# OpenGene/AfterQC

Measured on AMD Instinct MI355X. Metric: Mreads/s (paired 2x150 bp) end-to-end good/bad split, higher is better.
Workload: dtype u8

## Files before the change

### afterqc_amd/capi.py

```python
import ctypes as C
import os

import numpy as np

HERE = os.path.dirname(os.path.abspath(__file__))
LIB_PATH = os.environ.get("AQC_LIB") or os.path.join(HERE, "csrc", "libafterqc_hip.so")

AQC_MAX_READ_LEN = 1000
AQC_QC_COLS = 1024

FLAG_NAMES = ["GOOD", "BADBCD1", "BADBCD2", "BADTRIM1", "BADTRIM2", "BADBBL", "BADLEN", "BADPOL", "BADLQC",
              "BADNCT", "BADDIFF", "BADMISMATCH"]
(GOOD, BADBCD1, BADBCD2, BADTRIM1, BADTRIM2, BADBBL, BADLEN, BADPOL, BADLQC, BADNCT, BADDIFF,
 BADMISMATCH) = range(12)
N_FLAGS = 12
EDIT_FIX_R2, EDIT_FIX_R1, EDIT_MASK = 1, 2, 3
STORE_OFF, STORE_OVERLAP, STORE_MERGED = 0, 1, 2

C_TOTAL_READS, C_TOTAL_BASES, C_GOOD_READS, C_GOOD_BASES, C_FLAG0 = 0, 1, 2, 3, 4
C_READ_CORRECTED = C_FLAG0 + N_FLAGS
(C_BASE_CORRECTED, C_BASE_SKIPPED_CORRECTION, C_BASE_ZERO_QUAL_MASKED, C_OVERLAPPED, C_OVERLAP_LEN_SUM,
 C_OVERLAP_BASE_SUM, C_OVERLAP_BASE_ERR, C_TRIMMED_ADAPTER_BASE, C_TRIMMED_ADAPTER_READ,
 C_ERR_MATRIX0) = range(C_READ_CORRECTED + 1, C_READ_CORRECTED + 11)
N_COUNTERS = C_ERR_MATRIX0 + 16

(QC_TOTAL_NUM, QC_TOTAL_QUAL, QC_BASE_COUNT_A, QC_BASE_COUNT_T, QC_BASE_COUNT_C, QC_BASE_COUNT_G, QC_BASE_QUAL_A,
 QC_BASE_QUAL_T, QC_BASE_QUAL_C, QC_BASE_QUAL_G, QC_DISCONTINUITY, QC_GC_HIST, QC_SCALARS, QC_ROWS) = range(14)
QC_R1_PRE, QC_R2_PRE, QC_R1_POST, QC_R2_POST = range(4)
K_FILTER_OVERLAP, K_QC_STAT, N_KERNELS = 0, 1, 2
UINT64_MAX = (1 << 64) - 1

ERRORS = {-1: "HIP runtime error", -2: "bad argument", -3: "read longer than AQC_MAX_READ_LEN", -4: "no gfx950 device",
          -5: "bad call sequence", -6: "byte outside the reference's COMP alphabet", -7: "unsupported option value",
          -8: "quality line too short for the overlap walk (IndexError upstream)"}
ERR_ARG, ERR_ALPHABET, ERR_INDEX = -2, -6, -8
RECORD_ERRORS = (ERR_ARG, ERR_ALPHABET, ERR_INDEX)

EDIT_DTYPE = np.dtype([("o", "<u2"), ("kind", "u1"), ("base", "u1"), ("qual", "u1")])
RESULT_DTYPE = np.dtype([("flag", "u1"), ("n_edits", "u1"), ("start1", "<u2"), ("len1", "<u2"), ("start2", "<u2"),
                         ("len2", "<u2"), ("offset", "<i2"), ("overlap_len", "<u2"), ("distance", "<u2"),
                         ("edits", EDIT_DTYPE, (3,)), ("barcode", "u1")])
assert RESULT_DTYPE.itemsize == 32
SPAN_EVENT_DTYPE = np.dtype([("in_start", "<u4"), ("in_len", "<u4"), ("out_len", "<u4")])
CENSUS_HIT_DTYPE = np.dtype([("index", "<u8"), ("lane", "<i8"), ("tile_no", "<i8"), ("tile", "<i8"), ("x", "<i8"), ("y", "<i8"),
                             ("name_off", "<u4"), ("name_len", "<u4"), ("count", "<i4"), ("surface", "u1"), ("swath", "u1"),
                             ("camera", "u1"), ("base", "u1"), ("status", "u1"), ("wide", "u1"), ("pad_", "u1", (6,))])
CENSUS_OK, CENSUS_NO_NAME, CENSUS_RAISE = 0, 1, 2


def assemble_spans(chunk, end, events, stream0):
    out = []
    cursor = poff = 0
    for e in events:
        a, ln, ol = int(e["in_start"]), int(e["in_len"]), int(e["out_len"])
        out.append(bytes(chunk[cursor:a]))
        out.append(bytes(stream0[poff:poff + ol]))
        poff += ol
        cursor = a + ln
    out.append(bytes(chunk[cursor:end]))
    return b"".join(out)


class Config(C.Structure):
    _fields_ = [(n, C.c_int32) for n in (
        "paired", "count_r2_bases", "trim_front", "trim_tail", "trim_front2", "trim_tail2", "seq_len_req",
        "poly_size_limit", "allow_mismatch_in_poly", "qualified_quality_phred", "unqualified_base_limit",
        "n_base_limit", "no_overlap", "no_correction", "mask_mismatch", "barcode", "barcode_length",
        "barcode_verify_len")] + [("barcode_verify", C.c_uint8 * 32), ("debubble", C.c_int32), ("qc_kmer", C.c_int32)]

    def set_verify(self, verify):
        v = verify.encode() if isinstance(verify, str) else bytes(verify)
        if len(v) > 32:
            raise ValueError("barcode_verify longer than 32 bytes")
        self.barcode_verify_len = len(v)
        for i, ch in enumerate(v):
            self.barcode_verify[i] = ch


class CutConfig(C.Structure):
    _fields_ = [("front", C.c_int32), ("tail", C.c_int32), ("right", C.c_int32), ("window", C.c_int32), ("mean_quality", C.c_int32)]

    @property
    def on(self):
        return bool(self.front or self.tail or self.right)


class AdapterConfig(C.Structure):
    _fields_ = [("len1", C.c_int32), ("len2", C.c_int32), ("min_overlap", C.c_int32), ("seq1", C.c_uint8 * 64), ("seq2", C.c_uint8 * 64)]

    def __init__(self, seq1=b"", seq2=b"", min_overlap=4):
        super().__init__()
        seq1, seq2 = [s.encode() if isinstance(s, str) else bytes(s) for s in (seq1, seq2)]
        self.len1, self.len2, self.min_overlap = len(seq1), len(seq2), int(min_overlap)
        for dst, s in ((self.seq1, seq1), (self.seq2, seq2)):
            for i, ch in enumerate(s[:64]):
                dst[i] = ch

    @property
    def on(self):
        return bool(self.len1 or self.len2)

    def adapters(self):
        return bytes(self.seq1[:min(self.len1, 64)]), bytes(self.seq2[:min(self.len2, 64)])


class PolyConfig(C.Structure):
    _fields_ = [("min_len", C.c_int32 * 4)]

    def __init__(self, a=0, c=0, g=0, t=0):
        super().__init__()
        for i, v in enumerate((a, c, g, t)):
            self.min_len[i] = int(v)

    @property
    def on(self):
        return any(self.min_len)

    def lengths(self):
        return tuple(int(v) for v in self.min_len)


class BatchStruct(C.Structure):
    _fields_ = [("n", C.c_uint64), ("first_index", C.c_uint64),
                ("seq1", C.c_void_p), ("qual1", C.c_void_p), ("off1", C.c_void_p), ("qoff1", C.c_void_p),
                ("len1", C.c_void_p), ("bytes1", C.c_uint64), ("qbytes1", C.c_uint64),
                ("seq2", C.c_void_p), ("qual2", C.c_void_p), ("off2", C.c_void_p), ("qoff2", C.c_void_p),
                ("len2", C.c_void_p), ("bytes2", C.c_uint64), ("qbytes2", C.c_uint64),
                ("aux_lane", C.c_void_p), ("aux_tile", C.c_void_p), ("aux_x", C.c_void_p), ("aux_y", C.c_void_p),
                ("aux_ok", C.c_void_p), ("qlen1", C.c_void_p), ("qlen2", C.c_void_p)]


def _ptr(a):
    return None if a is None else a.ctypes.data_as(C.c_void_p)


class TextChunk(C.Structure):
    _fields_ = [("text1", C.c_void_p), ("bytes1", C.c_uint64), ("text2", C.c_void_p), ("bytes2", C.c_uint64),
                ("final1", C.c_int32), ("final2", C.c_int32), ("max_records", C.c_uint64), ("first_index", C.c_uint64)]


class TextExtent(C.Structure):
    _fields_ = [("offset", C.c_uint64), ("bytes", C.c_uint64), ("device_text", C.c_void_p)]


class FrameInfo(C.Structure):
    _fields_ = [("n", C.c_uint64), ("avail1", C.c_uint64), ("avail2", C.c_uint64), ("consumed1", C.c_uint64),
                ("consumed2", C.c_uint64), ("eof1", C.c_int32), ("eof2", C.c_int32), ("max_len", C.c_uint32),
                ("next_len1", C.c_uint32)]


class PipeIO(C.Structure):
    _fields_ = [("in_path", C.c_char_p * 2), ("in_mem", C.c_void_p * 2), ("in_mem_bytes", C.c_uint64 * 2),
                ("gzip_in", C.c_int32 * 2), ("out_path", (C.c_char_p * 3) * 2), ("gzip_out", C.c_int32), ("gzip_level", C.c_int32)]


class PipeOpts(C.Structure):
    _fields_ = [("chunk_records", C.c_uint64), ("qc_sample", C.c_int64), ("store_overlap", C.c_int32), ("no_output", C.c_int32),
                ("chunk_index0", C.c_uint64), ("chunk_index_stride", C.c_uint64)]


class PipeResult(C.Structure):
    _fields_ = [("records", C.c_uint64), ("chunks", C.c_uint64), ("bytes_out", C.c_uint64 * 6), ("anomaly", C.c_int32),
                ("fused_chunks", C.c_int32), ("extra_bases", C.c_uint64), ("seconds", C.c_double)] + [(k, C.c_double) for k in (
                    "t_read", "t_count", "t_wait_ring", "t_frame", "t_kernels", "t_wait_set", "t_fetch", "t_write")]

    def breakdown(self):
        return {k: round(getattr(self, k), 4) for k in ("seconds", "t_read", "t_count", "t_wait_ring", "t_frame", "t_kernels",
                                                        "t_wait_set", "t_fetch", "t_write")}


class HostBuffer:

    def __init__(self, lib, nbytes):
        self._lib = lib
        self.nbytes = int(nbytes)
        self.ptr = lib.aqc_host_alloc(self.nbytes)
        if not self.ptr:
            raise MemoryError("aqc_host_alloc(%d) failed" % self.nbytes)
        self.array = np.ctypeslib.as_array((C.c_uint8 * self.nbytes).from_address(self.ptr))
        self.view = memoryview(self.array)

    def free(self):
        if self.ptr:
            self.array = None
            self.view = None
            self._lib.aqc_host_free(self.ptr)
            self.ptr = None

# ... 68 lines not shown
    def _pack_strings(seqs, quals):
        enc = [s.encode("latin-1") if isinstance(s, str) else bytes(s) for s in seqs]
        lens = np.array([len(s) for s in enc], dtype=np.uint32)
        off, total = Batch._offsets(lens)
        sa = np.zeros(total, dtype=np.uint8)
        qa = np.zeros(total, dtype=np.uint8)
        for i, s in enumerate(enc):
            o = int(off[i])
            sa[o:o + len(s)] = np.frombuffer(s, dtype=np.uint8)
        if quals is not None:
            for i, q in enumerate(quals):
                q = q.encode("latin-1") if isinstance(q, str) else bytes(q)
                if len(q) != int(lens[i]):
                    raise ValueError("record %d: quality length %d != sequence length %d" % (i, len(q), int(lens[i])))
                o = int(off[i])
                qa[o:o + len(q)] = np.frombuffer(q, dtype=np.uint8)
        else:
            for i in range(len(enc)):
                o = int(off[i])
                qa[o:o + int(lens[i])] = ord("I")
        return sa, qa, off, lens

    @classmethod
    def from_raw(cls, rb1, rb2=None, first_index=0):
        b = cls(rb1.n, first_index)
        b.seq1 = b.qual1 = rb1.text
        b.off1, b.qoff1, b.len1 = rb1.seq_off, rb1.qual_off, rb1.seq_len
        irregular = not np.array_equal(rb1.seq_len, rb1.qual_len)
        if rb2 is not None:
            b.seq2 = b.qual2 = rb2.text
            b.off2, b.qoff2, b.len2 = rb2.seq_off, rb2.qual_off, rb2.seq_len
            irregular = irregular or not np.array_equal(rb2.seq_len, rb2.qual_len)
        if irregular:
            b.qlen1 = np.ascontiguousarray(rb1.qual_len, dtype=np.uint32)
            if rb2 is not None:
                b.qlen2 = np.ascontiguousarray(rb2.qual_len, dtype=np.uint32)
        return b

    def set_aux(self, lane, tile, x, y, ok):
        self.aux = (np.ascontiguousarray(lane, dtype=np.int32), np.ascontiguousarray(tile, dtype=np.int32),
                    np.ascontiguousarray(x, dtype=np.int32), np.ascontiguousarray(y, dtype=np.int32),
                    np.ascontiguousarray(ok, dtype=np.uint8))

    def max_len(self):
        m = int(self.len1.max()) if self.n else 0
        if self.len2 is not None and self.n:
            m = max(m, int(self.len2.max()))
        return m

    def as_struct(self):
        s = BatchStruct()
        s.n = self.n
        s.first_index = self.first_index
        s.seq1, s.qual1, s.off1, s.len1 = _ptr(self.seq1), _ptr(self.qual1), _ptr(self.off1), _ptr(self.len1)
        s.qoff1 = _ptr(self.qoff1)
        s.bytes1 = 0 if self.seq1 is None else self.seq1.size
        s.qbytes1 = 0 if self.qual1 is None else self.qual1.size
        s.seq2, s.qual2, s.off2, s.len2 = _ptr(self.seq2), _ptr(self.qual2), _ptr(self.off2), _ptr(self.len2)
        s.qoff2 = _ptr(self.qoff2)
        s.bytes2 = 0 if self.seq2 is None else self.seq2.size
        s.qbytes2 = 0 if self.qual2 is None else self.qual2.size
        if self.aux is not None:
            s.aux_lane, s.aux_tile, s.aux_x, s.aux_y, s.aux_ok = (_ptr(a) for a in self.aux)
        s.qlen1, s.qlen2 = _ptr(self.qlen1), _ptr(self.qlen2)
        return s

    def read1(self, i):
        o = int(self.off1[i]); l = int(self.len1[i])
        q = o if self.qoff1 is None else int(self.qoff1[i])
        ql = l if self.qlen1 is None else int(self.qlen1[i])
        return self.seq1[o:o + l].tobytes(), self.qual1[q:q + ql].tobytes()

    def read2(self, i):
        o = int(self.off2[i]); l = int(self.len2[i])
        q = o if self.qoff2 is None else int(self.qoff2[i])
        ql = l if self.qlen2 is None else int(self.qlen2[i])
        return self.seq2[o:o + l].tobytes(), self.qual2[q:q + ql].tobytes()


class AqcError(RuntimeError):
    def __init__(self, code, msg):
        RuntimeError.__init__(self, "afterqc_hip error %d (%s): %s" % (code, ERRORS.get(code, "?"), msg))
        self.code = code


_lib = None


def load_library():
    global _lib
    if _lib is not None:
        return _lib
    if not os.path.exists(LIB_PATH):
        raise RuntimeError("HIP library %s is missing: build it with `python __graft_entry__.py build` "
                           "(hipcc --offload-arch=gfx950); afterqc_amd has no CPU fallback" % LIB_PATH)
    lib = C.CDLL(LIB_PATH)
    P = C.c_void_p
    lib.aqc_abi_version.restype = C.c_int
    lib.aqc_device_count.restype = C.c_int
    lib.aqc_last_error.restype = C.c_char_p
    lib.aqc_create.argtypes = [C.c_int, C.c_int, C.POINTER(P)]
    lib.aqc_destroy.argtypes = [P]
    lib.aqc_destroy.restype = None
    lib.aqc_device_name.argtypes = [P, C.c_char_p, C.c_int]
    lib.aqc_set_config.argtypes = [P, C.POINTER(Config)]
    lib.aqc_set_circles.argtypes = [P, P, P, P, P, P, C.c_int32]
    lib.aqc_reset_stats.argtypes = [P]
    lib.aqc_set_quality_cut.argtypes = [P, C.POINTER(CutConfig)]
    lib.aqc_get_cut_stats.argtypes = [P, P]
    lib.aqc_cut_ms.argtypes = [P, C.c_int, C.POINTER(C.c_float)]
    lib.aqc_quality_cut_views.argtypes = [P, C.POINTER(BatchStruct), C.POINTER(CutConfig), C.c_int32, C.c_int32, P]
    lib.aqc_set_adapter_trim.argtypes = [P, C.POINTER(AdapterConfig)]
    lib.aqc_get_adapter_stats.argtypes = [P, P]
    lib.aqc_adapter_ms.argtypes = [P, C.c_int, C.POINTER(C.c_float)]
    lib.aqc_adapter_views.argtypes = [P, C.POINTER(BatchStruct), C.POINTER(AdapterConfig), C.c_int32, C.c_int32, P, P]
    lib.aqc_set_poly_trim.argtypes = [P, C.POINTER(PolyConfig)]
    lib.aqc_get_poly_stats.argtypes = [P, P]
    lib.aqc_poly_ms.argtypes = [P, C.c_int, C.POINTER(C.c_float)]
    lib.aqc_poly_views.argtypes = [P, C.POINTER(BatchStruct), C.POINTER(PolyConfig), C.c_int32, C.c_int32, P, P]
    lib.aqc_upload.argtypes = [P, C.c_int, C.POINTER(BatchStruct)]
    lib.aqc_run.argtypes = [P, C.c_int, C.c_uint64]
    lib.aqc_qc_stat.argtypes = [P, C.c_int, C.c_int, C.c_int, C.c_uint64, C.c_uint64, C.c_int]
    lib.aqc_fetch_results.argtypes = [P, C.c_int, P, C.c_uint64]
    lib.aqc_format_spans.argtypes = [P, C.c_int, C.c_uint64, C.c_int32, P, P]
    lib.aqc_fetch_span_events.argtypes = [P, C.c_int, C.c_int, P, C.c_uint64]
    lib.aqc_span_end.argtypes = [P, C.c_int, C.c_uint64, P]
    lib.aqc_poly_census.argtypes = [P, C.c_int, C.c_int32, P]
    lib.aqc_fetch_census.argtypes = [P, C.c_int, P, C.c_uint64]
    lib.aqc_census_ms.argtypes = [P, C.c_int, P]
    lib.aqc_format_fused.argtypes = [P, C.c_int]
    lib.aqc_fetch_quality_views.argtypes = [P, C.c_int, C.c_int, P, C.c_uint64]
    lib.aqc_error_record.argtypes = [P, C.c_int, C.POINTER(C.c_uint64)]
    lib.aqc_sync.argtypes = [P, C.c_int]
    lib.aqc_last_deferred.argtypes = [P, C.c_int, P, C.c_uint64, C.POINTER(C.c_uint64)]
    lib.aqc_last_deferred.restype = C.c_int
    lib.aqc_last_verdict_words.argtypes = [P, C.c_int]
    lib.aqc_last_verdict_words.restype = C.c_int
    lib.aqc_kernel_ms.argtypes = [P, C.c_int, P]
    lib.aqc_timing_reset.argtypes = [P, C.c_int]
    lib.aqc_timing_mean.argtypes = [P, C.c_int, P, P]
    lib.aqc_get_counters.argtypes = [P, P]
    lib.aqc_get_histograms.argtypes = [P, P, P, C.c_int32]
    lib.aqc_get_qc.argtypes = [P, C.c_int, P]
    lib.aqc_get_kmers.argtypes = [P, C.c_int, P, P, P, C.c_uint64, C.POINTER(C.c_uint64)]
    lib.aqc_overlap.argtypes = [P, C.POINTER(BatchStruct), P, P, P]
    lib.aqc_read_stats.argtypes = [P, C.POINTER(BatchStruct), C.c_int32, C.c_int32, C.c_int32, P, P, P]
    lib.aqc_edit_distance.argtypes = [P, C.POINTER(BatchStruct), P]
    lib.aqc_frame.argtypes = [P, C.c_int, C.POINTER(TextChunk), C.POINTER(FrameInfo)]
    lib.aqc_frame_mixed.argtypes = [P, C.c_int, C.POINTER(TextChunk), C.POINTER(TextExtent), C.c_uint64, C.c_uint8, C.POINTER(TextExtent), C.c_uint64, C.c_uint8,
                                    C.POINTER(FrameInfo)]
    lib.aqc_frame_mixed.restype = C.c_int
    lib.aqc_reframe.argtypes = [P, C.c_int, C.POINTER(FrameInfo)]
    lib.aqc_reframe.restype = C.c_int
    lib.aqc_format.argtypes = [P, C.c_int, C.c_uint64, C.c_int32, P]
    lib.aqc_format_plain.argtypes = [P, C.c_int, C.c_int, C.c_uint64, C.c_int32, P]
    lib.aqc_fetch_text.argtypes = [P, C.c_int, C.c_int, C.c_int, P, C.c_uint64]
    lib.aqc_fetch_streams.argtypes = [P, C.c_int, C.c_int32, C.POINTER(C.c_void_p * 6), C.POINTER(C.c_uint64 * 6)]
    lib.aqc_gunzip_dev.argtypes = [C.c_int, P, C.c_uint64, P, C.c_uint64, C.POINTER(C.c_uint64), P, C.c_int, C.c_uint64, C.c_uint64]
    lib.aqc_bunzip2_dev.argtypes = [C.c_int, P, C.c_uint64, P, C.c_uint64, C.POINTER(C.c_uint64), P, C.c_int, C.c_uint64]
    lib.aqc_bunzip2_dev.restype = C.c_int
    lib.aqc_gunzip_probe.argtypes = [C.c_int, C.c_int, P, C.c_uint64, C.c_int, P, P, P, C.c_uint32, C.c_uint32, C.c_uint32, P, C.c_uint64, P, P, P, P, C.c_uint64,
                                     C.POINTER(C.c_uint64), P, C.c_uint64, C.POINTER(C.c_uint64), P, C.POINTER(C.c_uint64)]
    lib.aqc_gunzip_probe.restype = C.c_int
    lib.aqc_compress.argtypes = [P, C.c_int, C.c_int32, P]
    lib.aqc_fetch_gz.argtypes = [P, C.c_int, C.c_int, C.c_int, P, C.c_uint64]
    lib.aqc_pipe_create.argtypes = [C.POINTER(P), C.c_int32, C.c_int32, C.c_int32, C.POINTER(P)]
    lib.aqc_pipe_create.restype = C.c_int
    lib.aqc_pipe_destroy.argtypes = [P]
    lib.aqc_pipe_destroy.restype = None
    lib.aqc_pipe_run.argtypes = [P, C.POINTER(PipeIO), C.POINTER(PipeOpts), C.POINTER(PipeResult)]
    lib.aqc_pipe_run.restype = C.c_int
    lib.aqc_pipe_last_error.restype = C.c_char_p
    lib.aqc_source_open.argtypes = [C.c_char_p, C.c_int32, C.c_int32]
    lib.aqc_source_open.restype = P
    lib.aqc_source_read.argtypes = [P, P, C.c_uint64]
    lib.aqc_source_read.restype = C.c_int64
    lib.aqc_source_close.argtypes = [P]
    lib.aqc_source_close.restype = None
    lib.aqc_source_open2.argtypes = [C.c_char_p, C.c_int32, C.c_int32, C.c_uint64]
    lib.aqc_source_open2.restype = P
    lib.aqc_source_error.argtypes = [P]
    lib.aqc_source_error.restype = C.c_char_p
    lib.aqc_source_gz_stats.argtypes = [P, C.POINTER(C.c_uint64 * 4)]
    lib.aqc_source_gz_stats.restype = C.c_int
    lib.aqc_gz_input_stats.argtypes = [C.POINTER(C.c_uint64 * 4)]
    lib.aqc_gz_input_stats.restype = C.c_int
    lib.aqc_bz2_input_stats.argtypes = [C.POINTER(C.c_uint64 * 4)]
    lib.aqc_bz2_input_stats.restype = C.c_int
    lib.aqc_gz_deflate_block.argtypes = [P, C.c_uint64, C.c_int32, P, C.c_uint64, C.POINTER(C.c_uint64)]
    lib.aqc_gz_deflate_block.restype = C.c_int
    lib.aqc_gz_inflate_raw.argtypes = [P, C.c_uint64, P, C.c_uint64]
    lib.aqc_gz_inflate_raw.restype = C.c_int64
    lib.aqc_gz_crc32.argtypes = [C.c_uint32, P, C.c_uint64]
    lib.aqc_gz_crc32.restype = C.c_uint32
    lib.aqc_host_count_newlines.argtypes = [P, C.c_uint64]
    lib.aqc_host_count_newlines.restype = C.c_uint64
    lib.aqc_bgzf_compress.argtypes = [P, C.c_uint64, C.c_int32, P, C.c_uint64, C.POINTER(C.c_uint64)]
    lib.aqc_bgzf_compress.restype = C.c_int
    lib.aqc_pipe_split.argtypes = [C.POINTER(PipeIO), C.c_int32, C.c_uint64, C.c_int32, P, P, C.c_uint64, C.POINTER(C.c_uint64),
                                   C.POINTER(C.c_uint32)]
    lib.aqc_pipe_split.restype = C.c_int
    lib.aqc_host_alloc.argtypes = [C.c_uint64]
    lib.aqc_host_alloc.restype = C.c_void_p
    lib.aqc_host_free.argtypes = [P]
    lib.aqc_host_free.restype = None
    for name in ("aqc_create", "aqc_device_name", "aqc_set_config", "aqc_set_circles", "aqc_reset_stats", "aqc_upload",
                 "aqc_run", "aqc_qc_stat", "aqc_fetch_results", "aqc_sync", "aqc_kernel_ms", "aqc_timing_reset",
                 "aqc_timing_mean", "aqc_get_counters", "aqc_get_histograms", "aqc_get_qc", "aqc_get_kmers",
                 "aqc_overlap", "aqc_read_stats", "aqc_edit_distance", "aqc_frame", "aqc_frame_mixed", "aqc_reframe", "aqc_format", "aqc_format_plain",
                 "aqc_fetch_text", "aqc_fetch_quality_views", "aqc_error_record", "aqc_format_spans", "aqc_fetch_span_events", "aqc_span_end", "aqc_format_fused",
                 "aqc_poly_census", "aqc_fetch_census", "aqc_census_ms", "aqc_set_quality_cut", "aqc_get_cut_stats", "aqc_cut_ms", "aqc_quality_cut_views",
                 "aqc_set_adapter_trim", "aqc_get_adapter_stats", "aqc_adapter_ms", "aqc_adapter_views",
                 "aqc_set_poly_trim", "aqc_get_poly_stats", "aqc_poly_ms", "aqc_poly_views"):
        getattr(lib, name).restype = C.c_int
    if lib.aqc_abi_version() != 3:
        raise RuntimeError("libafterqc_hip.so ABI version mismatch")
    _lib = lib
    return lib


EXPORTED_SYMBOLS = ["aqc_abi_version", "aqc_device_count", "aqc_device_index", "aqc_device_numa_node", "aqc_device_numa_node_of", "aqc_bind_thread_to_node", "aqc_last_error", "aqc_create", "aqc_destroy",
                    "aqc_device_name", "aqc_set_config", "aqc_set_circles", "aqc_reset_stats", "aqc_upload", "aqc_run",
                    "aqc_qc_stat", "aqc_fetch_results", "aqc_fetch_quality_views", "aqc_error_record", "aqc_sync", "aqc_last_deferred", "aqc_last_verdict_words", "aqc_kernel_ms", "aqc_timing_reset",
                    "aqc_timing_mean", "aqc_get_counters",
                    "aqc_get_histograms", "aqc_get_qc", "aqc_get_kmers", "aqc_overlap", "aqc_read_stats",
                    "aqc_edit_distance", "aqc_frame", "aqc_frame_mixed", "aqc_reframe", "aqc_format", "aqc_format_spans", "aqc_fetch_span_events", "aqc_span_end", "aqc_format_fused", "aqc_poly_census", "aqc_fetch_census", "aqc_census_ms", "aqc_format_plain", "aqc_fetch_text", "aqc_fetch_streams", "aqc_compress", "aqc_fetch_gz", "aqc_gunzip_dev", "aqc_bunzip2_dev", "aqc_gunzip_probe", "aqc_host_alloc",
                    "aqc_host_free",
                    "aqc_pipe_create", "aqc_pipe_destroy", "aqc_pipe_run", "aqc_pipe_last_error",
                    "aqc_host_count_newlines", "aqc_bgzf_compress", "aqc_pipe_split",
                    "aqc_source_open", "aqc_source_open2", "aqc_source_read", "aqc_source_error", "aqc_source_gz_stats", "aqc_gz_input_stats", "aqc_bz2_input_stats", "aqc_source_close",
                    "aqc_gz_deflate_block", "aqc_gz_inflate_raw", "aqc_gz_crc32",
                    "aqc_set_quality_cut", "aqc_get_cut_stats", "aqc_cut_ms", "aqc_quality_cut_views",
                    "aqc_set_adapter_trim", "aqc_get_adapter_stats", "aqc_adapter_ms", "aqc_adapter_views",
                    "aqc_set_poly_trim", "aqc_get_poly_stats", "aqc_poly_ms", "aqc_poly_views",
                    "edit_distance", "seek_overlap"]


class Engine:

    formats_merged = True

    def __init__(self, device=0, n_slots=2):
        self.lib = load_library()
        if self.lib.aqc_device_count() <= 0:
            raise RuntimeError("afterqc_amd: no AMD GPU visible (aqc_device_count() == 0); the HIP path is the only "
                               "path — there is no CPU fallback")
        h = C.c_void_p()
        self._check(self.lib.aqc_create(device, n_slots, C.byref(h)))
        self.h = h
        self.n_slots = n_slots
        self.slot_n = [0] * n_slots

    def _check(self, rc):
        if rc != 0:
            raise AqcError(rc, (self.lib.aqc_last_error() or b"").decode("utf-8", "replace"))

    def close(self):
        if getattr(self, "h", None):
            self.lib.aqc_destroy(self.h)
            self.h = None

    def __del__(self):
        try:
            self.close()
        except Exception:
            pass

    def device_name(self):
        buf = C.create_string_buffer(256)
        self._check(self.lib.aqc_device_name(self.h, buf, 256))
        return buf.value.decode()

    def set_config(self, cfg):
        self._check(self.lib.aqc_set_config(self.h, C.byref(cfg)))

    def set_circles(self, circles):
        n = len(circles)
        cx = np.array([c[0] for c in circles], dtype=np.float64)
        cy = np.array([c[1] for c in circles], dtype=np.float64)
        cr = np.array([c[2] for c in circles], dtype=np.float64)
        ln = np.array([c[3] for c in circles], dtype=np.int32)
        tl = np.array([c[4] for c in circles], dtype=np.int32)
        self._check(self.lib.aqc_set_circles(self.h, _ptr(cx), _ptr(cy), _ptr(cr), _ptr(ln), _ptr(tl), n))

    def reset_stats(self):
        self._check(self.lib.aqc_reset_stats(self.h))

    def _four_counts(self, getter):
        out = np.zeros(4, dtype=np.int64)
        self._check(getter(self.h, _ptr(out)))
        return out

    def _pass_ms(self, getter, slot):
        ms = C.c_float(0)
        self._check(getter(self.h, slot, C.byref(ms)))
        return float(ms.value)

    def set_quality_cut(self, cut):
        self._check(self.lib.aqc_set_quality_cut(self.h, C.byref(cut) if cut is not None else None))

    def cut_stats(self):
        return self._four_counts(self.lib.aqc_get_cut_stats)

    def cut_ms(self, slot):
        return self._pass_ms(self.lib.aqc_cut_ms, slot)

    def set_adapter_trim(self, adapter):
        self._check(self.lib.aqc_set_adapter_trim(self.h, C.byref(adapter) if adapter is not None else None))

    def adapter_stats(self):
        return self._four_counts(self.lib.aqc_get_adapter_stats)

    def adapter_ms(self, slot):
        return self._pass_ms(self.lib.aqc_adapter_ms, slot)

    def set_poly_trim(self, poly):
        self._check(self.lib.aqc_set_poly_trim(self.h, C.byref(poly) if poly is not None else None))

    def poly_stats(self):
        return self._four_counts(self.lib.aqc_get_poly_stats)

    def poly_ms(self, slot):
        return self._pass_ms(self.lib.aqc_poly_ms, slot)

    def upload(self, slot, batch):
        s = batch.as_struct()
        self._check(self.lib.aqc_upload(self.h, slot, C.byref(s)))
        self.slot_n[slot] = batch.n

    def run(self, slot, accum_limit=UINT64_MAX):
        self._check(self.lib.aqc_run(self.h, slot, accum_limit))

    def qc_stat(self, slot, which, mate, first, count, post):
        self._check(self.lib.aqc_qc_stat(self.h, slot, which, mate, first, count, 1 if post else 0))

    def fetch_results(self, slot):
        out = np.zeros(self.slot_n[slot], dtype=RESULT_DTYPE)
        self._check(self.lib.aqc_fetch_results(self.h, slot, _ptr(out), self.slot_n[slot]))
        return out

    def sync(self, slot):
        self._check(self.lib.aqc_sync(self.h, slot))

    def fetch_quality_views(self, slot, mate):
        out = np.zeros(self.slot_n[slot], dtype=np.uint32)
        self._check(self.lib.aqc_fetch_quality_views(self.h, slot, mate, _ptr(out), self.slot_n[slot]))
        return (out & 0xffff).astype(np.int64), (out >> 16).astype(np.int64)

    def error_record(self, slot):
        rec = C.c_uint64(0)
        self._check(self.lib.aqc_error_record(self.h, slot, C.byref(rec)))
        return None if rec.value == UINT64_MAX else int(rec.value)

    def last_deferred(self, slot, want_indices=False):
        n = C.c_uint64(0)
        cap = self.slot_n[slot] if want_indices else 0
        idx = np.zeros(max(cap, 1), dtype=np.uint32)
        self._check(self.lib.aqc_last_deferred(self.h, slot, _ptr(idx), cap, C.byref(n)))
        return (int(n.value), idx[:min(int(n.value), cap)]) if want_indices else int(n.value)

    def last_verdict_words(self, slot):
        w = self.lib.aqc_last_verdict_words(self.h, slot)
        if w < 0:
            self._check(w)
        return int(w)

    def kernel_ms(self, slot):
        ms = np.zeros(N_KERNELS, dtype=np.float32)
        self._check(self.lib.aqc_kernel_ms(self.h, slot, _ptr(ms)))
        return ms

    def timing_reset(self, slot):
        self._check(self.lib.aqc_timing_reset(self.h, slot))

    def timing_mean(self, slot):
        ms = np.zeros(N_KERNELS, dtype=np.float32)
        n = np.zeros(N_KERNELS, dtype=np.int32)
        self._check(self.lib.aqc_timing_mean(self.h, slot, _ptr(ms), _ptr(n)))
        return ms, n

    def counters(self):
        out = np.zeros(N_COUNTERS, dtype=np.int64)
        self._check(self.lib.aqc_get_counters(self.h, _ptr(out)))
        return out

    def histograms(self, n=AQC_QC_COLS):
        a = np.zeros(n, dtype=np.int64)
        b = np.zeros(n, dtype=np.int64)
        self._check(self.lib.aqc_get_histograms(self.h, _ptr(a), _ptr(b), n))
        return a, b

    def qc(self, which):
        out = np.zeros((QC_ROWS, AQC_QC_COLS), dtype=np.int64)
        self._check(self.lib.aqc_get_qc(self.h, which, _ptr(out)))
        return out

    def kmers(self, which, cap=1 << 22):
        keys = np.zeros(cap, dtype=np.uint64)
        counts = np.zeros(cap, dtype=np.int64)
        order = np.zeros(cap, dtype=np.uint64)
        n = C.c_uint64(0)
        self._check(self.lib.aqc_get_kmers(self.h, which, _ptr(keys), _ptr(counts), _ptr(order), cap, C.byref(n)))
        m = n.value
        return keys[:m], counts[:m], order[:m]

    def host_buffer(self, nbytes):
        return HostBuffer(self.lib, nbytes)

    def frame(self, slot, text1, bytes1, final1, text2=None, bytes2=0, final2=False, max_records=UINT64_MAX, first_index=0):
        ch = TextChunk()
        ch.text1, ch.bytes1, ch.final1 = text1.ctypes.data, int(bytes1), 1 if final1 else 0
        if text2 is not None:
            ch.text2, ch.bytes2, ch.final2 = text2.ctypes.data, int(bytes2), 1 if final2 else 0
        ch.max_records, ch.first_index = int(max_records), int(first_index)
        info = FrameInfo()
        self._check(self.lib.aqc_frame(self.h, slot, C.byref(ch), C.byref(info)))
        self.slot_n[slot] = info.n
        return info

    def reframe(self, slot):
        info = FrameInfo()
        self._check(self.lib.aqc_reframe(self.h, slot, C.byref(info)))
        self.slot_n[slot] = info.n
        return info

    def format(self, slot, n, store_overlap=False):
        sizes = np.zeros(6, dtype=np.uint64)
        self._check(self.lib.aqc_format(self.h, slot, int(n), int(store_overlap), _ptr(sizes)))
        return [int(x) for x in sizes]

    def format_spans(self, slot, n, store_overlap=False):
        sizes = (C.c_uint64 * 6)()
        n_ev = (C.c_uint64 * 2)()
        self._check(self.lib.aqc_format_spans(self.h, slot, n, int(store_overlap), sizes, n_ev))
        return [int(x) for x in sizes], [int(x) for x in n_ev]

    def fetch_span_events(self, slot, file, n_events):
        ev = np.zeros(max(n_events, 1), dtype=SPAN_EVENT_DTYPE)
        self._check(self.lib.aqc_fetch_span_events(self.h, slot, file, _ptr(ev), n_events))
        return ev[:n_events]

    def format_fused(self, slot):
        rc = self.lib.aqc_format_fused(self.h, slot)
        if rc < 0:
            self._check(rc)
        return rc == 1

    def span_end(self, slot, n):
        end = (C.c_uint64 * 2)()
        self._check(self.lib.aqc_span_end(self.h, slot, n, end))
        return [int(x) for x in end]

    def poly_census(self, slot, poly_max):
        n = C.c_uint64()
        self._check(self.lib.aqc_poly_census(self.h, slot, int(poly_max), C.byref(n)))
        return int(n.value)

    def fetch_census(self, slot, n):
        out = np.zeros(n, dtype=CENSUS_HIT_DTYPE)
        if n:
            self._check(self.lib.aqc_fetch_census(self.h, slot, _ptr(out), n))
        return out

    def census_ms(self, slot):
        ms = C.c_float()
        self._check(self.lib.aqc_census_ms(self.h, slot, C.byref(ms)))
        return float(ms.value)

    def format_plain(self, slot, verdict_slot, n, store_overlap=False):
        sizes = np.zeros(6, dtype=np.uint64)
        self._check(self.lib.aqc_format_plain(self.h, slot, verdict_slot, int(n), int(store_overlap), _ptr(sizes)))
        return [int(x) for x in sizes]

    def compress(self, slot, level=2):
        sizes = np.zeros(6, dtype=np.uint64)
        self._check(self.lib.aqc_compress(self.h, slot, int(level), _ptr(sizes)))
        return [int(x) for x in sizes]

    def fetch_gz(self, slot, file, stream, dst, cap):
        self._check(self.lib.aqc_fetch_gz(self.h, slot, file, stream, dst.ctypes.data if dst is not None else None, int(cap)))

    def fetch_text(self, slot, file, stream, dst, cap):
        self._check(self.lib.aqc_fetch_text(self.h, slot, file, stream, dst.ctypes.data if dst is not None else None, int(cap)))

    def overlap(self, batch):
        n = batch.n
        off = np.zeros(n, dtype=np.int32); ol = np.zeros(n, dtype=np.int32); df = np.zeros(n, dtype=np.int32)
        s = batch.as_struct()
        self._check(self.lib.aqc_overlap(self.h, C.byref(s), _ptr(off), _ptr(ol), _ptr(df)))
        return off, ol, df

    def read_stats(self, batch, max_poly, mismatch, qual):
        n = batch.n
        px = np.zeros(n, dtype=np.uint8); lq = np.zeros(n, dtype=np.int32); nn = np.zeros(n, dtype=np.int32)
        s = batch.as_struct()
        self._check(self.lib.aqc_read_stats(self.h, C.byref(s), max_poly, mismatch, qual, _ptr(px), _ptr(lq), _ptr(nn)))
        return px, lq, nn

    def quality_cut_views(self, batch, cut, trim_front=0, trim_tail=0):
        v = np.zeros(batch.n, dtype=np.uint32)
        s = batch.as_struct()
        self._check(self.lib.aqc_quality_cut_views(self.h, C.byref(s), C.byref(cut), int(trim_front), int(trim_tail), _ptr(v)))
        return (v & 0xffff).astype(np.int64), (v >> 16).astype(np.int64)

    def adapter_views(self, batch, adapter, trim_front=0, trim_tail=0, view_in=None):
        v = np.zeros(batch.n, dtype=np.uint32)
        vin = None
        if view_in is not None:
            vin = (np.asarray(view_in[0], dtype=np.uint32) | (np.asarray(view_in[1], dtype=np.uint32) << 16)).astype(np.uint32)
            assert vin.shape == (batch.n,)
        s = batch.as_struct()
        self._check(self.lib.aqc_adapter_views(self.h, C.byref(s), C.byref(adapter), int(trim_front), int(trim_tail),
                                               _ptr(vin) if vin is not None else None, _ptr(v)))
        return (v & 0xffff).astype(np.int64), (v >> 16).astype(np.int64)

    def poly_views(self, batch, poly, trim_front=0, trim_tail=0, view_in=None):
        v = np.zeros(batch.n, dtype=np.uint32)
        vin = None
        if view_in is not None:
            vin = (np.asarray(view_in[0], dtype=np.uint32) | (np.asarray(view_in[1], dtype=np.uint32) << 16)).astype(np.uint32)
            assert vin.shape == (batch.n,)
        s = batch.as_struct()
        self._check(self.lib.aqc_poly_views(self.h, C.byref(s), C.byref(poly), int(trim_front), int(trim_tail),
                                            _ptr(vin) if vin is not None else None, _ptr(v)))
        return (v & 0xffff).astype(np.int64), (v >> 16).astype(np.int64)

    def edit_distance(self, batch):
        d = np.zeros(batch.n, dtype=np.int32)
        s = batch.as_struct()
        self._check(self.lib.aqc_edit_distance(self.h, C.byref(s), _ptr(d)))
        return d


class Pipe:

    def __init__(self, engines, slots=3, io_threads=0):
        self.lib = load_library()
        self.engines = list(engines)
        arr = (C.c_void_p * len(self.engines))(*[e.h for e in self.engines])
        h = C.c_void_p()
        rc = self.lib.aqc_pipe_create(arr, len(self.engines), slots, io_threads, C.byref(h))
        if rc != 0:
            raise AqcError(rc, "aqc_pipe_create failed")
        self.h = h

    def close(self):
        if getattr(self, "h", None):
            self.lib.aqc_pipe_destroy(self.h)
            self.h = None

    def __del__(self):
        try:
            self.close()
        except Exception:
            pass

    def run(self, inputs, outputs=None, gzip_in=(False, False), gzip_out=False, gzip_level=2, chunk_records=0, qc_sample=200000,
            store_overlap=False, no_output=False, chunk_index0=0, chunk_index_stride=1):
        io = PipeIO()
        keep = []
        for k, src in enumerate(inputs):
            if src is None:
                continue
            if isinstance(src, (str, bytes)):
                b = src.encode() if isinstance(src, str) else src
                keep.append(b)
                io.in_path[k] = b
                io.gzip_in[k] = int(gzip_in[k]) if gzip_in[k] else 0
            else:
                arr, nbytes = src
                keep.append(arr)
# ... 215 lines not shown
```

### afterqc_amd/csrc/aqc_capi.hip

```cpp
#include <hip/hip_runtime.h>

#include <cstdarg>
#include <cstdio>
#include <cstdlib>
#include <cstring>
#include <algorithm>
#include <mutex>
#include <vector>

#include "aqc_ctx.hpp"
#include <sys/mman.h>
#include <sched.h>
#include <pthread.h>
#include <cctype>

using namespace aqc;

static thread_local char g_err[512] = "";

int aqc::fail(int code, const char* fmt, ...) {
    va_list ap;
    va_start(ap, fmt);
    vsnprintf(g_err, sizeof(g_err), fmt, ap);
    va_end(ap);
    return code;
}

namespace aqc {

hipEvent_t launch_event(Slot& s, int k, int which) {
    if (s.collecting && s.ring_used[k] < RING_CAP) {
        if ((int)s.ring[k][which].size() <= s.ring_used[k]) {
            hipEvent_t e = nullptr;
            (void)hipEventCreate(&e);
            s.ring[k][which].push_back(e);
        }
        hipEvent_t e = s.ring[k][which][s.ring_used[k]];
        if (which == 1) s.ring_used[k]++;
        return e;
    }
    return s.ev[k][which];
}

hipError_t slot_sync(Slot& s) {
    hipError_t e = hipStreamSynchronize(s.stream);
    const uint64_t g = s.qc.gen.load(std::memory_order_acquire);
    if (e == hipSuccess && s.qc.synced.load(std::memory_order_acquire) < g) {
        e = hipEventSynchronize(s.ev_qc);
        if (e == hipSuccess) {
            uint64_t seen = s.qc.synced.load(std::memory_order_relaxed);
            while (seen < g && !s.qc.synced.compare_exchange_weak(seen, g, std::memory_order_release)) { }
        }
    }
    return e;
}

const char* status_text(int st, bool at_record) {
    if (st == AQC_ERR_ALPHABET) return "a base outside the reference's COMP table reached the correction walk (KeyError upstream)";
    if (at_record) {
        if (st == AQC_ERR_INDEX) return "the overlap walk read a quality line beyond its length — the line is shorter than its sequence line (IndexError upstream)";
        if (st == AQC_ERR_ARG) return "a name field the bubble filter converts with int() is not a number (ValueError upstream)";
    } else {
        if (st == AQC_ERR_READ_TOO_LONG) return "a read (or its quality line) is longer than AQC_MAX_READ_LEN";
        if (st == AQC_ERR_ARG) return "a read shorter than 5 bases reached statRead (IndexError upstream)";
        if (st == AQC_ERR_UNSUPPORTED) return "device limit exceeded (k-mer table full or string longer than 64)";
    }
    return "device-side error";
}

int check_status(Slot& sl) {
    StatusWords w{0, 0, ~0ull};
    HIP_TRY(hipMemcpyAsync(&w, sl.status, sizeof(w), hipMemcpyDeviceToHost, sl.stream));
    HIP_TRY(hipStreamSynchronize(sl.stream));
    int st = w.status;
    if (st != 0) {
        (void)hipMemcpyAsync(sl.status, &STATUS_CLEAR, sizeof(STATUS_CLEAR), hipMemcpyHostToDevice, sl.stream);
        (void)hipStreamSynchronize(sl.stream);
        sl.err_record = UINT64_MAX;
        const bool record_kind = st == AQC_ERR_INDEX || st == AQC_ERR_ALPHABET || st == AQC_ERR_ARG;
        if (w.err_key != ~0ull && record_kind) {
            sl.err_record = w.err_key >> 8;
            st = -(int)(w.err_key & 0xffu);
            return fail(st, "%s; record %llu of the chunk — the run ends there, the records before it are valid (aqc_error_record)", status_text(st, true),
                        (unsigned long long)sl.err_record);
        }
        return fail(st, "%s", status_text(st, false));
    }
    return 0;
}

int get_slot(aqc_ctx* c, int slot, Slot** out) {
    if (!c) return fail(AQC_ERR_ARG, "null context");
    if (slot < 0 || slot >= c->n_slots) return fail(AQC_ERR_ARG, "slot %d out of range", slot);
    HIP_TRY(hipSetDevice(c->device));
    *out = &c->slots[slot];
    return 0;
}

int fetch_out(Slot& s, const void* src, uint64_t bytes, void* dst, uint64_t cap, const char* who) {
    if (bytes > cap) return fail(AQC_ERR_ARG, "%s: %llu bytes do not fit %llu", who, (unsigned long long)bytes, (unsigned long long)cap);
    if (bytes) {
        if (!dst) return fail(AQC_ERR_ARG, "%s: null destination", who);
        HIP_TRY(hipMemcpyAsync(dst, src, bytes, hipMemcpyDeviceToHost, s.stream));
    }
    HIP_TRY(hipStreamSynchronize(s.stream));
    return check_status(s);
}

int sync_all(aqc_ctx* c) {
    HIP_TRY(hipSetDevice(c->device));
    for (auto& s : c->slots) {
        HIP_TRY(slot_sync(s));
        int rc = check_status(s);
        if (rc) return rc;
    }
    return 0;
}

}

extern "C" {

int aqc_abi_version(void) { return AQC_ABI_VERSION; }

int aqc_device_count(void) {
    int n = 0;
    if (hipGetDeviceCount(&n) != hipSuccess) return 0;
    return n;
}

const char* aqc_last_error(void) { return g_err; }

int aqc_create(int device, int n_slots, aqc_ctx** out) {
    if (!out || n_slots < 1 || n_slots > 16) return fail(AQC_ERR_ARG, "aqc_create: bad arguments");
    int n = 0;
    if (hipGetDeviceCount(&n) != hipSuccess || n <= 0) return fail(AQC_ERR_NO_DEVICE, "no HIP device visible");
    if (device < 0 || device >= n) return fail(AQC_ERR_ARG, "device %d out of range (%d visible)", device, n);
    HIP_TRY(hipSetDevice(device));
    {
        const char* sy = getenv("AQC_SYNC");
        if (!(sy && !strcmp(sy, "spin")) && hipSetDeviceFlags(hipDeviceScheduleBlockingSync) != hipSuccess) (void)hipGetLastError();
    }
    aqc_ctx* c = new aqc_ctx();
    c->device = device;
    c->n_slots = n_slots;
    c->slots = std::vector<Slot>(n_slots);
    hipDeviceProp_t prop;
    HIP_TRY(hipGetDeviceProperties(&prop, device));
    snprintf(c->name, sizeof(c->name), "%s (%s, %d CUs)", prop.name, prop.gcnArchName, prop.multiProcessorCount);
    c->n_cu = prop.multiProcessorCount > 0 ? prop.multiProcessorCount : 256;
    const char* fg = getenv("AQC_FORCE_GENERIC");
    c->force_generic = fg && fg[0] == '1';
    const char* fu = getenv("AQC_FUSED");
    c->fuse_opt = fu && fu[0] == '1';
    const char* qi = getenv("AQC_QC_STREAM");
    c->qc_inline = qi && qi[0] == '0';
    if (int rc = allow_kmer_lds()) return rc;
    HIP_TRY(hipStreamCreateWithFlags(&c->qc_stream, hipStreamNonBlocking));
    for (auto& s : c->slots) {
        HIP_TRY(hipStreamCreateWithFlags(&s.stream, hipStreamNonBlocking));
        for (int k = 0; k < AQC_N_KERNELS; k++)
            for (int j = 0; j < 2; j++) HIP_TRY(hipEventCreate(&s.ev[k][j]));
        HIP_TRY(hipEventCreateWithFlags(&s.ev_main, hipEventDisableTiming));
        HIP_TRY(hipEventCreateWithFlags(&s.ev_qc, hipEventDisableTiming));
    }
    HIP_TRY(hipMalloc((void**)&c->counters, sizeof(unsigned long long) * (AQC_N_COUNTERS + 16)));
    HIP_TRY(hipMalloc((void**)&c->ovl_hist, sizeof(unsigned long long) * AQC_QC_COLS));
    HIP_TRY(hipMalloc((void**)&c->dist_hist, sizeof(unsigned long long) * AQC_QC_COLS));
    for (auto& s : c->slots) {
        HIP_TRY(hipMalloc((void**)&s.status, sizeof(StatusWords)));
        HIP_TRY(hipMemcpy(s.status, &STATUS_CLEAR, sizeof(STATUS_CLEAR), hipMemcpyHostToDevice));
    }
    for (int k = 0; k < 4; k++)
        HIP_TRY(hipMalloc((void**)&c->qc[k].acc, sizeof(unsigned long long) * AQC_QC_ROWS * AQC_QC_COLS));
    *out = c;
    return aqc_reset_stats(c);
}

void aqc_destroy(aqc_ctx* c) {
    if (!c) return;
    (void)hipSetDevice(c->device);
    (void)hipDeviceSynchronize();
    for (auto& s : c->slots) {
        for (int k = 0; k < AQC_N_KERNELS; k++)
            for (int j = 0; j < 2; j++) {
                if (s.ev[k][j]) (void)hipEventDestroy(s.ev[k][j]);
                for (hipEvent_t e : s.ring[k][j]) (void)hipEventDestroy(e);
            }
        if (s.status) (void)hipFree(s.status);
        for (hipEvent_t e : s.census_ev) if (e) (void)hipEventDestroy(e);
        for (ViewPass& vp : s.pass)
            for (hipEvent_t e : vp.ev) if (e) (void)hipEventDestroy(e);
        if (s.ev_main) (void)hipEventDestroy(s.ev_main);
        if (s.ev_qc) (void)hipEventDestroy(s.ev_qc);
        if (s.stream) (void)hipStreamDestroy(s.stream);
    }
    if (c->qc_stream) (void)hipStreamDestroy(c->qc_stream);
    (void)hipFree(c->counters); (void)hipFree(c->ovl_hist); (void)hipFree(c->dist_hist);
    for (PassCounts& pc : c->pass_stats) pc.free();
    for (int k = 0; k < 4; k++) {
        (void)hipFree(c->qc[k].acc);
        free_kmer(c->qc[k].kt);
    }
    delete c;
}

int aqc_device_index(aqc_ctx* c) { return c ? c->device : -1; }

int aqc_device_numa_node_of(int device) {
    char bus[64] = "";
    if (hipDeviceGetPCIBusId(bus, (int)sizeof(bus), device) != hipSuccess) { (void)hipGetLastError(); return -1; }
    for (char* p = bus; *p; ++p) *p = (char)tolower((unsigned char)*p);
    char path[160];
    snprintf(path, sizeof(path), "/sys/bus/pci/devices/%s/numa_node", bus);
    int node = -1;
    if (FILE* f = fopen(path, "r")) {
        if (fscanf(f, "%d", &node) != 1) node = -1;
        fclose(f);
    }
    return node;
}
int aqc_device_numa_node(aqc_ctx* c) { return c ? aqc_device_numa_node_of(c->device) : -1; }

int aqc_bind_thread_to_node(int node) {
    if (node < 0) return 0;
    if (const char* e = getenv("AQC_PIPE_NUMA")) if (e[0] == '0') return 0;
    char path[96];
    snprintf(path, sizeof(path), "/sys/devices/system/node/node%d/cpulist", node);
    FILE* f = fopen(path, "r");
    if (!f) return 0;
    char list[4096] = "";
    const bool got = fgets(list, sizeof(list), f) != nullptr;
    fclose(f);
    if (!got) return 0;
    cpu_set_t have, want;
    CPU_ZERO(&want);
    if (sched_getaffinity(0, sizeof(have), &have) != 0) return 0;
    int n = 0;
    for (char* p = list; *p;) {
        char* q;
        const long a = strtol(p, &q, 10);
        if (q == p) break;
        long b = a;
        if (*q == '-') { p = q + 1; b = strtol(p, &q, 10); }
        for (long cpu = a; cpu <= b && cpu < CPU_SETSIZE; ++cpu)
            if (CPU_ISSET((int)cpu, &have)) { CPU_SET((int)cpu, &want); ++n; }
        p = *q == ',' ? q + 1 : q;
        if (*q != ',') break;
    }
    if (n == 0 || n == CPU_COUNT(&have)) return 0;
    if (pthread_setaffinity_np(pthread_self(), sizeof(want), &want) != 0) return 0;
    return n;
}

int aqc_device_name(aqc_ctx* c, char* buf, int buflen) {
    if (!c || !buf || buflen <= 0) return fail(AQC_ERR_ARG, "aqc_device_name: bad arguments");
    snprintf(buf, (size_t)buflen, "%s", c->name);
    return 0;
}

int aqc_set_config(aqc_ctx* c, const aqc_config* cfg) {
    if (!c || !cfg) return fail(AQC_ERR_ARG, "aqc_set_config: null argument");
    if (cfg->trim_front < 0 || cfg->trim_tail < 0 || cfg->trim_front2 < 0 || cfg->trim_tail2 < 0)
        return fail(AQC_ERR_ARG, "trim values must be resolved (>= 0) before they reach the device");
    if (cfg->qc_kmer < 1 || cfg->qc_kmer > 8) return fail(AQC_ERR_UNSUPPORTED, "qc_kmer %d outside 1..8", cfg->qc_kmer);
    if (cfg->barcode) {
        if (cfg->barcode_verify_len < 0 || cfg->barcode_verify_len > 32 || cfg->barcode_length < 1 ||
            cfg->barcode_length + 1 + cfg->barcode_verify_len > 62)
            return fail(AQC_ERR_UNSUPPORTED, "barcode_length + verify too long for the device path");
    }
    c->cfg = *cfg;
    c->has_cfg = true;
    return 0;
}

int aqc_set_quality_cut(aqc_ctx* c, const aqc_cut_config* cut) {
    if (!c) return fail(AQC_ERR_ARG, "aqc_set_quality_cut: null context");
    QcutOpts o{};
    if (cut) o = QcutOpts{cut->front ? 1 : 0, cut->tail ? 1 : 0, cut->right ? 1 : 0, cut->window, cut->mean_quality};
    if (!qcut_on(o)) { c->cut = QcutOpts{}; return 0; }
    if (!qcut_opts_ok(o))
        return fail(AQC_ERR_ARG, "aqc_set_quality_cut: window %d (1 .. %d) / mean quality %d (0 .. %d)", o.window, AQC_MAX_READ_LEN, o.mean_quality, QCUT_MAX_QUALITY);
    HIP_TRY(c->pass_stats[VP_CUT].ensure(c->device));
    c->cut = o;
    return 0;
}

static int get_pass_stats(aqc_ctx* c, ViewPassId which, int64_t out[4]) {
    if (!c || !out) return fail(AQC_ERR_ARG, "null argument");
    int rc = sync_all(c);
    if (rc) return rc;
    HIP_TRY(c->pass_stats[which].get(out));
    return 0;
}
int aqc_get_cut_stats(aqc_ctx* c, int64_t out[4]) { return get_pass_stats(c, VP_CUT, out); }

int aqc_set_adapter_trim(aqc_ctx* c, const aqc_adapter_config* adapter) {
    if (!c) return fail(AQC_ERR_ARG, "aqc_set_adapter_trim: null context");
    AdapterOpts a{};
    if (!adp_from_config(adapter, a))
        return fail(AQC_ERR_ARG, "aqc_set_adapter_trim: adapter lengths %d / %d (0 or %d .. %d letters of ACGT), min overlap %d (1 .. the shorter adapter)",
                    adapter->len1, adapter->len2, ADP_MIN_LEN, ADP_MAX_LEN, adapter->min_overlap);
    if (!adp_on(a)) { c->adapter = AdapterOpts{}; return 0; }
    HIP_TRY(c->pass_stats[VP_ADAPTER].ensure(c->device));
    c->adapter = a;
    return 0;
}

int aqc_get_adapter_stats(aqc_ctx* c, int64_t out[4]) { return get_pass_stats(c, VP_ADAPTER, out); }

int aqc_set_poly_trim(aqc_ctx* c, const aqc_poly_config* poly) {
    if (!c) return fail(AQC_ERR_ARG, "aqc_set_poly_trim: null context");
    PolyOpts o{};
    if (!poly_from_config(poly, o))
        return fail(AQC_ERR_ARG, "aqc_set_poly_trim: minimum lengths %d / %d / %d / %d of A / C / G / T (0: off, or 1 .. %d)", poly->min_len[0], poly->min_len[1],
                    poly->min_len[2], poly->min_len[3], POLY_MAX_MIN_LEN);
    if (!poly_on(o)) { c->poly = PolyOpts{}; return 0; }
    HIP_TRY(c->pass_stats[VP_POLY].ensure(c->device));
    c->poly = o;
    return 0;
}

int aqc_get_poly_stats(aqc_ctx* c, int64_t out[4]) { return get_pass_stats(c, VP_POLY, out); }

int aqc_set_circles(aqc_ctx* c, const double* cx, const double* cy, const double* r, const int32_t* lane,
                    const int32_t* tile, int32_t n) {
    if (!c || n < 0) return fail(AQC_ERR_ARG, "aqc_set_circles: bad arguments");
    HIP_TRY(hipSetDevice(c->device));
    c->circles = DevCircles{};
    c->circles.n = n;
    if (n == 0) return 0;
    const void* src[5] = {cx, cy, r, lane, tile};
    const size_t sz[5] = {sizeof(double) * n, sizeof(double) * n, sizeof(double) * n, sizeof(int32_t) * n, sizeof(int32_t) * n};
    for (int k = 0; k < 5; k++) {
        if (!src[k]) return fail(AQC_ERR_ARG, "aqc_set_circles: null array");
        if (c->circ[k].reserve(sz[k])) return fail(AQC_ERR_HIP, "hipMalloc failed");
        HIP_TRY(hipMemcpy(c->circ[k].p, src[k], sz[k], hipMemcpyHostToDevice));
    }
    c->circles.cx = (const double*)c->circ[0].p;
    c->circles.cy = (const double*)c->circ[1].p;
    c->circles.cr = (const double*)c->circ[2].p;
    c->circles.lane = (const int32_t*)c->circ[3].p;
    c->circles.tile = (const int32_t*)c->circ[4].p;
    return 0;
}

int aqc_reset_stats(aqc_ctx* c) {
    if (!c) return fail(AQC_ERR_ARG, "null context");
    HIP_TRY(hipSetDevice(c->device));
    HIP_TRY(hipDeviceSynchronize());
    HIP_TRY(hipMemset(c->counters, 0, sizeof(unsigned long long) * (AQC_N_COUNTERS + 16)));
    HIP_TRY(hipMemset(c->ovl_hist, 0, sizeof(unsigned long long) * AQC_QC_COLS));
    HIP_TRY(hipMemset(c->dist_hist, 0, sizeof(unsigned long long) * AQC_QC_COLS));
    for (PassCounts& pc : c->pass_stats) HIP_TRY(pc.zero());
    for (auto& sl : c->slots) { HIP_TRY(hipMemcpy(sl.status, &STATUS_CLEAR, sizeof(STATUS_CLEAR), hipMemcpyHostToDevice)); sl.err_record = UINT64_MAX; }
    for (int k = 0; k < 4; k++) {
        HIP_TRY(hipMemset(c->qc[k].acc, 0, sizeof(unsigned long long) * AQC_QC_ROWS * AQC_QC_COLS));
        c->qc[k].last_end = 0;
        c->qc[k].epoch = 0;
        if (c->qc[k].kt.keys) {
// ... 165 lines not shown
```

### afterqc_amd/csrc/aqc_capi_run.hip

```cpp
#include <hip/hip_runtime.h>

#include <cstdio>
#include <cstdlib>
#include <functional>
#include <mutex>
#include <vector>

#include "aqc_ctx.hpp"
#include "aqc_prim.hpp"
#include "aqc_upload.hpp"
#include "aqc_record.hpp"
#include "aqc_seams.hpp"
#include "aqc_fast.hpp"
#include "aqc_gzdev.hpp"
#include "aqc_gzlz.hpp"
#include "aqc_gz.hpp"
#include <zlib.h>

using namespace aqc;

static bool views_on(const aqc_ctx* c) { return qcut_on(c->cut) || adp_on(c->adapter) || poly_on(c->poly); }

constexpr int FUSE_WPBT = 12;
#ifndef AQC_TIER20_WPBT
// ... 324 lines not shown
                           (const unsigned int*)s->n_deferred.p);
    }
    HIP_TRY(hipGetLastError());
    HIP_TRY(hipEventRecord(launch_event(*s, AQC_K_FILTER_OVERLAP, 1), s->stream));
    s->timed[AQC_K_FILTER_OVERLAP] = !s->collecting;
    s->ran = true;
    return 0;
}

int aqc_fetch_results(aqc_ctx* c, int slot, aqc_result* out, uint64_t n) {
    GET_SLOT(s);
    if (!s->ran) return fail(AQC_ERR_STATE, "aqc_fetch_results before aqc_run");
    if (n > s->n) return fail(AQC_ERR_ARG, "aqc_fetch_results: n exceeds the slot's records");
    if (n) HIP_TRY(hipMemcpyAsync(out, s->results.p, sizeof(aqc_result) * n, hipMemcpyDeviceToHost, s->stream));
    HIP_TRY(slot_sync(*s));
    return check_status(*s);
}

int aqc_fetch_quality_views(aqc_ctx* c, int slot, int mate, uint32_t* out, uint64_t n) {
    GET_SLOT(s);
    if (!s->ran) return fail(AQC_ERR_STATE, "aqc_fetch_quality_views before aqc_run");
    if (n > s->n || !out || mate < 0 || mate > 1 || (mate == 1 && !s->paired)) return fail(AQC_ERR_ARG, "aqc_fetch_quality_views: bad arguments");
    if (n == 0) return 0;
    if (s->off_stage.reserve(sizeof(uint32_t) * n)) return fail(AQC_ERR_HIP, "hipMalloc failed");
    hipLaunchKernelGGL(quality_views_kernel, dim3((unsigned)((n + 255) / 256)), dim3(256), 0, s->stream, s->view, (const aqc_result*)s->results.p, mate,
                       (uint32_t*)s->off_stage.p, n);
    HIP_TRY(hipGetLastError());
    HIP_TRY(hipMemcpyAsync(out, s->off_stage.p, sizeof(uint32_t) * n, hipMemcpyDeviceToHost, s->stream));
    HIP_TRY(slot_sync(*s));
    return 0;
}

static int view_pass_ms(aqc_ctx* c, int slot, ViewPassId which, float* ms, const char* who) {
    GET_SLOT(s);
    if (!ms) return fail(AQC_ERR_ARG, "%s: null argument", who);
    *ms = 0.f;
    const ViewPass& vp = s->pass[which];
    if (!vp.ran) return 0;
    HIP_TRY(slot_sync(*s));
    HIP_TRY(hipEventElapsedTime(ms, vp.ev[0], vp.ev[1]));
    return 0;
}
int aqc_cut_ms(aqc_ctx* c, int slot, float* ms) { return view_pass_ms(c, slot, VP_CUT, ms, "aqc_cut_ms"); }
int aqc_adapter_ms(aqc_ctx* c, int slot, float* ms) { return view_pass_ms(c, slot, VP_ADAPTER, ms, "aqc_adapter_ms"); }
int aqc_poly_ms(aqc_ctx* c, int slot, float* ms) { return view_pass_ms(c, slot, VP_POLY, ms, "aqc_poly_ms"); }

int aqc_last_verdict_words(aqc_ctx* c, int slot) {
    GET_SLOT(s);
    if (!s->ran) return fail(AQC_ERR_STATE, "aqc_last_verdict_words before aqc_run");
    return s->verdict_words;
}

int aqc_last_deferred(aqc_ctx* c, int slot, uint32_t* idx, uint64_t cap, uint64_t* n) {
    GET_SLOT(s);
    if (!n) return fail(AQC_ERR_ARG, "aqc_last_deferred: null argument");
    if (!s->ran) return fail(AQC_ERR_STATE, "aqc_last_deferred before aqc_run");
    HIP_TRY(slot_sync(*s));
    *n = 0;
    if (!s->used_fast || !s->n_deferred.p) return 0;
    unsigned int m = 0;
    HIP_TRY(hipMemcpy(&m, s->n_deferred.p, sizeof(m), hipMemcpyDeviceToHost));
    *n = m;
    const uint64_t w = m < cap ? m : cap;
    if (idx && w) HIP_TRY(hipMemcpy(idx, s->deferred.p, sizeof(uint32_t) * w, hipMemcpyDeviceToHost));
    return 0;
}

static int ensure_gz_tables(aqc_ctx* c) {
    if (c->gz_crc.p) return 0;
    GzCrcTables t;
    for (uint32_t i = 0; i < 256; ++i) {
        uint32_t v = i;
        for (int k = 0; k < 8; ++k) v = (v >> 1) ^ (0xEDB88320u & (0u - (v & 1u)));
        t.byte_table[i] = v;
    }
    for (int k = 0; k < 8; ++k)
        for (int j = 0; j < 32; ++j) t.shift[k][j] = (uint32_t)crc32_combine((uLong)(1u << j), 0UL, (z_off_t)(GZ_SEG << k));
    if (c->gz_crc.reserve(sizeof(t))) return fail(AQC_ERR_HIP, "hipMalloc failed");
    HIP_TRY(hipMemcpy(c->gz_crc.p, &t, sizeof(t), hipMemcpyHostToDevice));
    return 0;
}

int aqc_compress(aqc_ctx* c, int slot, int32_t level, uint64_t gz_bytes_out[6]) {
    GET_SLOT(s);
    int rc;
    if (!gz_bytes_out) return fail(AQC_ERR_ARG, "aqc_compress: null argument");
    if (!s->formatted) return fail(AQC_ERR_STATE, "aqc_compress before aqc_format");
    if (level < 1) return fail(AQC_ERR_UNSUPPORTED, "aqc_compress: level %d (stored output is the host writer's business)", level);
    if (level > 9) return fail(AQC_ERR_ARG, "aqc_compress: level %d (1 .. 9)", level);
    if ((rc = ensure_gz_tables(c))) return rc;
    static_assert(sizeof(GzCodebookDev) == sizeof(aqcgz::GzCodebook), "host and device codebook layouts must agree");
    GzJob J{};
    uint32_t n_members = 0;
    static const bool wave_enc = [] { const char* e = getenv("AQC_GZ_ENCODER"); return !(e && e[0] == 's'); }();
    static const bool lz_on = [] { const char* e = getenv("AQC_GZ_LZ"); return !(e && e[0] == '0'); }();
    const bool lz = level >= 6 && lz_on;
    const bool wave_members = wave_enc && !lz;
    J.member_text = wave_members ? (uint32_t)GZW_TEXT : (uint32_t)GZ_TEXT;
    J.slot_bytes = wave_members ? (uint32_t)GZW_SLOT : (uint32_t)GZ_SLOT;
    for (int q = 0; q < 6; ++q) {
        J.text[q] = (const uint8_t*)s->f_out[q].p;
        J.bytes[q] = s->f_bytes[q];
        J.first_block[q] = n_members;
        n_members += (uint32_t)((s->f_bytes[q] + J.member_text - 1) / J.member_text);
        s->g_bytes[q] = 0;
        gz_bytes_out[q] = 0;
    }
    J.first_block[6] = n_members;
    if (n_members == 0) { s->compressed = true; return 0; }
    if (s->g_stage.reserve((size_t)n_members * J.slot_bytes) || s->g_sizes.reserve(4 * (size_t)n_members) || s->g_offsets.reserve(8 * (size_t)n_members) ||
        s->g_total.reserve(64) || s->g_hist.reserve(6 * 320 * 4) || s->g_code.reserve(6 * sizeof(GzCodebookDev)))
        return fail(AQC_ERR_HIP, "hipMalloc failed");
    for (int q = 0; q < 6; ++q) {
        const uint64_t nb = J.first_block[q + 1] - J.first_block[q];
        if (s->g_packed[q].reserve(nb * (J.member_text + 31) + 64)) return fail(AQC_ERR_HIP, "hipMalloc failed");
        J.packed[q] = (uint8_t*)s->g_packed[q].p;
    }
    J.stage = (uint8_t*)s->g_stage.p; J.sizes = (uint32_t*)s->g_sizes.p; J.offsets = (uint64_t*)s->g_offsets.p; J.total = (uint64_t*)s->g_total.p;
    J.hist = (uint32_t*)s->g_hist.p; J.code = (const GzCodebookDev*)s->g_code.p; J.crc = (const GzCrcTables*)c->gz_crc.p;
    HIP_TRY(hipMemsetAsync(s->g_hist.p, 0, 6 * 320 * 4, s->stream));
    if (lz) hipLaunchKernelGGL(gz_hist_lz_kernel, dim3(6 * GZ_SAMPLES), dim3(WAVE), 0, s->stream, J, gzlz_depth(level));
    else hipLaunchKernelGGL(gz_hist_kernel, dim3(6 * GZ_SAMPLES), dim3(GZ_THREADS), 0, s->stream, J);
    HIP_TRY(hipGetLastError());
    uint32_t h[6][320];
    HIP_TRY(hipMemcpyAsync(h, s->g_hist.p, sizeof(h), hipMemcpyDeviceToHost, s->stream));
    HIP_TRY(hipStreamSynchronize(s->stream));
    std::vector<aqcgz::GzCodebook> cb(6);
    for (int q = 0; q < 6; ++q)
        if (!aqcgz::build_codebook(h[q], h[q] + 286, &cb[q])) return fail(AQC_ERR_STATE, "aqc_compress: could not build a Huffman code");
    HIP_TRY(hipMemcpyAsync(s->g_code.p, cb.data(), 6 * sizeof(aqcgz::GzCodebook), hipMemcpyHostToDevice, s->stream));
    if (lz) hipLaunchKernelGGL(gz_encode_lz_kernel, dim3(n_members), dim3(WAVE), 0, s->stream, J, gzlz_depth(level));
    else if (wave_enc) hipLaunchKernelGGL(gz_encode_wave_kernel, dim3(n_members), dim3(WAVE), 0, s->stream, J);
    else hipLaunchKernelGGL(gz_encode_kernel, dim3(n_members), dim3(GZ_THREADS), 0, s->stream, J);
    hipLaunchKernelGGL(gz_offsets_kernel, dim3(6), dim3(GZ_THREADS), 0, s->stream, J);
    hipLaunchKernelGGL(gz_pack_kernel, dim3(n_members), dim3(GZ_THREADS), 0, s->stream, J);
    HIP_TRY(hipGetLastError());
    unsigned long long tot[6];
    HIP_TRY(hipMemcpyAsync(tot, s->g_total.p, sizeof(tot), hipMemcpyDeviceToHost, s->stream));
    HIP_TRY(hipStreamSynchronize(s->stream));
    for (int q = 0; q < 6; ++q) {
        s->g_bytes[q] = tot[q];
        gz_bytes_out[q] = tot[q];
    }
    rc = check_status(*s);
    s->compressed = rc == 0;
    return rc;
}

int aqc_fetch_gz(aqc_ctx* c, int slot, int file, int stream, uint8_t* dst, uint64_t cap) {
    GET_SLOT(s);
    if (!s->compressed) return fail(AQC_ERR_STATE, "aqc_fetch_gz before aqc_compress");
    if (file < 0 || file > 1 || stream < 0 || stream > 2) return fail(AQC_ERR_ARG, "aqc_fetch_gz: bad file/stream");
    const int q = file * 3 + stream;
    return fetch_out(*s, s->g_packed[q].p, s->g_bytes[q], dst, cap, "aqc_fetch_gz");
}

static int seam_prepare(aqc_ctx* c, const aqc_batch* b, bool need_qual, bool need_pair, Slot** out) {
    if (!c || !b) return fail(AQC_ERR_ARG, "null argument");
    Slot* s;
    int rc = get_slot(c, c->n_slots - 1, &s);
    if (rc) return rc;
    if ((rc = fill_slot(c, *s, b, need_qual, need_pair))) return rc;
    for (uint64_t i = 0; i < b->n; i++)
        if (b->len1[i] > AQC_MAX_READ_LEN || (need_pair && b->len2[i] > AQC_MAX_READ_LEN))
            return fail(AQC_ERR_READ_TOO_LONG, "record %llu is longer than %d", (unsigned long long)i, AQC_MAX_READ_LEN);
    *out = s;
    return 0;
}

static int seam_out_bytes(Slot* s, DevBuf& d, void* host, size_t bytes) {
    if (bytes) HIP_TRY(hipMemcpyAsync(host, d.p, bytes, hipMemcpyDeviceToHost, s->stream));
    return 0;
}
#define seam_out(s, d, host, n) seam_out_bytes(s, d, host, sizeof(*(host)) * (n))

int aqc_overlap(aqc_ctx* c, const aqc_batch* b, int32_t* offset, int32_t* overlap_len, int32_t* diff) {
    Slot* s;
    int rc = seam_prepare(c, b, false, true, &s);
    if (rc) return rc;
    const uint64_t n = b->n;
    if (n == 0) return 0;
    DevBuf o[3];
    for (auto& d : o)
        if (d.reserve(4 * n)) return fail(AQC_ERR_HIP, "hipMalloc failed");
    hipLaunchKernelGGL(overlap_seam_kernel, dim3((unsigned)((n + WPB - 1) / WPB)), dim3(BLOCK), 0, s->stream, s->view,
                       (int32_t*)o[0].p, (int32_t*)o[1].p, (int32_t*)o[2].p);
    HIP_TRY(hipGetLastError());
    if ((rc = seam_out(s, o[0], offset, n)) || (rc = seam_out(s, o[1], overlap_len, n)) || (rc = seam_out(s, o[2], diff, n))) return rc;
    HIP_TRY(slot_sync(*s));
    return 0;
}

int aqc_read_stats(aqc_ctx* c, const aqc_batch* b, int32_t max_poly, int32_t mismatch, int32_t qual, uint8_t* polyx,
                   int32_t* low_qual, int32_t* n_count) {
    Slot* s;
    int rc = seam_prepare(c, b, true, false, &s);
    if (rc) return rc;
    const uint64_t n = b->n;
    if (n == 0) return 0;
    DevBuf o[3];
    if (o[0].reserve(n) || o[1].reserve(4 * n) || o[2].reserve(4 * n)) return fail(AQC_ERR_HIP, "hipMalloc failed");
    hipLaunchKernelGGL(read_stats_seam_kernel, dim3((unsigned)((n + WPB - 1) / WPB)), dim3(BLOCK), 0, s->stream, s->view,
                       max_poly, mismatch, qual, (uint8_t*)o[0].p, (int32_t*)o[1].p, (int32_t*)o[2].p);
    HIP_TRY(hipGetLastError());
    if ((rc = seam_out(s, o[0], polyx, n)) || (rc = seam_out(s, o[1], low_qual, n)) || (rc = seam_out(s, o[2], n_count, n))) return rc;
    HIP_TRY(slot_sync(*s));
    return 0;
}

int aqc_edit_distance(aqc_ctx* c, const aqc_batch* b, int32_t* dist) {
    Slot* s;
    int rc = seam_prepare(c, b, false, true, &s);
    if (rc) return rc;
    const uint64_t n = b->n;
    if (n == 0) return 0;
    DevBuf o;
    if (o.reserve(4 * n)) return fail(AQC_ERR_HIP, "hipMalloc failed");
    hipLaunchKernelGGL(edit_distance_seam_kernel, dim3((unsigned)((n + 255) / 256)), dim3(256), 0, s->stream, s->view,
                       (int32_t*)o.p, s->status);
    HIP_TRY(hipGetLastError());
    if ((rc = seam_out(s, o, dist, n))) return rc;
    HIP_TRY(slot_sync(*s));
    return check_status(*s);
}

static int view_seam(aqc_ctx* c, const aqc_batch* b, bool need_qual, const uint32_t* view_in, uint32_t* view,
                     const std::function<int(Slot&, uint32_t*)>& launch) {
    Slot* s;
    int rc = seam_prepare(c, b, need_qual, false, &s);
    if (rc) return rc;
    const uint64_t n = b->n;
    if (n == 0) return 0;
    DevBuf out;
    if (out.reserve(4 * n)) return fail(AQC_ERR_HIP, "hipMalloc failed");
    if (view_in) HIP_TRY(hipMemcpyAsync(out.p, view_in, 4 * n, hipMemcpyHostToDevice, s->stream));
    if ((rc = launch(*s, (uint32_t*)out.p))) return rc;
    if ((rc = seam_out(s, out, view, n))) return rc;
    HIP_TRY(slot_sync(*s));
    return check_status(*s);
}

int aqc_quality_cut_views(aqc_ctx* c, const aqc_batch* b, const aqc_cut_config* cut, int32_t trim_front, int32_t trim_tail, uint32_t* view) {
    if (!cut || !view) return fail(AQC_ERR_ARG, "aqc_quality_cut_views: null argument");
    const QcutOpts o{cut->front ? 1 : 0, cut->tail ? 1 : 0, cut->right ? 1 : 0, cut->window, cut->mean_quality};
    if (!qcut_opts_ok(o) || trim_front < 0 || trim_tail < 0) return fail(AQC_ERR_ARG, "aqc_quality_cut_views: window / mean quality / trim out of range");
    const int32_t tf[2] = {trim_front, 0}, tt[2] = {trim_tail, 0};
    return view_seam(c, b, true, nullptr, view, [&](Slot& s, uint32_t* v) { return launch_cut(c, s, o, tf, tt, 1, v, nullptr, UINT64_MAX); });
}

int aqc_adapter_views(aqc_ctx* c, const aqc_batch* b, const aqc_adapter_config* adapter, int32_t trim_front, int32_t trim_tail, const uint32_t* view_in,
                      uint32_t* view) {
    if (!adapter || !view) return fail(AQC_ERR_ARG, "aqc_adapter_views: null argument");
    AdapterOpts a{};
    if (!adp_from_config(adapter, a) || trim_front < 0 || trim_tail < 0) return fail(AQC_ERR_ARG, "aqc_adapter_views: adapter / min overlap / trim out of range");
    a.len[1] = 0;
    const int32_t tf[2] = {trim_front, 0}, tt[2] = {trim_tail, 0};
    return view_seam(c, b, b && b->qual1 != nullptr, view_in, view,
                     [&](Slot& s, uint32_t* v) { return launch_adapter(c, s, a, tf, tt, 1, view_in ? v : nullptr, v, nullptr, UINT64_MAX); });
}

int aqc_poly_views(aqc_ctx* c, const aqc_batch* b, const aqc_poly_config* poly, int32_t trim_front, int32_t trim_tail, const uint32_t* view_in,
                   uint32_t* view) {
    if (!poly || !view) return fail(AQC_ERR_ARG, "aqc_poly_views: null argument");
    PolyOpts o{};
    if (!poly_from_config(poly, o) || trim_front < 0 || trim_tail < 0) return fail(AQC_ERR_ARG, "aqc_poly_views: minimum length / trim out of range");
    const int32_t tf[2] = {trim_front, 0}, tt[2] = {trim_tail, 0};
    return view_seam(c, b, b && b->qual1 != nullptr, view_in, view,
                     [&](Slot& s, uint32_t* v) { return launch_poly(c, s, o, tf, tt, 1, view_in ? v : nullptr, v, nullptr, UINT64_MAX); });
}

static std::mutex g_compat_mu;
static aqc_ctx* g_compat = nullptr;
static DevBuf* const g_compat_buf = new DevBuf[4];

static int compat_prepare(const char* a, size_t la, const char* b, size_t lb, size_t row_bytes) {
    if (!g_compat) {
        int rc = aqc_create(0, 1, &g_compat);
        if (rc) { g_compat = nullptr; return rc; }
    }
    HIP_TRY(hipSetDevice(g_compat->device));
    if (g_compat_buf[0].reserve(la + 16) || g_compat_buf[1].reserve(lb + 16) || g_compat_buf[2].reserve(row_bytes + 16) ||
        g_compat_buf[3].reserve(16))
        return fail(AQC_ERR_HIP, "hipMalloc failed");
    if (la) HIP_TRY(hipMemcpy(g_compat_buf[0].p, a, la, hipMemcpyHostToDevice));
    if (lb) HIP_TRY(hipMemcpy(g_compat_buf[1].p, b, lb, hipMemcpyHostToDevice));
    return 0;
}

unsigned int edit_distance(const char* a, const unsigned int asize, const char* b, const unsigned int bsize) {
    if (asize == 0) return bsize;
    if (bsize == 0) return asize;
    std::lock_guard<std::mutex> g(g_compat_mu);
    int out = -1;
    if (compat_prepare(a, asize, b, bsize, sizeof(int) * ((size_t)bsize + 1)) == 0) {
        hipLaunchKernelGGL(edit_distance_any_kernel, dim3(1), dim3(WAVE), 0, 0, (const uint8_t*)g_compat_buf[0].p, (int)asize,
                           (const uint8_t*)g_compat_buf[1].p, (int)bsize, (int*)g_compat_buf[2].p, (int*)g_compat_buf[3].p);
        if (hipMemcpy(&out, g_compat_buf[3].p, sizeof(int), hipMemcpyDeviceToHost) != hipSuccess) out = -1;
    }
    if (out < 0) fprintf(stderr, "libafterqc_hip: edit_distance failed: %s\n", aqc_last_error());
    return (unsigned int)out;
}

int seek_overlap(const char* r1, const int len1, const char* r2, const int len2, const int limit_distance,
                 const int complete_compare_require, const int overlap_require) {
    std::lock_guard<std::mutex> g(g_compat_mu);
    int out = 0x7FFFFFFF;
    bool ok = len1 >= 0 && len2 >= 0 && compat_prepare(r1, (size_t)len1, r2, (size_t)len2, 0) == 0;
// ... 13 lines not shown
```

### afterqc_amd/csrc/aqc_capi_text.hip

```cpp
#include <hip/hip_runtime.h>

#include <cstddef>
#include <cstdlib>
#include <cstring>
#include <algorithm>

#include "aqc_ctx.hpp"
#include "aqc_prim.hpp"
#include "aqc_fast.hpp"
#include "aqc_textin.hpp"
#include "aqc_fmt.hpp"
#include "aqc_fmtcopy.hpp"
#include "aqc_census.hpp"

using namespace aqc;

extern "C" {

struct TextScratch {
    alignas(64) FrameMeta meta[2];
    alignas(64) unsigned long long lines[2];
    union alignas(64) { FrameOut frame; unsigned long long fmt_totals[FMT_STREAMS]; };
};
constexpr size_t TEXT_SCRATCH_BYTES = 256;
static_assert(offsetof(TextScratch, lines) == 64 && offsetof(TextScratch, frame) == 128 && offsetof(TextScratch, fmt_totals) == 128 &&
              sizeof(TextScratch) <= TEXT_SCRATCH_BYTES, "the kernels of both stages were measured with these places");

struct FrameExtents { const aqc_text_extent* ext[2]; uint64_t n[2]; uint8_t last[2]; };
struct FrameJob {
    const aqc_text_chunk* ch;
    int nf;
    const uint8_t* text[2];
    uint64_t bytes[2];
    uint8_t* tbase[2];
    uint64_t tiles[2], cap[2];
    uint32_t virt[2];
    bool bubble;
};
constexpr size_t TEXT_SLACK = IDX_TILE + 64;

static int put_extents(Slot* s, const FrameJob& j, int k, const FrameExtents& fx) {
    uint64_t cur = 0;
    for (uint64_t e = 0; e < fx.n[k]; ++e) {
        const aqc_text_extent& x = fx.ext[k][e];
        if (x.offset < cur || x.offset + x.bytes > j.bytes[k] || !x.device_text) return fail(AQC_ERR_ARG, "aqc_frame_mixed: extents must be sorted, disjoint and inside the chunk");
        if (x.offset > cur) HIP_TRY(hipMemcpyAsync(j.tbase[k] + cur, j.text[k] + cur, x.offset - cur, hipMemcpyHostToDevice, s->stream));
        if (x.bytes) HIP_TRY(hipMemcpyAsync(j.tbase[k] + x.offset, x.device_text, x.bytes, hipMemcpyDeviceToDevice, s->stream));
        cur = x.offset + x.bytes;
    }
    if (j.bytes[k] > cur) HIP_TRY(hipMemcpyAsync(j.tbase[k] + cur, j.text[k] + cur, j.bytes[k] - cur, hipMemcpyHostToDevice, s->stream));
    return 0;
}

static int put_text(Slot* s, FrameJob& j, int k, bool resident, const FrameExtents* fx) {
    Mate& m = s->m[k];
    if (m.seq.reserve(TEXT_FRONT + j.bytes[k] + TEXT_SLACK)) return fail(AQC_ERR_HIP, "hipMalloc of %llu bytes failed", (unsigned long long)j.bytes[k]);
    j.tbase[k] = (uint8_t*)m.seq.p + TEXT_FRONT;
    if (resident) return 0;
    const bool mixed = fx && fx->n[k];
    if (mixed) {
        const int rc = put_extents(s, j, k, *fx);
        if (rc) return rc;
    } else if (j.bytes[k]) HIP_TRY(hipMemcpyAsync(j.tbase[k], j.text[k], j.bytes[k], hipMemcpyHostToDevice, s->stream));
    HIP_TRY(hipMemsetAsync(j.tbase[k] + j.bytes[k], 0, TEXT_SLACK, s->stream));
    m.last_byte = !j.bytes[k] ? (uint8_t)'\n' : mixed ? fx->last[k] : j.text[k][j.bytes[k] - 1];
    return 0;
}

static int size_line_table(Slot* s, FrameJob& j, int k) {
    DevBuf& le = s->m[k].line_end;
    j.tiles[k] = j.bytes[k] ? (j.bytes[k] + IDX_TILE - 1) / IDX_TILE : 1;
    const uint64_t guess = j.bytes[k] / 16 + 4096;
    j.cap[k] = le.cap / sizeof(uint32_t) > guess + 2 ? le.cap / sizeof(uint32_t) - 2 : guess;
    if (le.reserve(sizeof(uint32_t) * (j.cap[k] + 2))) return fail(AQC_ERR_HIP, "hipMalloc failed");
    return 0;
}

static int launch_index_and_frame(Slot* s, const FrameJob& j, TextScratch* sc) {
    const uint64_t all_tiles = j.tiles[0] + j.tiles[1];
    HIP_TRY(hipMemsetAsync(s->t_tile.p, 0, sizeof(unsigned long long) * (all_tiles + 1), s->stream));
    IndexFile f[2] = {};
    uint32_t t0 = 0;
    for (int k = 0; k < j.nf; k++) {
        f[k] = IndexFile{(const uint8_t*)j.tbase[k], j.bytes[k], (uint32_t*)s->m[k].line_end.p, j.cap[k], sc->lines + k, t0, (uint32_t)j.tiles[k]};
        t0 += (uint32_t)j.tiles[k];
    }
    hipLaunchKernelGGL(text_index_kernel, dim3((unsigned)all_tiles), dim3(TXT_BLOCK), 0, s->stream, f[0], f[1],
                       (unsigned long long*)s->t_tile.p, (unsigned int*)((unsigned long long*)s->t_tile.p + all_tiles));
    HIP_TRY(hipGetLastError());
    const FrameMeta init{0xffffffffu, 0u, 0xffffffffu, 0u};
    const FrameMeta h_meta[2] = {init, init};
    HIP_TRY(hipMemcpyAsync(sc->meta, h_meta, sizeof(h_meta), hipMemcpyHostToDevice, s->stream));
    uint64_t rec_cap = 0;
    for (int k = 0; k < j.nf; k++) {
        Mate& m = s->m[k];
        const uint64_t r = (j.cap[k] + 1) / 4 + 1;
        rec_cap = std::max(rec_cap, r);
        if (m.off.reserve(4 * r) || m.qoff.reserve(4 * r) || m.len.reserve(4 * r) || m.name_off.reserve(4 * r) || m.name_len.reserve(4 * r) ||
            m.plus_off.reserve(4 * r) || m.plus_len.reserve(4 * r) || m.qual_len.reserve(4 * r))
            return fail(AQC_ERR_HIP, "hipMalloc failed");
        FramedFile ff{(uint32_t*)m.off.p, (uint32_t*)m.qoff.p, (uint32_t*)m.len.p, (uint32_t*)m.name_off.p,
                      (uint32_t*)m.name_len.p, (uint32_t*)m.plus_off.p, (uint32_t*)m.plus_len.p, (uint32_t*)m.qual_len.p};
        hipLaunchKernelGGL(frame_records_kernel, dim3((unsigned)((r + TXT_BLOCK - 1) / TXT_BLOCK)), dim3(TXT_BLOCK), 0, s->stream,
                           (const uint8_t*)j.tbase[k], (const uint32_t*)m.line_end.p, (const unsigned long long*)(sc->lines + k), j.virt[k], ff, sc->meta + k, (uint64_t)j.cap[k]);
    }
    hipLaunchKernelGGL(frame_finish_kernel, dim3(1), dim3(1), 0, s->stream, (const unsigned long long*)sc->lines, (const FrameMeta*)sc->meta,
                       (const uint32_t*)s->m[0].line_end.p, (const uint32_t*)s->m[j.nf - 1].line_end.p, (const uint32_t*)s->m[0].len.p,
                       j.virt[0], j.virt[1], (unsigned long long)j.bytes[0], (unsigned long long)j.bytes[1], j.nf, (unsigned long long)j.ch->max_records, &sc->frame,
                       (unsigned long long)j.cap[0], (unsigned long long)j.cap[1]);
    if (j.bubble) {
        for (int k = 0; k < 5; k++)
            if (s->aux[k].reserve((k < 4 ? sizeof(int32_t) : 1) * rec_cap)) return fail(AQC_ERR_HIP, "hipMalloc failed");
        hipLaunchKernelGGL(parse_names_kernel, dim3((unsigned)((rec_cap + TXT_BLOCK - 1) / TXT_BLOCK)), dim3(TXT_BLOCK), 0, s->stream,
                           (const uint8_t*)j.tbase[0], (const uint32_t*)s->m[0].name_off.p, (const uint32_t*)s->m[0].name_len.p, (const unsigned long long*)&sc->frame.n,
                           (int32_t*)s->aux[0].p, (int32_t*)s->aux[1].p, (int32_t*)s->aux[2].p, (int32_t*)s->aux[3].p,
                           (uint8_t*)s->aux[4].p);
    }
    HIP_TRY(hipGetLastError());
    return 0;
}

static int index_and_frame(Slot* s, FrameJob& j, FrameOut& fo) {
    TextScratch* sc = (TextScratch*)s->t_scratch.p;
    for (int attempt = 0; attempt < 2; ++attempt) {
        const int rc = launch_index_and_frame(s, j, sc);
        if (rc) return rc;
        HIP_TRY(hipMemcpyAsync(&fo, &sc->frame, sizeof(fo), hipMemcpyDeviceToHost, s->stream));
        HIP_TRY(slot_sync(*s));
        bool fits = true;
        for (int k = 0; k < j.nf; k++) {
            const uint64_t real = fo.lines[k] - (j.virt[k] ? 1 : 0);
            if (real > j.cap[k]) {
                fits = false;
                j.cap[k] = real;
                if (s->m[k].line_end.reserve(sizeof(uint32_t) * (j.cap[k] + 2))) return fail(AQC_ERR_HIP, "hipMalloc failed");
            }
        }
        if (fits) break;
    }
    return 0;
}

static int publish_view(Slot* s, const FrameJob& j, const FrameOut& fo) {
    const uint64_t n = fo.n;
    DevBatch v{};
    v.n = n;
    v.first_index = j.ch->first_index;
    if (s->results.reserve(sizeof(aqc_result) * (n ? n : 1))) return fail(AQC_ERR_HIP, "hipMalloc failed");
    s->has_irregular = fo.first_mismatch[0] < n || (j.nf == 2 && fo.first_mismatch[1] < n);
    for (int k = 0; k < j.nf; k++) {
        Mate& m = s->m[k];
        if (s->has_irregular && m.qview.reserve(sizeof(uint32_t) * (n ? n : 1))) return fail(AQC_ERR_HIP, "hipMalloc failed");
        set_mate(v, k, MateView{j.tbase[k], j.tbase[k], (const uint32_t*)m.off.p, (const uint32_t*)m.qoff.p, (const uint32_t*)m.len.p,
                                (const uint32_t*)m.qual_len.p, (uint32_t*)m.qview.p});
    }
    for (int k = 0; k < 2; k++) s->m[k].consumed = fo.consumed[k];
    if (j.bubble) {
        v.aux_lane = (const int32_t*)s->aux[0].p; v.aux_tile = (const int32_t*)s->aux[1].p;
        v.aux_x = (const int32_t*)s->aux[2].p; v.aux_y = (const int32_t*)s->aux[3].p; v.aux_ok = (const uint8_t*)s->aux[4].p;
    }
    s->view = v;
    s->n = n;
    s->paired = j.nf == 2;
    s->raw_max_len = s->max_len = fo.max_len;
    return 0;
}

static void fill_frame_info(aqc_frame_info* info, const FrameOut& fo, bool paired) {
    memset(info, 0, sizeof(*info));
    info->n = fo.n;
    info->avail1 = fo.avail[0];
    info->avail2 = fo.avail[1];
    info->eof1 = (int32_t)fo.eof[0];
    info->eof2 = paired ? (int32_t)fo.eof[1] : 0;
    info->max_len = fo.max_len;
    info->consumed1 = fo.consumed[0];
    info->consumed2 = fo.consumed[1];
    info->next_len1 = fo.next_len1;
}

static int frame_impl(aqc_ctx* c, int slot, const aqc_text_chunk* ch, aqc_frame_info* info, bool resident, const FrameExtents* fx = nullptr) {
    GET_SLOT(s);
    if (!ch || !info || !ch->text1) return fail(AQC_ERR_ARG, "aqc_frame: null argument");
    const bool paired = ch->text2 != nullptr;
    FrameJob j{ch, paired ? 2 : 1, {ch->text1, ch->text2}, {ch->bytes1, paired ? ch->bytes2 : 0}};
    for (int k = 0; k < j.nf; k++)
        if (j.bytes[k] >= (1ull << 31) - IDX_TILE) return fail(AQC_ERR_ARG, "aqc_frame: chunks must be < 2 GiB");
    HIP_TRY(slot_sync(*s));
    s->framed = s->formatted = false;
    s->ran = false;
    s->fused = false;
    if (s->t_scratch.reserve(TEXT_SCRATCH_BYTES)) return fail(AQC_ERR_HIP, "hipMalloc failed");
    int rc;
    for (int k = 0; k < j.nf; k++)
        if ((rc = put_text(s, j, k, resident, fx)) || (rc = size_line_table(s, j, k))) return rc;
    if (s->t_tile.reserve(sizeof(unsigned long long) * (j.tiles[0] + j.tiles[1] + 1))) return fail(AQC_ERR_HIP, "hipMalloc failed");
    const int final_[2] = {ch->final1, ch->final2};
    for (int k = 0; k < j.nf; k++)
        if (final_[k] && j.bytes[k] > 0 && s->m[k].last_byte != '\n') j.virt[k] = (uint32_t)j.bytes[k] | LINE_WS;
    j.bubble = c->has_cfg && c->cfg.debubble;
    FrameOut fo{};
    if ((rc = index_and_frame(s, j, fo)) || (rc = publish_view(s, j, fo))) return rc;
    fill_frame_info(info, fo, paired);
    s->framed = true;
    s->last_chunk = *ch;
    return 0;
}

int aqc_frame(aqc_ctx* c, int slot, const aqc_text_chunk* ch, aqc_frame_info* info) { return frame_impl(c, slot, ch, info, false); }

int aqc_frame_mixed(aqc_ctx* c, int slot, const aqc_text_chunk* ch, const aqc_text_extent* ext1, uint64_t n_ext1, uint8_t last1,
                    const aqc_text_extent* ext2, uint64_t n_ext2, uint8_t last2, aqc_frame_info* info) {
    if ((n_ext1 && !ext1) || (n_ext2 && !ext2)) return fail(AQC_ERR_ARG, "aqc_frame_mixed: null extent list");
    const FrameExtents fx{{ext1, ext2}, {n_ext1, ch && ch->text2 ? n_ext2 : 0}, {last1, last2}};
    return frame_impl(c, slot, ch, info, false, &fx);
}

int aqc_reframe(aqc_ctx* c, int slot, aqc_frame_info* info) {
    GET_SLOT(s);
    if (!s->framed) return fail(AQC_ERR_STATE, "aqc_reframe needs a slot filled by aqc_frame");
    const aqc_text_chunk ch = s->last_chunk;
    return frame_impl(c, slot, &ch, info, true);
}

static FormatView make_format_view(const aqc_ctx* c, const Slot* s, const Slot* vs, bool plain, int32_t store_overlap, bool spans) {
    FormatView v{};
    v.paired = s->paired ? 1 : 0;
    v.results = (const aqc_result*)vs->results.p;
    v.plain = plain ? 1 : 0;
    v.verdict_paired = vs->paired ? 1 : 0;
    v.barcode = c->cfg.barcode ? 1 : 0;
    v.barcode_length = c->cfg.barcode_length;
    v.store_overlap = !(store_overlap && vs->paired) ? 0 : store_overlap == AQC_STORE_MERGED ? AQC_STORE_MERGED : AQC_STORE_OVERLAP;
    v.spans = (spans && !plain) ? 1 : 0;
    v.n_framed = s->n;
    v.consumed[0] = (uint32_t)s->m[0].consumed; v.consumed[1] = (uint32_t)s->m[1].consumed;
    for (int k = 0; k < (s->paired ? 2 : 1); k++) {
        const Mate& m = s->m[k];
        v.f[k].text = (const uint8_t*)m.seq.p + TEXT_FRONT;
        v.f[k].seq_off = (const uint32_t*)m.off.p;
        v.f[k].qual_off = (const uint32_t*)m.qoff.p;
        v.f[k].seq_len = (const uint32_t*)m.len.p;
        v.f[k].name_off = (const uint32_t*)m.name_off.p;
        v.f[k].name_len = (const uint32_t*)m.name_len.p;
        v.f[k].plus_off = (const uint32_t*)m.plus_off.p;
        v.f[k].plus_len = (const uint32_t*)m.plus_len.p;
        v.f[k].qual_len = (const uint32_t*)m.qual_len.p;
        v.f[k].qview = (const uint32_t*)m.qview.p;
    }
    return v;
}

static int sizes_from_fused(Slot* s, FormatView& v, unsigned long long h_tot[FMT_STREAMS]) {
    unsigned long long misc[5];
    HIP_TRY(hipMemcpyAsync(misc, s->fz_misc.p, sizeof(misc), hipMemcpyDeviceToHost, s->stream));
    HIP_TRY(hipStreamSynchronize(s->stream));
    if ((misc[0] >> 32) != 0) return 0;
    v.fused = 1;
    v.fstate[0] = (const uint32_t*)s->m[0].fz_rec.p; v.fstate[1] = (const uint32_t*)s->m[1].fz_rec.p;
    v.fbatch = (const unsigned long long*)s->fz_state.p;
    v.fbatch_shift = 5;
    static_assert(FastWaveLds<10, true, true>::PPW == 32, "fbatch_shift");
    h_tot[0] = misc[1]; h_tot[3] = misc[2]; h_tot[1] = misc[3]; h_tot[4] = misc[4];
    return 0;
}

static int sizes_from_sums(Slot* s, const FormatView& v, uint64_t n, uint64_t n_tiles, uint64_t n_super, unsigned long long h_tot[FMT_STREAMS]) {
    if (s->f_tile.reserve(sizeof(unsigned long long) * FMT_STREAMS * (n_tiles + n_super)) || s->t_scratch.reserve(TEXT_SCRATCH_BYTES))
        return fail(AQC_ERR_HIP, "hipMalloc failed");
    unsigned long long* d_tot = ((TextScratch*)s->t_scratch.p)->fmt_totals;
    unsigned long long* d_super = (unsigned long long*)s->f_tile.p + FMT_STREAMS * n_tiles;
    if (n) hipLaunchKernelGGL(fmt_tile_sums_kernel, dim3((unsigned)n_super), dim3(TXT_BLOCK), 0, s->stream, v, n, n_tiles, n_super, (unsigned long long*)s->f_tile.p, d_super);
    else HIP_TRY(hipMemsetAsync(s->f_tile.p, 0, sizeof(unsigned long long) * FMT_STREAMS * (n_tiles + n_super), s->stream));
    hipLaunchKernelGGL(fmt_tile_bases_kernel, dim3(v.spans ? FMT_STREAMS : 6), dim3(TXT_BLOCK), 0, s->stream, d_super, n_super, d_tot);
    HIP_TRY(hipGetLastError());
    HIP_TRY(hipMemcpyAsync(h_tot, d_tot, sizeof(unsigned long long) * (v.spans ? FMT_STREAMS : 6), hipMemcpyDeviceToHost, s->stream));
    HIP_TRY(hipStreamSynchronize(s->stream));
    return 0;
}

struct FormatLayout {
    uint64_t n_tasks, gen_cap, per_list;
    uint4 *plan0, *listed, *patch0, *wplan;
    FmtTask* over;
    uint32_t* lists;
    unsigned int *n_gen, *n_whole;
    unsigned list_blocks, copy_blocks;
};
static int carve_format_buffers(Slot* s, uint64_t n, uint64_t n_tiles, FormatLayout& L) {
    const int nf = s->paired ? 2 : 1;
    L.n_tasks = n * nf;
    L.gen_cap = ((n_tiles + GEN_LISTS - 1) / GEN_LISTS) * FMT_TILE * nf;
    const uint64_t plan0_bytes = (16 * L.n_tasks + 255) / 256 * 256;
    if (s->f_plan.reserve(plan0_bytes + 16 * PLAN_Q * L.gen_cap * GEN_LISTS) || s->f_patch.reserve(16 * L.n_tasks + 32 * L.gen_cap * GEN_LISTS) || s->f_over.reserve(sizeof(FmtTask) * L.n_tasks) ||
        s->f_pos.reserve(4 * L.gen_cap * GEN_LISTS + 2 * sizeof(unsigned int) * GEN_LISTS + 64))
        return fail(AQC_ERR_HIP, "hipMalloc failed");
    L.plan0 = (uint4*)s->f_plan.p;
    L.listed = (uint4*)((uint8_t*)s->f_plan.p + plan0_bytes);
    L.patch0 = (uint4*)s->f_patch.p;
    L.wplan = (uint4*)((uint8_t*)s->f_patch.p + 16 * L.n_tasks);
    L.over = (FmtTask*)s->f_over.p;
    L.lists = (uint32_t*)s->f_pos.p;
    L.n_gen = (unsigned int*)((uint8_t*)s->f_pos.p + 4 * L.gen_cap * GEN_LISTS);
    L.n_whole = L.n_gen + GEN_LISTS;
    L.per_list = std::min<uint64_t>(std::max<uint64_t>((L.gen_cap + GEN_ROUND - 1) / GEN_ROUND, 1), 32);
    L.list_blocks = (unsigned)(GEN_LISTS * L.per_list);
    L.copy_blocks = (unsigned)((L.n_tasks + (COPY_BLOCK / 32) * FMT_UNROLL - 1) / ((COPY_BLOCK / 32) * FMT_UNROLL));
    return 0;
}

enum class Writer {
    PLACE_COPY,
    PLAN_WHOLE,
    PLAN_ONLY,
    PLAN_LISTED,
};
static Writer choose_writer(const FormatView& v, int pass) {
    static const bool place_copy = [] { const char* e = getenv("AQC_PLACE_COPY"); return !(e && e[0] == '0'); }();
    const bool sparse = v.spans || v.fused;
    if (sparse) return Writer::PLAN_LISTED;
    if (place_copy && pass == 0 && !v.plain && !v.barcode) return Writer::PLACE_COPY;
    return v.barcode && !v.plain ? Writer::PLAN_ONLY : Writer::PLAN_WHOLE;
}

static void write_pass(Slot* s, const FormatView& v, const FormatLayout& L, const FormatOut& outs, int pass, uint64_t n, uint64_t n_tiles, uint64_t n_super) {
    const unsigned long long* tb = (const unsigned long long*)s->f_tile.p;
    const Writer w = choose_writer(v, pass);
    if (w == Writer::PLACE_COPY) {
        hipLaunchKernelGGL(fmt_place_copy_kernel, dim3((unsigned)n_tiles), dim3(PC_BLOCK), 0, s->stream, v, n, n_tiles, n_super, tb, tb + FMT_STREAMS * n_tiles,
                           L.listed, L.lists, L.n_gen, L.gen_cap, outs);
        hipLaunchKernelGGL(fmt_plan_listed_kernel, dim3(L.list_blocks), dim3(FMT_TILE), 0, s->stream, v, L.listed, L.over,
                           (const uint32_t*)L.lists, (const unsigned int*)L.n_gen, L.gen_cap, s->status);
    } else {
        hipLaunchKernelGGL(fmt_plan_kernel, dim3((unsigned)n_tiles), dim3(FMT_TILE), 0, s->stream, v, n, n_tiles, n_super,
                           tb, tb + FMT_STREAMS * n_tiles, pass, s->status, L.plan0, L.patch0,
                           L.listed, L.over, L.lists, L.n_gen, L.gen_cap, L.wplan, L.n_whole, outs.p[0], outs.p[3],
                           (SpanEvent*)s->m[0].f_events.p, (SpanEvent*)s->m[1].f_events.p);
        if (w == Writer::PLAN_WHOLE) hipLaunchKernelGGL(fmt_copy_whole_kernel, dim3(L.copy_blocks), dim3(COPY_BLOCK), 0, s->stream, v, L.n_tasks, (const uint4*)L.plan0,
                                                        (const uint4*)L.patch0, outs);
        if (w == Writer::PLAN_LISTED) hipLaunchKernelGGL(fmt_copy_whole_list_kernel, dim3(L.list_blocks), dim3(COPY_BLOCK), 0, s->stream, v, (const uint4*)L.wplan, outs,
                                                         (const unsigned int*)L.n_whole, L.gen_cap);
    }
    hipLaunchKernelGGL(fmt_copy_kernel, dim3(L.list_blocks), dim3(COPY_BLOCK), 0, s->stream, v,
                       (const uint4*)L.listed, (const FmtTask*)L.over, outs, (const uint32_t*)L.lists,
                       (const unsigned int*)L.n_gen, L.gen_cap);
}

static int format_impl(aqc_ctx* c, int slot, int verdict_slot, uint64_t n, int32_t store_overlap, uint64_t bytes_out[6], bool spans = false) {
    GET_SLOT(s);
    int rc;
    const bool plain = verdict_slot != slot;
    Slot* vs = s;
    if (plain && (rc = get_slot(c, verdict_slot, &vs))) return rc;
    if (!bytes_out) return fail(AQC_ERR_ARG, "aqc_format: null argument");
    if (!s->framed) return fail(AQC_ERR_STATE, "aqc_format needs a slot filled by aqc_frame");
    if (!vs->ran) return fail(AQC_ERR_STATE, "aqc_format before aqc_run");
    if (n > s->n || n > vs->n) return fail(AQC_ERR_ARG, "aqc_format: n exceeds the slot's records");
    if (plain) HIP_TRY(slot_sync(*vs));
    FormatView v = make_format_view(c, s, vs, plain, store_overlap, spans);
    s->m[0].n_events = s->m[1].n_events = 0;
    const uint64_t n_tiles = n ? (n + FMT_TILE - 1) / FMT_TILE : 1;
    const uint64_t n_super = (n_tiles + FMT_SUPER - 1) / FMT_SUPER;
    unsigned long long h_tot[FMT_STREAMS] = {0, 0, 0, 0, 0, 0, 0, 0};
    if (s->fused && !plain && !spans && !v.store_overlap && n == s->n && n > 0 && (rc = sizes_from_fused(s, v, h_tot))) return rc;
    if (!v.fused) {
        s->fused = false;
        if ((rc = sizes_from_sums(s, v, n, n_tiles, n_super, h_tot))) return rc;
    }
    for (int f = 0; f < (v.spans ? (s->paired ? 2 : 1) : 0); ++f) {
        s->m[f].n_events = h_tot[FMT_EVENT_STREAM + f];
        if (s->m[f].f_events.reserve(sizeof(SpanEvent) * (s->m[f].n_events + 1))) return fail(AQC_ERR_HIP, "hipMalloc failed");
    }
    FormatOut outs{};
    for (int q = 0; q < 6; q++) {
        const bool live = (q < 3 || s->paired) && (q % 3 != 2 || v.store_overlap);
        s->f_bytes[q] = live ? h_tot[q] : 0;
        bytes_out[q] = s->f_bytes[q];
        if (s->f_out[q].reserve(s->f_bytes[q] + 64)) return fail(AQC_ERR_HIP, "hipMalloc failed");
        outs.p[q] = (uint8_t*)s->f_out[q].p;
    }
    if (n) {
        FormatLayout L;
        if ((rc = carve_format_buffers(s, n, n_tiles, L))) return rc;
        for (int pass = 0; pass < (v.store_overlap ? 2 : 1); ++pass) {
            if (pass == 1 && v.store_overlap == AQC_STORE_MERGED) {
                if (!plain) {
                    const unsigned long long* tb = (const unsigned long long*)s->f_tile.p;
                    hipLaunchKernelGGL(fmt_merged_kernel, dim3((unsigned)n_tiles), dim3(FMT_TILE), 0, s->stream, v, n, n_tiles, n_super, tb, tb + FMT_STREAMS * n_tiles,
                                       s->status, outs.p[2]);
                }
                continue;
            }
            HIP_TRY(hipMemsetAsync(L.n_gen, 0, 2 * sizeof(unsigned int) * GEN_LISTS, s->stream));
            write_pass(s, v, L, outs, pass, n, n_tiles, n_super);
        }
        HIP_TRY(hipGetLastError());
    }
    s->formatted = true;
    s->formatted_fused = v.fused != 0;
    s->compressed = false;
    return 0;
}

int aqc_format(aqc_ctx* c, int slot, uint64_t n, int32_t store_overlap, uint64_t bytes_out[6]) {
    return format_impl(c, slot, slot, n, store_overlap, bytes_out);
}

int aqc_format_spans(aqc_ctx* c, int slot, uint64_t n, int32_t store_overlap, uint64_t bytes_out[6], uint64_t n_events[2]) {
    if (!n_events) return fail(AQC_ERR_ARG, "aqc_format_spans: null argument");
    const int rc = format_impl(c, slot, slot, n, store_overlap, bytes_out, true);
    if (rc) return rc;
    n_events[0] = c->slots[slot].m[0].n_events;
    n_events[1] = c->slots[slot].m[1].n_events;
    return 0;
}

int aqc_format_fused(aqc_ctx* c, int slot) {
    GET_SLOT(s);
    if (!s->formatted) return fail(AQC_ERR_STATE, "aqc_format_fused before aqc_format");
    return s->formatted_fused ? 1 : 0;
}

int aqc_span_end(aqc_ctx* c, int slot, uint64_t n, uint64_t end[2]) {
    GET_SLOT(s);
    if (!s->framed || !end || n > s->n) return fail(AQC_ERR_ARG, "aqc_span_end: bad arguments");
    for (int f = 0; f < 2; ++f) {
        end[f] = 0;
        if (f == 1 && !s->paired) break;
        if (n == s->n) { end[f] = s->m[f].consumed; continue; }
        uint32_t off = 0;
        HIP_TRY(hipMemcpyAsync(&off, (const uint32_t*)s->m[f].name_off.p + n, sizeof(off), hipMemcpyDeviceToHost, s->stream));
        HIP_TRY(hipStreamSynchronize(s->stream));
        end[f] = off;
    }
    return 0;
}

int aqc_format_plain(aqc_ctx* c, int slot, int verdict_slot, uint64_t n, int32_t store_overlap, uint64_t bytes_out[6]) {
    if (slot == verdict_slot) return fail(AQC_ERR_ARG, "aqc_format_plain: the verdicts must come from another slot");
    return format_impl(c, slot, verdict_slot, n, store_overlap, bytes_out);
}

int aqc_fetch_text(aqc_ctx* c, int slot, int file, int stream, uint8_t* dst, uint64_t cap) {
    GET_SLOT(s);
    if (!s->formatted) return fail(AQC_ERR_STATE, "aqc_fetch_text before aqc_format");
    if (file < 0 || file > 1 || stream < 0 || stream > 2) return fail(AQC_ERR_ARG, "aqc_fetch_text: bad file/stream");
    const int q = file * 3 + stream;
    return fetch_out(*s, s->f_out[q].p, s->f_bytes[q], dst, cap, "aqc_fetch_text");
}

int aqc_fetch_streams(aqc_ctx* c, int slot, int32_t gz, uint8_t* const dst[6], const uint64_t cap[6]) {
    GET_SLOT(s);
    if (!dst || !cap) return fail(AQC_ERR_ARG, "aqc_fetch_streams: null argument");
    if (!s->formatted) return fail(AQC_ERR_STATE, "aqc_fetch_streams before aqc_format");
    if (gz && !s->compressed) return fail(AQC_ERR_STATE, "aqc_fetch_streams(gz) before aqc_compress");
    for (int q = 0; q < 6; ++q) {
        const uint64_t nb = gz ? s->g_bytes[q] : s->f_bytes[q];
        if (!nb) continue;
        if (!dst[q] || nb > cap[q]) return fail(AQC_ERR_ARG, "aqc_fetch_streams: stream %d (%llu bytes) does not fit", q, (unsigned long long)nb);
        HIP_TRY(hipMemcpyAsync(dst[q], gz ? s->g_packed[q].p : s->f_out[q].p, nb, hipMemcpyDeviceToHost, s->stream));
    }
    HIP_TRY(hipStreamSynchronize(s->stream));
    return check_status(*s);
}

int aqc_fetch_span_events(aqc_ctx* c, int slot, int file, aqc_span_event* dst, uint64_t cap) {
    GET_SLOT(s);
    if (!s->formatted) return fail(AQC_ERR_STATE, "aqc_fetch_span_events before aqc_format_spans");
    if (file < 0 || file > 1) return fail(AQC_ERR_ARG, "aqc_fetch_span_events: bad file");
    static_assert(sizeof(aqc_span_event) == sizeof(SpanEvent), "host and device event layouts must agree");
    const uint64_t ne = s->m[file].n_events;
    if (ne > cap) return fail(AQC_ERR_ARG, "aqc_fetch_span_events: %llu events do not fit %llu", (unsigned long long)ne, (unsigned long long)cap);
    return fetch_out(*s, s->m[file].f_events.p, sizeof(SpanEvent) * ne, dst, sizeof(SpanEvent) * ne, "aqc_fetch_span_events");
}

int aqc_poly_census(aqc_ctx* c, int slot, int32_t poly_max, uint64_t* n_hits) {
    GET_SLOT(s);
    int rc;
    if (!n_hits || poly_max < 1) return fail(AQC_ERR_ARG, "aqc_poly_census: null argument or poly_max < 1");
    if (!s->framed) return fail(AQC_ERR_STATE, "aqc_poly_census needs a slot filled by aqc_frame");
    if (s->paired) return fail(AQC_ERR_ARG, "aqc_poly_census: the census reads single-end slots (one file per chunk)");
    *n_hits = 0;
    s->n_census = 0;
    const uint64_t n = s->n;
    if (s->census_hits.reserve(sizeof(aqc_census_hit) * (n ? n : 1)) || s->census_n.reserve(sizeof(unsigned long long)))
        return fail(AQC_ERR_HIP, "hipMalloc failed");
    HIP_TRY(hipMemsetAsync(s->census_n.p, 0, sizeof(unsigned long long), s->stream));
    if (n) {
        const DevBatch& v = s->view;
        for (hipEvent_t& e : s->census_ev)
            if (!e) HIP_TRY(hipEventCreate(&e));
        HIP_TRY(hipEventRecord(s->census_ev[0], s->stream));
        const uint64_t per_block = (uint64_t)TXT_BLOCK * CENSUS_PER_THREAD;
        hipLaunchKernelGGL(poly_census_kernel, dim3((unsigned)((n + per_block - 1) / per_block)), dim3(TXT_BLOCK), 0, s->stream, v.seq1, v.off1,
                           v.len1, (const uint32_t*)s->m[0].name_off.p, (const uint32_t*)s->m[0].name_len.p, n, (int)poly_max, v.first_index,
                           (aqc_census_hit*)s->census_hits.p, (unsigned long long*)s->census_n.p, s->status);
        const uint64_t name_blocks = std::min<uint64_t>((n + TXT_BLOCK - 1) / TXT_BLOCK, (uint64_t)c->n_cu * 4);
        hipLaunchKernelGGL(census_names_kernel, dim3((unsigned)name_blocks), dim3(TXT_BLOCK), 0, s->stream, v.seq1,
                           (aqc_census_hit*)s->census_hits.p, (const unsigned long long*)s->census_n.p);
        HIP_TRY(hipGetLastError());
        HIP_TRY(hipEventRecord(s->census_ev[1], s->stream));
    }
    unsigned long long h = 0;
    HIP_TRY(hipMemcpyAsync(&h, s->census_n.p, sizeof(h), hipMemcpyDeviceToHost, s->stream));
    HIP_TRY(hipStreamSynchronize(s->stream));
    rc = check_status(*s);
    if (rc) return rc;
    s->n_census = h;
    *n_hits = h;
    return 0;
}

int aqc_census_ms(aqc_ctx* c, int slot, float* ms) {
    GET_SLOT(s);
    if (!ms) return fail(AQC_ERR_ARG, "aqc_census_ms: null argument");
    *ms = 0.f;
    if (s->census_ev[1]) HIP_TRY(hipEventElapsedTime(ms, s->census_ev[0], s->census_ev[1]));
    return 0;
}

int aqc_fetch_census(aqc_ctx* c, int slot, aqc_census_hit* dst, uint64_t cap) {
    GET_SLOT(s);
    if (!dst && cap) return fail(AQC_ERR_ARG, "aqc_fetch_census: null destination");
    const uint64_t m = std::min(cap, s->n_census);
    if (m) {
        HIP_TRY(hipMemcpyAsync(dst, s->census_hits.p, sizeof(aqc_census_hit) * m, hipMemcpyDeviceToHost, s->stream));
        HIP_TRY(hipStreamSynchronize(s->stream));
    }
    return 0;
}

}
```

### afterqc_amd/csrc/aqc_ctx.hpp

```cpp
#pragma once
#include <hip/hip_runtime.h>

#include <atomic>
#include <mutex>
#include <vector>

#include "aqc_dev.hpp"
#include "aqc_batch.hpp"
#include "aqc_qcut.hpp"
#include "aqc_adapter.hpp"
#include "aqc_polytail.hpp"

namespace aqc {

enum ViewPassId { VP_CUT = 0, VP_ADAPTER = 1, VP_POLY = 2, VP_N = 3 };
struct ViewPass { hipEvent_t ev[2] = {nullptr, nullptr}; bool ran = false; };
struct __attribute__((visibility("hidden"))) PassCounts {
    unsigned long long* p = nullptr;
    hipError_t ensure(int device) {
        if (p) return hipSuccess;
        hipError_t e = hipSetDevice(device);
        if (e == hipSuccess) e = hipMalloc((void**)&p, sizeof(unsigned long long) * 4);
        return e == hipSuccess ? zero() : e;
    }
    hipError_t zero() { return p ? hipMemset(p, 0, sizeof(unsigned long long) * 4) : hipSuccess; }
    hipError_t get(int64_t out[4]) const {
        for (int k = 0; k < 4; ++k) out[k] = 0;
        return p ? hipMemcpy(out, p, sizeof(int64_t) * 4, hipMemcpyDeviceToHost) : hipSuccess;
    }
    void free() { if (p) (void)hipFree(p); p = nullptr; }
};

struct __attribute__((visibility("hidden"))) Mate {
    DevBuf seq, qual, off, qoff, len;
    DevBuf qlen, qview;
    DevBuf fz_rec;
    DevBuf line_end, name_off, name_len, plus_off, plus_len, qual_len;
    uint8_t last_byte = '\n';
    uint64_t consumed = 0;
    DevBuf f_events;
    uint64_t n_events = 0;
};

struct MateView { const uint8_t *seq, *qual; const uint32_t *off, *qoff, *len, *qlen; uint32_t* qview; };
static inline void set_mate(DevBatch& v, int k, const MateView& m) {
    if (k == 0) { v.seq1 = m.seq; v.qual1 = m.qual; v.off1 = m.off; v.qoff1 = m.qoff; v.len1 = m.len; v.qlen1 = v.qlen2 = m.qlen; v.qview1 = v.qview2 = m.qview; }
    else { v.seq2 = m.seq; v.qual2 = m.qual; v.off2 = m.off; v.qoff2 = m.qoff; v.len2 = m.len; v.qlen2 = m.qlen; v.qview2 = m.qview; }
}

struct __attribute__((visibility("hidden"))) Slot {
    hipStream_t stream = nullptr;
    int* status = nullptr;
    uint64_t err_record = UINT64_MAX;
    hipEvent_t ev_main = nullptr, ev_qc = nullptr;
    struct QcGen {
        std::atomic<uint64_t> gen{0}, synced{0};
        bool pending() const { return synced.load(std::memory_order_acquire) < gen.load(std::memory_order_acquire); }
    } qc;
    hipEvent_t ev[AQC_N_KERNELS][2] = {};
    bool timed[AQC_N_KERNELS] = {};
    std::vector<hipEvent_t> ring[AQC_N_KERNELS][2];
    int ring_used[AQC_N_KERNELS] = {};
    bool collecting = false;

    bool has_irregular = false;
    Mate m[2];
    DevBuf aux[5], results;
    DevBuf deferred, n_deferred;
    DevBuf off_stage;
    uint32_t max_len = 0;
    uint32_t raw_max_len = 0;
    DevBatch view{};
    uint64_t n = 0;
    bool paired = false, ran = false, used_fast = false;
    int verdict_words = 0;
    DevBuf cut;
    ViewPass pass[VP_N];
    DevBuf fz_state, fz_misc;
    bool fused = false;

    DevBuf t_tile;
    DevBuf t_scratch;
    aqc_text_chunk last_chunk{};
    bool framed = false, formatted = false;
    DevBuf f_pos, f_tile, f_plan, f_patch, f_over, f_out[6];
    bool formatted_fused = false;
    uint64_t f_bytes[6] = {0, 0, 0, 0, 0, 0};
    DevBuf census_hits, census_n;
    uint64_t n_census = 0;
    hipEvent_t census_ev[2] = {nullptr, nullptr};

    DevBuf g_stage, g_sizes, g_offsets, g_total, g_hist, g_code, g_packed[6];
    uint64_t g_bytes[6] = {0, 0, 0, 0, 0, 0};
    bool compressed = false;
};

constexpr int RING_CAP = 256;

constexpr uint64_t KMER_CAP = 1ull << 21;
constexpr uint64_t DENSE_CAP = (uint64_t)N_XCD * DENSE_ENTRIES;

struct __attribute__((visibility("hidden"))) QcDev {
    unsigned long long* acc = nullptr;
    KmerTable kt{};
    unsigned long long last_end = 0, epoch = 0;
};

}

struct __attribute__((visibility("hidden"))) aqc_ctx {
    bool force_generic = false;
    bool fuse_opt = false;
    bool qc_inline = false;
    int device = 0;
    int n_slots = 0;
    std::vector<aqc::Slot> slots;
    aqc_config cfg{};
    bool has_cfg = false;
    aqc::QcutOpts cut{};
    aqc::AdapterOpts adapter{};
    aqc::PolyOpts poly{};
    aqc::PassCounts pass_stats[aqc::VP_N];
    aqc::DevBuf circ[5];
    aqc::DevBuf kmer_partial;
    aqc::DevBuf gz_crc;
    hipStream_t qc_stream = nullptr;
    std::mutex qc_mu;
    aqc::DevCircles circles{};
    unsigned long long *counters = nullptr, *ovl_hist = nullptr, *dist_hist = nullptr;
    aqc::QcDev qc[4];
    int n_cu = 256;
    char name[256] = "";
};

namespace aqc {

struct StatusWords { int status; int pad_; unsigned long long err_key; };
static const StatusWords STATUS_CLEAR{0, 0, ~0ull};
static unsigned long long* err_key_of(const Slot& sl) { return reinterpret_cast<unsigned long long*>(sl.status + 2); }

constexpr size_t ARENA_SLACK = 1024;
constexpr size_t TEXT_FRONT = 64;

#define AQC_INTERNAL __attribute__((visibility("hidden")))
AQC_INTERNAL hipEvent_t launch_event(Slot& s, int k, int which);
AQC_INTERNAL hipError_t slot_sync(Slot& s);
AQC_INTERNAL const char* status_text(int st, bool at_record);
AQC_INTERNAL int check_status(Slot& sl);
AQC_INTERNAL int get_slot(aqc_ctx* c, int slot, Slot** out);
AQC_INTERNAL int fetch_out(Slot& s, const void* src, uint64_t bytes, void* dst, uint64_t cap, const char* who);
AQC_INTERNAL int sync_all(aqc_ctx* c);
AQC_INTERNAL int allow_kmer_lds();
AQC_INTERNAL void free_kmer(KmerTable& t);
#ifdef AQC_PROFILE
AQC_INTERNAL void fetch_kprof(unsigned long long kp[16]);
#endif

#define GET_SLOT(s)                      \
    Slot* s;                             \
    do {                                 \
        int rc_ = get_slot(c, slot, &s); \
        if (rc_) return rc_;             \
    } while (0)

}
```

### afterqc_amd/csrc/aqc_pipe.cpp

```cpp
#include <sys/stat.h>
#include <sys/uio.h>
#include <zlib.h>

#include <atomic>
#include <chrono>
#include <condition_variable>
#include <cstdarg>
#include <cstdio>
#include <cstdlib>
#include <cstring>
#include <map>
#include <memory>
#include <mutex>
#include <string>
#include <thread>
#include <vector>

#include "../../include/afterqc_hip.h"
#include "aqc_gz.hpp"
#include "aqc_pool.hpp"
#include "aqc_pipe_prim.hpp"
#include "aqc_pipe_source.hpp"
#include "aqc_pipe_out.hpp"

// ... 643 lines not shown
        if (bytes < k.fill) k.carry_host.assign(hb.p + bytes, hb.p + k.fill);
        return true;
    }

    void read_stretches(int f, GzSource* src, int dec_device) {
        const uint64_t want_lines = 4 * K;
        double est = 360.0;
        StretchChunk k;
        k.f = f;
        bool eof = false;
        for (uint64_t idx = 0; !abort; ++idx) {
            const bool same_dev = aqc_device_index(P->ctx[(size_t)(idx % jobq.size())]) == dec_device;
            RingHold rb(*this, f);
            size_t cap = 0;
            if (!open_chunk(rb, est, k.carry_host.size(), cap)) return;
            HostBuf& hb = rb.buf();
            if (!take_carry(k, hb, same_dev)) return;
            while (k.lines < want_lines && !eof) {
                if (k.fill >= cap && !grow_chunk(hb, cap, k.fill)) return;
                const size_t want = std::min(hb.cap, cap) - k.fill;
                std::vector<aqcgz::DevSegment> segs;
                const uint64_t tr = now_ns();
                const size_t got = src->read_segments(hb.p + k.fill, want, same_dev ? &segs : nullptr);
                ns_read += now_ns() - tr;
                if (src->failed()) { fail(AQC_ERR_ARG, "%s: %s", io->in_path[f], src->why()); return; }
                if (got < want) eof = true;
                if (!add_stretches(k, hb, got, segs)) return;
            }
            size_t bytes = k.fill;
            if (k.lines >= want_lines && !cut_stretches(k, hb, bytes)) return;
            InChunk c;
            c.idx = idx;
            c.data = hb.p;
            c.bytes = bytes;
            uint8_t last_byte = '\n';
            if (bytes) {
                const Stretch& z = k.st.back();
                if (!z.dev) last_byte = hb.p[bytes - 1];
                else if (k.lines < want_lines && !fetch_now(z.d, z.d.sec_off + z.d.len - 1, z.d.sec_off + z.d.len, &last_byte)) {
                    device_copy_failed(f);
                    return;
                }
            }
            c.last_byte = last_byte;
            for (Stretch& x : k.st)
                if (x.dev && x.len) {
                    if (!c.ext) c.ext = std::make_shared<std::vector<aqcgz::DevSegment>>();
                    x.d.dst_off = x.off;
                    c.ext->push_back(std::move(x.d));
                }
            if (!close_chunk(c, rb, k.lines, eof && k.carry.empty() && k.carry_host.empty(), last_byte, est)) break;
        }
        inq[f]->close();
    }

    void release_inputs(const Job& j) { for (int f = 0; f < nf; ++f) release_ring(f, j.c[f].buf); }
    void dispatcher() {
        bind_io_thread("dispatcher");
        static const uint8_t nothing[1] = {0};
        bool over[2] = {false, nf < 2};
        for (uint64_t idx = 0; !abort && !ended; ++idx) {
            Job j;
            j.idx = idx;
            bool got[2] = {false, false};
            for (int f = 0; f < nf; ++f) {
                if (!over[f]) got[f] = inq[f]->pop(j.c[f]);
                if (!got[f]) {
                    j.c[f] = InChunk();
                    j.c[f].idx = idx; j.c[f].data = nothing; j.c[f].final = true;
                    over[f] = true;
                } else if (j.c[f].final) over[f] = true;
            }
            if (!got[0] && !(nf == 2 && got[1])) break;
            if (abort || ended) { release_inputs(j); break; }
            j.last = j.c[0].final;
            j.ticket = group_tickets[group_of_ctx[idx % jobq.size()]]++;
            if (!jobq[idx % jobq.size()]->push(j)) { release_inputs(j); break; }
            if (j.last) break;
        }
        for (auto& q : jobq) q->close();
    }

    struct Turn {
        aqc_ctx* c;
        int ci, slot, wid;
        Job& j;
        RingHold in[2];
        aqc_text_chunk ch{};
        aqc_frame_info info{};
        uint64_t n = 0;
        bool fatal = false;
        uint64_t tt = 0;
        Turn(Run& r, aqc_ctx* ctx, int ci_, int slot_, Job& job)
            : c(ctx), ci(ci_), slot(slot_), wid(ci_ * r.P->slots + slot_), j(job), in{{r, 0, job.c[0].buf}, {r, 1, job.c[1].buf}} {}
        void drop_input() { in[0].release(); in[1].release(); }
    };
    enum class Step { go, skip, quit };

    void worker(int ci, int slot) {
        aqc_ctx* c = P->ctx[ci];
        {
            const int node = aqc_device_numa_node(c), bound = aqc_bind_thread_to_node(node);
            if (slot == 0 && dbg)
                fprintf(stderr, "pipe: context %d (device %d) — NUMA node %d, its %d slot workers %s; reader / writer / pool threads are not bound (they serve all contexts)\n",
                        ci, aqc_device_index(c), node, P->slots, bound ? "bound to that node's CPUs" : "not bound (single node, unknown, or AQC_PIPE_NUMA=0)");
        }
        Job j;
        int set = 0;
        while (!abort && jobq[ci]->pop(j)) {
            Turn t(*this, c, ci, slot, j);
            if (!frame_chunk(t)) return;
            const Step s = end_of_input(t);
            if (s == Step::quit) return;
            if (s == Step::skip) continue;
            OutChunk oc;
            oc.idx = j.idx; oc.last = j.last; oc.worker = t.wid;
            if (t.n == 0) {
                t.drop_input();
                if (!outq.push(oc)) return;
                continue;
            }
            if (int rc = aqc_run(c, slot, UINT64_MAX)) { fail(rc, "aqc_run: %s", aqc_last_error()); return; }
            if (!qc_turn(t)) return;
            if (!opt->no_output) {
                if (!format_and_fetch(t, oc, set)) return;
                oc.set = set;
                set ^= 1;
            } else if (!sync_only(t)) return;
            oc.n = t.n;
            oc.fatal = t.fatal;
            if (t.fatal) oc.last = true;
            records += t.n;
            if (!outq.push(oc) || t.fatal) return;
        }
    }

    bool frame_chunk(Turn& t) {
        Job& j = t.j;
        aqc_text_chunk& ch = t.ch;
        ch.text1 = j.c[0].data; ch.bytes1 = j.c[0].bytes; ch.final1 = j.c[0].final ? 1 : 0;
        if (nf == 2) { ch.text2 = j.c[1].data; ch.bytes2 = j.c[1].bytes; ch.final2 = j.c[1].final ? 1 : 0; }
        ch.max_records = UINT64_MAX;
        ch.first_index = (opt->chunk_index0 + j.idx * (opt->chunk_index_stride ? opt->chunk_index_stride : 1)) * K;
        t.tt = now_ns();
        int rc;
        {
            GatePass up(*this);
            if (!up.enter(*up_gate[group_of_ctx[t.ci]], j.ticket)) return false;
            if (j.c[0].ext || (nf == 2 && j.c[1].ext)) {
                std::vector<aqc_text_extent> ex[2];
                for (int f = 0; f < nf; ++f)
                    if (j.c[f].ext)
                        for (const aqcgz::DevSegment& g : *j.c[f].ext) ex[f].push_back(aqc_text_extent{(uint64_t)g.dst_off, (uint64_t)g.len, g.dev});
                rc = aqc_frame_mixed(t.c, t.slot, &ch, ex[0].data(), ex[0].size(), j.c[0].last_byte, ex[1].data(), ex[1].size(), nf == 2 ? j.c[1].last_byte : (uint8_t)'\n', &t.info);
                for (int f = 0; f < nf; ++f) j.c[f].ext.reset();
            } else rc = aqc_frame(t.c, t.slot, &ch, &t.info);
        }
        ns_frame += now_ns() - t.tt;
        t.tt = now_ns();
        if (!spans_on || rc) t.drop_input();
        if (rc) { fail(rc, "aqc_frame: %s", aqc_last_error()); return false; }
        t.n = t.info.n;
        return true;
    }

    Step end_of_input(Turn& t) {
        Job& j = t.j;
        const aqc_frame_info& info = t.info;
        const bool fin1 = j.c[0].final, fin2 = nf == 2 ? j.c[1].final : fin1;
        const bool done1 = (info.eof1 || fin1) && info.avail1 == info.n;
        const bool done2 = nf == 2 && (info.eof2 || fin2) && info.avail2 == info.n;
        const bool stop = done1 || (done2 && info.avail1 > info.n);
        std::unique_lock<std::mutex> lk(fr_mu);
        fr_cv.wait(lk, [&] { return abort.load() || framed_next == j.idx; });
        if (abort) return Step::quit;
        const bool behind_end = end_chunk != UINT64_MAX;
        bool foreign = false;
        if (!behind_end) {
            if (stop) {
                end_chunk = j.idx;
                extra_bases = (!done1 && done2 && info.avail1 > info.n) ? info.next_len1 : 0;
                j.last = true;
            } else if (info.n != K) foreign = true;
        }
        framed_next = j.idx + 1;
        lk.unlock();
        fr_cv.notify_all();
        if (foreign) { anomaly = true; t.drop_input(); stop_all(); return Step::quit; }
        if (behind_end) return Step::skip;
        if (stop) end_input();
        return Step::go;
    }

    bool qc_turn(Turn& t) {
        const uint64_t idx = t.j.idx, g0 = t.ch.first_index;
        uint64_t n_qc = t.n;
        if (opt->qc_sample > 0) n_qc = (uint64_t)opt->qc_sample - 1 > g0 ? std::min<uint64_t>(t.n, (uint64_t)opt->qc_sample - 1 - g0) : 0;
        const bool may_qc = opt->qc_sample <= 0 || g0 < (uint64_t)opt->qc_sample - 1;
        if (!may_qc) {
            std::lock_guard<std::mutex> g(qc_mu);
            if (qc_next == idx) { qc_next = idx + 1; qc_cv.notify_all(); }
            return true;
        }
        int rc = 0;
        std::unique_lock<std::mutex> lk(qc_mu);
        qc_cv.wait(lk, [&] { return abort || qc_next == idx; });
        if (!abort && n_qc > 0) {
            rc = aqc_qc_stat(t.c, t.slot, AQC_QC_R1_POST, 0, 0, n_qc, 1);
            if (!rc && nf == 2) rc = aqc_qc_stat(t.c, t.slot, AQC_QC_R2_POST, 1, 0, n_qc, 1);
            if (!rc) rc = aqc_sync(t.c, t.slot);
        }
        qc_next = idx + 1;
        lk.unlock();
        qc_cv.notify_all();
        if (rc && !dies_at_record(t, rc)) { fail(rc, "aqc_qc_stat: %s", aqc_last_error()); return false; }
        return true;
    }

    bool format_and_fetch(Turn& t, OutChunk& oc, int set) {
        GatePass down(*this);
        bool have_set = false;
        uint64_t n_ev[2] = {0, 0};
        for (int round = 0; ; ++round) {
            const char* where = "aqc_format";
            int rc = spans_on ? aqc_format_spans(t.c, t.slot, t.n, opt->store_overlap, oc.sizes, n_ev) : aqc_format(t.c, t.slot, t.n, opt->store_overlap, oc.sizes);
            if (!rc) oc.fused = aqc_format_fused(t.c, t.slot) == 1;
            if (!rc && !have_set) {
                ns_kernels += now_ns() - t.tt;
                t.tt = now_ns();
                if (!acquire_set(t.wid, set)) return false;
                have_set = true;
                ns_wait_set += now_ns() - t.tt;
                t.tt = now_ns();
            }
            oc.gz = gz_on_device;
            if (!rc && oc.gz) { where = "aqc_compress"; rc = aqc_compress(t.c, t.slot, io->gzip_level, oc.gz_sizes); }
            if (!rc) {
                if (!down.held() && !down.enter(*down_gate[group_of_ctx[t.ci]], t.j.ticket)) return false;
                where = "fetching the output streams";
                if (!fetch_streams(t, oc, set, rc)) return false;
                if (!rc && spans_on && !fetch_spans(t, oc, set, n_ev, rc)) return false;
            }
            if (!rc) break;
            if (round == 0 && !t.fatal && dies_at_record(t, rc)) continue;
            fail(rc, "%s: %s", where, aqc_last_error());
            return false;
        }
        down.leave();
        ns_fetch += now_ns() - t.tt;
        return true;
    }
    bool fetch_streams(Turn& t, OutChunk& oc, int set, int& rc) {
        uint8_t* dstq[6] = {nullptr, nullptr, nullptr, nullptr, nullptr, nullptr};
        uint64_t capq[6] = {0, 0, 0, 0, 0, 0};
        for (int q = 0; q < 6; ++q) {
            if (!oc.sizes[q]) continue;
            HostBuf& hb = P->wbufs[t.wid].out[set][q];
            hb.ensure(oc.gz ? oc.gz_sizes[q] : oc.sizes[q]);
            if (!hb.p) { fail(AQC_ERR_HIP, "page-locked allocation failed"); return false; }
            dstq[q] = hb.p; capq[q] = hb.cap;
        }
        rc = aqc_fetch_streams(t.c, t.slot, oc.gz ? 1 : 0, dstq, capq);
        return true;
    }
    bool fetch_spans(Turn& t, OutChunk& oc, int set, const uint64_t n_ev[2], int& rc) {
        auto sp = std::make_shared<OutChunk::Spans>();
        for (int f = 0; f < nf && !rc; ++f) {
            sp->ev[f].resize((size_t)n_ev[f]);
            rc = aqc_fetch_span_events(t.c, t.slot, f, sp->ev[f].data(), n_ev[f]);
            sp->in[f] = t.j.c[f].data;
            sp->end[f] = t.n == t.info.n ? (f == 0 ? t.info.consumed1 : t.info.consumed2) : 0;
        }
        if (!rc && t.n != t.info.n) {
            uint64_t e2[2] = {0, 0};
            rc = aqc_span_end(t.c, t.slot, t.n, e2);
            sp->end[0] = e2[0]; sp->end[1] = e2[1];
        }
        if (rc) return true;
        for (int f = 0; f < nf; ++f) {
            uint64_t total = 0;
            walk_spans(sp->ev[f].data(), 0, sp->ev[f].size(), sp->end[f], [&](uint64_t, uint64_t len) { total += len; }, [&](uint64_t len) { total += len; });
            sp->good_total[f] = total;
        }
        if (!spans_assemble) {
            oc.spans = sp;
            for (int f = 0; f < nf; ++f) oc.in_buf[f] = t.in[f].hand_on();
            return true;
        }
        for (int f = 0; f < nf; ++f) {
            HostBuf& gb = P->wbufs[t.wid].good[set][f];
            gb.pageable = true;
            gb.ensure((size_t)sp->good_total[f] + 64);
            if (sp->good_total[f] && !gb.p) { fail(AQC_ERR_HIP, "allocation of a good-output buffer failed"); return false; }
            assemble_good(*sp, f, oc.sizes[3 * f] ? P->wbufs[t.wid].out[set][3 * f].p : nullptr, gb.p);
            oc.good_ptr[f] = gb.p;
            oc.good_bytes[f] = sp->good_total[f];
        }
        t.drop_input();
        return true;
    }
    bool sync_only(Turn& t) {
        {
            GatePass down(*this);
            if (!down.enter(*down_gate[group_of_ctx[t.ci]], t.j.ticket)) return false;
        }
        const int rc = aqc_sync(t.c, t.slot);
        if (rc && !dies_at_record(t, rc)) { fail(rc, "aqc_sync: %s", aqc_last_error()); return false; }
        return true;
    }

    void assemble_good(const OutChunk::Spans& sp, int f, const uint8_t* patch, uint8_t* dst) {
        const aqc_span_event* ev = sp.ev[f].data();
        const size_t n_ev = sp.ev[f].size();
        const uint8_t* in = sp.in[f];
        const uint64_t TASK = 1u << 20;
        struct Cut { size_t e; uint64_t out, poff; };
        std::vector<Cut> cuts{Cut{0, 0, 0}};
        size_t e = 0;
        uint64_t out = 0, poff = 0;
        walk_spans(ev, 0, n_ev, 0, [&](uint64_t, uint64_t len) { out += len; },
                   [&](uint64_t len) {
                       out += len; poff += len; ++e;
                       if (out - cuts.back().out >= TASK) cuts.push_back(Cut{e, out, poff});
                   });
        P->pool->parallel_for(cuts.size(), [&](size_t t) {
            const bool last = t + 1 == cuts.size();
            uint64_t o = cuts[t].out, po = cuts[t].poff;
            walk_spans(ev, cuts[t].e, last ? n_ev : cuts[t + 1].e, last ? sp.end[f] : 0,
                       [&](uint64_t at, uint64_t len) { memcpy(dst + o, in + at, (size_t)len); o += len; },
                       [&](uint64_t len) { if (len) { memcpy(dst + o, patch + po, (size_t)len); o += len; po += len; } });
        });
    }

    bool dies_at_record(Turn& t, int rc) {
        if (rc != AQC_ERR_INDEX && rc != AQC_ERR_ALPHABET && rc != AQC_ERR_ARG) return false;
        uint64_t rec = UINT64_MAX;
        if (aqc_error_record(t.c, t.slot, &rec) || rec == UINT64_MAX || rec >= t.n) return false;
        {
            std::lock_guard<std::mutex> g(err_mu);
            if (fatal_chunk == UINT64_MAX || t.j.idx < fatal_chunk) {
                fatal_chunk = t.j.idx;
                fatal_err = aqc_last_error();
                fatal_code = rc;
            }
        }
        t.n = rec;
        t.fatal = true;
        return true;
    }

    enum class Feed { nothing, assembled, spans, stream, device_gz };
    struct Share { Feed kind; uint64_t bytes; };
    Share share_of(const OutChunk& oc, int q) const {
        const int f = q / 3;
        uint64_t bytes = oc.sizes[q];
        Feed kind = !io->gzip_out ? Feed::stream : oc.gz ? Feed::device_gz : Feed::stream;
        if (q % 3 == 0 && oc.good_ptr[f]) { kind = Feed::assembled; bytes = oc.good_bytes[f]; }
        else if (q % 3 == 0 && oc.spans) { kind = Feed::spans; bytes = oc.spans->good_total[f]; }
        return Share{bytes ? kind : Feed::nothing, bytes};
    }

    void file_writer(int q) {
        bind_io_thread("file writer");
        std::shared_ptr<Commit> cm;
        while (fileq[q]->pop(cm)) {
            const OutChunk& oc = cm->oc;
            const uint64_t tw = now_ns();
            const Share sh = abort ? Share{Feed::nothing, 0} : share_of(oc, q);
            const uint8_t* p = oc.set >= 0 ? P->wbufs[oc.worker].out[oc.set][q].p : nullptr;
            bool ok = true;
            switch (sh.kind) {
            case Feed::nothing: break;
            case Feed::assembled: ok = out[q].append(oc.good_ptr[q / 3], (size_t)sh.bytes); break;
            case Feed::spans: {
                const OutChunk::Spans& sp = *oc.spans;
                const int f = q / 3;
                std::vector<struct iovec> iov;
                iov.reserve(2 * sp.ev[f].size() + 1);
                uint64_t poff = 0;
                walk_spans(sp.ev[f].data(), 0, sp.ev[f].size(), sp.end[f],
                           [&](uint64_t at, uint64_t len) { iov.push_back({(void*)(sp.in[f] + at), (size_t)len}); },
                           [&](uint64_t len) { if (len) { iov.push_back({(void*)(p + poff), (size_t)len}); poff += len; } });
                ok = out[q].appendv(iov);
                break;
            }
            case Feed::device_gz: ok = out[q].append(p, (size_t)oc.gz_sizes[q]); break;
            case Feed::stream: ok = io->gzip_out ? append_bgzf(q, p, (size_t)sh.bytes) : out[q].append(p, (size_t)sh.bytes); break;
            }
            if (!ok) fail(AQC_ERR_ARG, "write error on output %d (disk full?)", q);
            ns_write += now_ns() - tw;
            if (cm->remaining.fetch_sub(1) == 1) release_set(oc);
            writes_done.fetch_add(1);
        }
    }
    bool append_bgzf(int q, const uint8_t* p, size_t n) {
        const size_t blk = 0xff00;
        const size_t nb = (n + blk - 1) / blk;
        std::vector<std::vector<uint8_t>> z(nb);
        P->pool->parallel_for(nb, [&](size_t i) {
            const size_t o = i * blk;
            bgzf_block(p + o, std::min<size_t>(blk, n - o), io->gzip_level, z[i]);
        });
        size_t total = 0;
        for (auto& b : z) total += b.size();
        std::vector<uint8_t> cat(total);
        size_t o = 0;
        for (auto& b : z) { memcpy(cat.data() + o, b.data(), b.size()); o += b.size(); }
        return out[q].append(cat.data(), total);
    }

    void writer() {
        bind_io_thread("commit");
        std::map<uint64_t, OutChunk> pending;
        uint64_t next = 0;
        OutChunk oc;
// ... 312 lines not shown
```

### include/afterqc_hip.h

```cpp
#ifndef AFTERQC_HIP_H
#define AFTERQC_HIP_H

#include <stdint.h>

#ifdef __cplusplus
extern "C" {
#endif

#define AQC_ABI_VERSION 3

#define AQC_MAX_READ_LEN 1000
#define AQC_QC_COLS 1024

#define AQC_OK 0
#define AQC_ERR_HIP -1
#define AQC_ERR_ARG -2
#define AQC_ERR_READ_TOO_LONG -3
#define AQC_ERR_NO_DEVICE -4
#define AQC_ERR_STATE -5
#define AQC_ERR_ALPHABET -6
#define AQC_ERR_UNSUPPORTED -7
#define AQC_ERR_INDEX -8

enum aqc_flag {
// ... 53 lines not shown
    int32_t no_overlap;
    int32_t no_correction;
    int32_t mask_mismatch;
    int32_t barcode;
    int32_t barcode_length;
    int32_t barcode_verify_len;
    uint8_t barcode_verify[32];
    int32_t debubble;
    int32_t qc_kmer;
} aqc_config;

typedef struct aqc_batch {
    uint64_t n;
    uint64_t first_index;
    const uint8_t* seq1;
    const uint8_t* qual1;
    const uint64_t* off1;
    const uint64_t* qoff1;
    const uint32_t* len1;
    uint64_t bytes1;
    uint64_t qbytes1;
    const uint8_t* seq2;
    const uint8_t* qual2;
    const uint64_t* off2;
    const uint64_t* qoff2;
    const uint32_t* len2;
    uint64_t bytes2;
    uint64_t qbytes2;
    const int32_t* aux_lane;
    const int32_t* aux_tile;
    const int32_t* aux_x;
    const int32_t* aux_y;
    const uint8_t* aux_ok;
    const uint32_t* qlen1;
    const uint32_t* qlen2;
} aqc_batch;

enum aqc_counter {
    AQC_C_TOTAL_READS = 0,
    AQC_C_TOTAL_BASES,
    AQC_C_GOOD_READS,
    AQC_C_GOOD_BASES,
    AQC_C_FLAG0,
    AQC_C_READ_CORRECTED = AQC_C_FLAG0 + AQC_N_FLAGS,
    AQC_C_BASE_CORRECTED,
    AQC_C_BASE_SKIPPED_CORRECTION,
    AQC_C_BASE_ZERO_QUAL_MASKED,
    AQC_C_OVERLAPPED,
    AQC_C_OVERLAP_LEN_SUM,
    AQC_C_OVERLAP_BASE_SUM,
    AQC_C_OVERLAP_BASE_ERR,
    AQC_C_TRIMMED_ADAPTER_BASE,
    AQC_C_TRIMMED_ADAPTER_READ,
    AQC_C_ERR_MATRIX0,
    AQC_N_COUNTERS = AQC_C_ERR_MATRIX0 + 16
};

enum aqc_qc_row {
    AQC_QC_TOTAL_NUM = 0,
    AQC_QC_TOTAL_QUAL,
    AQC_QC_BASE_COUNT_A, AQC_QC_BASE_COUNT_T, AQC_QC_BASE_COUNT_C, AQC_QC_BASE_COUNT_G,
    AQC_QC_BASE_QUAL_A, AQC_QC_BASE_QUAL_T, AQC_QC_BASE_QUAL_C, AQC_QC_BASE_QUAL_G,
    AQC_QC_DISCONTINUITY,
    AQC_QC_GC_HIST,
    AQC_QC_SCALARS,
    AQC_QC_ROWS
};
#define AQC_QC_R1_PRE 0
#define AQC_QC_R2_PRE 1
#define AQC_QC_R1_POST 2
#define AQC_QC_R2_POST 3

enum aqc_kernel_id { AQC_K_FILTER_OVERLAP = 0, AQC_K_QC_STAT = 1, AQC_N_KERNELS = 2 };

typedef struct aqc_ctx aqc_ctx;

int aqc_abi_version(void);
int aqc_device_count(void);
const char* aqc_last_error(void);
int aqc_create(int device, int n_slots, aqc_ctx** out);
void aqc_destroy(aqc_ctx* ctx);
int aqc_device_name(aqc_ctx* ctx, char* buf, int buflen);
int aqc_device_index(aqc_ctx* ctx);
int aqc_device_numa_node(aqc_ctx* ctx);
int aqc_device_numa_node_of(int device);
int aqc_bind_thread_to_node(int node);

int aqc_set_config(aqc_ctx* ctx, const aqc_config* cfg);
int aqc_set_circles(aqc_ctx* ctx, const double* cx, const double* cy, const double* radius,
                    const int32_t* lane, const int32_t* tile, int32_t n);
int aqc_reset_stats(aqc_ctx* ctx);

typedef struct aqc_cut_config { int32_t front, tail, right, window, mean_quality; } aqc_cut_config;
int aqc_set_quality_cut(aqc_ctx* ctx, const aqc_cut_config* cut);
int aqc_get_cut_stats(aqc_ctx* ctx, int64_t out[4]);
int aqc_cut_ms(aqc_ctx* ctx, int slot, float* ms);

typedef struct aqc_adapter_config { int32_t len1, len2, min_overlap; uint8_t seq1[64], seq2[64]; } aqc_adapter_config;
int aqc_set_adapter_trim(aqc_ctx* ctx, const aqc_adapter_config* adapter);
int aqc_get_adapter_stats(aqc_ctx* ctx, int64_t out[4]);
int aqc_adapter_ms(aqc_ctx* ctx, int slot, float* ms);

typedef struct aqc_poly_config { int32_t min_len[4]; } aqc_poly_config;
int aqc_set_poly_trim(aqc_ctx* ctx, const aqc_poly_config* poly);
int aqc_get_poly_stats(aqc_ctx* ctx, int64_t out[4]);
int aqc_poly_ms(aqc_ctx* ctx, int slot, float* ms);

int aqc_upload(aqc_ctx* ctx, int slot, const aqc_batch* batch);
int aqc_run(aqc_ctx* ctx, int slot, uint64_t accum_limit);
int aqc_qc_stat(aqc_ctx* ctx, int slot, int which, int mate, uint64_t first, uint64_t count, int post);
int aqc_last_deferred(aqc_ctx* ctx, int slot, uint32_t* idx, uint64_t cap, uint64_t* n);
int aqc_last_verdict_words(aqc_ctx* ctx, int slot);
int aqc_fetch_results(aqc_ctx* ctx, int slot, aqc_result* out, uint64_t n);
int aqc_sync(aqc_ctx* ctx, int slot);
int aqc_fetch_quality_views(aqc_ctx* ctx, int slot, int mate, uint32_t* out, uint64_t n);
int aqc_error_record(aqc_ctx* ctx, int slot, uint64_t* record);
int aqc_kernel_ms(aqc_ctx* ctx, int slot, float* ms );
int aqc_timing_reset(aqc_ctx* ctx, int slot);
int aqc_timing_mean(aqc_ctx* ctx, int slot, float* mean_ms , int32_t* launches );

int aqc_get_counters(aqc_ctx* ctx, int64_t* out );
int aqc_get_histograms(aqc_ctx* ctx, int64_t* overlap_hist, int64_t* distance_hist, int32_t n);
int aqc_get_qc(aqc_ctx* ctx, int which, int64_t* out );
int aqc_get_kmers(aqc_ctx* ctx, int which, uint64_t* keys, int64_t* counts, uint64_t* order,
                  uint64_t cap, uint64_t* n);

typedef struct aqc_text_chunk {
    const uint8_t* text1;
    uint64_t bytes1;
    const uint8_t* text2;
    uint64_t bytes2;
    int32_t final1, final2;
    uint64_t max_records;
    uint64_t first_index;
} aqc_text_chunk;

typedef struct aqc_frame_info {
    uint64_t n;
    uint64_t avail1, avail2;
    uint64_t consumed1, consumed2;
    int32_t eof1, eof2;
    uint32_t max_len;
    uint32_t next_len1;
} aqc_frame_info;

int aqc_frame(aqc_ctx* ctx, int slot, const aqc_text_chunk* chunk, aqc_frame_info* info);
typedef struct aqc_text_extent {
    uint64_t offset, bytes;
    const void* device_text;
} aqc_text_extent;
int aqc_frame_mixed(aqc_ctx* ctx, int slot, const aqc_text_chunk* chunk, const aqc_text_extent* ext1, uint64_t n_ext1, uint8_t last1,
                    const aqc_text_extent* ext2, uint64_t n_ext2, uint8_t last2, aqc_frame_info* info);
int aqc_reframe(aqc_ctx* ctx, int slot, aqc_frame_info* info);
#define AQC_STORE_OVERLAP 1
#define AQC_STORE_MERGED 2
int aqc_format(aqc_ctx* ctx, int slot, uint64_t n, int32_t store_overlap, uint64_t bytes_out[6]);
typedef struct aqc_span_event {
    uint32_t in_start;
    uint32_t in_len;
    uint32_t out_len;
} aqc_span_event;
int aqc_format_spans(aqc_ctx* ctx, int slot, uint64_t n, int32_t store_overlap, uint64_t bytes_out[6], uint64_t n_events[2]);
int aqc_fetch_span_events(aqc_ctx* ctx, int slot, int file, aqc_span_event* dst, uint64_t cap);
int aqc_span_end(aqc_ctx* ctx, int slot, uint64_t n, uint64_t end[2]);

#define AQC_CENSUS_OK 0
#define AQC_CENSUS_NO_NAME 1
#define AQC_CENSUS_RAISE 2
typedef struct aqc_census_hit {
    uint64_t index;
    int64_t lane, tile_no, tile, x, y;
    uint32_t name_off;
    uint32_t name_len;
    int32_t count;
    uint8_t surface, swath, camera;
    uint8_t base;
    uint8_t status;
    uint8_t wide;
    uint8_t pad_[6];
} aqc_census_hit;
int aqc_poly_census(aqc_ctx* ctx, int slot, int32_t poly_max, uint64_t* n_hits);
int aqc_fetch_census(aqc_ctx* ctx, int slot, aqc_census_hit* dst, uint64_t cap);
int aqc_census_ms(aqc_ctx* ctx, int slot, float* ms);
int aqc_format_fused(aqc_ctx* ctx, int slot);
int aqc_format_plain(aqc_ctx* ctx, int slot, int verdict_slot, uint64_t n, int32_t store_overlap, uint64_t bytes_out[6]);
int aqc_fetch_text(aqc_ctx* ctx, int slot, int file, int stream, uint8_t* dst, uint64_t cap);
int aqc_fetch_streams(aqc_ctx* ctx, int slot, int32_t gz, uint8_t* const dst[6], const uint64_t cap[6]);
int aqc_compress(aqc_ctx* ctx, int slot, int32_t level, uint64_t gz_bytes_out[6]);
int aqc_fetch_gz(aqc_ctx* ctx, int slot, int file, int stream, uint8_t* dst, uint64_t cap);
int aqc_gunzip_dev(int device, const uint8_t* gz, uint64_t size, uint8_t* out, uint64_t cap, uint64_t* n_out, uint64_t stats[8], int threads,
                   uint64_t section_bytes, uint64_t group_bytes);
int aqc_bunzip2_dev(int device, const uint8_t* bz, uint64_t size, uint8_t* out, uint64_t cap, uint64_t* n_out, uint64_t stats[8], int threads,
                    uint64_t group_blocks);
int aqc_gunzip_probe(int engine, int device, const uint8_t* gz, uint64_t size, int n, const uint64_t* nominal, const uint64_t* stop, const uint8_t* exact,
                     uint32_t ratio_cap, uint32_t tok_ratio, uint32_t overlap_tokens, const uint8_t* win, uint64_t wlen, uint64_t* sec, int32_t* run,
                     uint32_t* crc, uint32_t* piece_nl, uint64_t piece_cap, uint64_t* n_pieces, uint8_t* text, uint64_t text_cap, uint64_t* n_text,
                     uint8_t* tail, uint64_t* tail_len);
void* aqc_host_alloc(uint64_t bytes);
void aqc_host_free(void* p);

int aqc_overlap(aqc_ctx* ctx, const aqc_batch* pairs, int32_t* offset, int32_t* overlap_len, int32_t* diff);
int aqc_read_stats(aqc_ctx* ctx, const aqc_batch* reads, int32_t max_poly, int32_t mismatch, int32_t qual,
                   uint8_t* polyx, int32_t* low_qual, int32_t* n_count);
int aqc_edit_distance(aqc_ctx* ctx, const aqc_batch* pairs, int32_t* dist);
int aqc_quality_cut_views(aqc_ctx* ctx, const aqc_batch* reads, const aqc_cut_config* cut, int32_t trim_front, int32_t trim_tail, uint32_t* view);
int aqc_adapter_views(aqc_ctx* ctx, const aqc_batch* reads, const aqc_adapter_config* adapter, int32_t trim_front, int32_t trim_tail,
                      const uint32_t* view_in , uint32_t* view);
int aqc_poly_views(aqc_ctx* ctx, const aqc_batch* reads, const aqc_poly_config* poly, int32_t trim_front, int32_t trim_tail,
                   const uint32_t* view_in , uint32_t* view);

typedef struct aqc_pipe aqc_pipe;

typedef struct aqc_pipe_io {
    const char* in_path[2];
    const uint8_t* in_mem[2];
    uint64_t in_mem_bytes[2];
    int32_t gzip_in[2];
    const char* out_path[2][3];
    int32_t gzip_out;
    int32_t gzip_level;
} aqc_pipe_io;

typedef struct aqc_pipe_opts {
    uint64_t chunk_records;
    int64_t qc_sample;
    int32_t store_overlap;
    int32_t no_output;
    uint64_t chunk_index0;
    uint64_t chunk_index_stride;
} aqc_pipe_opts;

typedef struct aqc_pipe_result {
    uint64_t records;
    uint64_t chunks;
    uint64_t bytes_out[6];
    int32_t anomaly;
    int32_t fused_chunks;
    uint64_t extra_bases;
    double seconds;
    double t_read, t_count, t_wait_ring, t_frame, t_kernels, t_wait_set, t_fetch, t_write;
} aqc_pipe_result;

int aqc_pipe_create(aqc_ctx** ctxs, int32_t n_ctx, int32_t slots_per_ctx, int32_t io_threads, aqc_pipe** out);
void aqc_pipe_destroy(aqc_pipe* p);
int aqc_pipe_run(aqc_pipe* p, const aqc_pipe_io* io, const aqc_pipe_opts* opts, aqc_pipe_result* result);
const char* aqc_pipe_last_error(void);
typedef struct aqc_source aqc_source;
aqc_source* aqc_source_open(const char* path, int32_t gzip, int32_t io_threads);
aqc_source* aqc_source_open2(const char* path, int32_t gzip, int32_t io_threads, uint64_t gz_section_bytes);
int64_t aqc_source_read(aqc_source* s, uint8_t* dst, uint64_t want);
const char* aqc_source_error(aqc_source* s);
int aqc_source_gz_stats(aqc_source* s, uint64_t out[4]);
int aqc_gz_input_stats(uint64_t out[4]);
int aqc_bz2_input_stats(uint64_t out[4]);
void aqc_source_close(aqc_source* s);
int aqc_gz_deflate_block(const uint8_t* src, uint64_t n, int32_t level, uint8_t* dst, uint64_t cap, uint64_t* out_n);
int64_t aqc_gz_inflate_raw(const uint8_t* src, uint64_t n, uint8_t* dst, uint64_t cap);
uint32_t aqc_gz_crc32(uint32_t crc, const uint8_t* p, uint64_t n);

uint64_t aqc_host_count_newlines(const uint8_t* p, uint64_t n);
int aqc_bgzf_compress(const uint8_t* src, uint64_t n, int32_t level, uint8_t* dst, uint64_t cap, uint64_t* out_n);
int aqc_pipe_split(const aqc_pipe_io* io, int32_t file_index, uint64_t chunk_records, int32_t io_threads, uint64_t* bytes,
                   uint64_t* lines, uint64_t cap, uint64_t* n_chunks, uint32_t* crc);

unsigned int edit_distance(const char* a, const unsigned int asize, const char* b, const unsigned int bsize);
int seek_overlap(const char* r1, const int len1, const char* r2_revcomp, const int len2, const int limit_distance,
                 const int complete_compare_require, const int overlap_require);

#ifdef __cplusplus
}
#endif
#endif
```

Before: 64.92.

## Split frame and fetch into begin/end phases and narrow the download gate

Splits framing and stream fetching into begin and end calls. The pipeline's download gate is now held only while the device-to-host copies are enqueued, not across the stream synchronize, span fetch and the rest of the fetch. This lets other slots issue their downloads while one slot waits for completion. It also adds an opt-in per-device link lane (AQC_LINK_ORDER=1) that orders host-device copies across streams through events; it is off by default and adds a mutex and event record on each copy when enabled.

```diff
diff --git a/afterqc_amd/capi.py b/afterqc_amd/capi.py
--- a/afterqc_amd/capi.py
+++ b/afterqc_amd/capi.py
@@ -34,6 +34,7 @@
           -5: "bad call sequence", -6: "byte outside the reference's COMP alphabet", -7: "unsupported option value",
           -8: "quality line too short for the overlap walk (IndexError upstream)"}
 ERR_ARG, ERR_ALPHABET, ERR_INDEX = -2, -6, -8
+ERR_STATE = -5
 RECORD_ERRORS = (ERR_ARG, ERR_ALPHABET, ERR_INDEX)
 
 EDIT_DTYPE = np.dtype([("o", "<u2"), ("kind", "u1"), ("base", "u1"), ("qual", "u1")])
@@ -408,6 +409,14 @@
     lib.aqc_frame_mixed.restype = C.c_int
     lib.aqc_reframe.argtypes = [P, C.c_int, C.POINTER(FrameInfo)]
     lib.aqc_reframe.restype = C.c_int
+    lib.aqc_frame_begin.argtypes = [P, C.c_int, C.POINTER(TextChunk)]
+    lib.aqc_frame_begin_mixed.argtypes = [P, C.c_int, C.POINTER(TextChunk), C.POINTER(TextExtent), C.c_uint64, C.c_uint8, C.POINTER(TextExtent), C.c_uint64, C.c_uint8]
+    lib.aqc_frame_end.argtypes = [P, C.c_int, C.POINTER(FrameInfo)]
+    lib.aqc_fetch_streams_begin.argtypes = [P, C.c_int, C.c_int32, C.POINTER(C.c_void_p * 6), C.POINTER(C.c_uint64 * 6)]
+    lib.aqc_fetch_streams_end.argtypes = [P, C.c_int]
+    lib.aqc_link_stats.argtypes = [C.c_int, C.POINTER(C.c_uint64 * 4)]
+    for name in ("aqc_frame_begin", "aqc_frame_begin_mixed", "aqc_frame_end", "aqc_fetch_streams", "aqc_fetch_streams_begin", "aqc_fetch_streams_end", "aqc_link_stats"):
+        getattr(lib, name).restype = C.c_int
     lib.aqc_format.argtypes = [P, C.c_int, C.c_uint64, C.c_int32, P]
     lib.aqc_format_plain.argtypes = [P, C.c_int, C.c_int, C.c_uint64, C.c_int32, P]
     lib.aqc_fetch_text.argtypes = [P, C.c_int, C.c_int, C.c_int, P, C.c_uint64]
@@ -489,7 +498,17 @@
                     "aqc_set_quality_cut", "aqc_get_cut_stats", "aqc_cut_ms", "aqc_quality_cut_views",
                     "aqc_set_adapter_trim", "aqc_get_adapter_stats", "aqc_adapter_ms", "aqc_adapter_views",
                     "aqc_set_poly_trim", "aqc_get_poly_stats", "aqc_poly_ms", "aqc_poly_views",
+                    "aqc_frame_begin", "aqc_frame_begin_mixed", "aqc_frame_end", "aqc_fetch_streams_begin", "aqc_fetch_streams_end", "aqc_link_stats",
                     "edit_distance", "seek_overlap"]
+
+
+def link_stats(device=0):
+    lib = load_library()
+    out = (C.c_uint64 * 4)()
+    rc = lib.aqc_link_stats(int(device), C.byref(out))
+    if rc != 0:
+        raise AqcError(rc, (lib.aqc_last_error() or b"").decode("utf-8", "replace"))
+    return tuple(int(x) for x in out)
 
 
 class Engine:
@@ -673,6 +692,34 @@
         self._check(self.lib.aqc_frame(self.h, slot, C.byref(ch), C.byref(info)))
         self.slot_n[slot] = info.n
         return info
+
+    def frame_begin(self, slot, text1, bytes1, final1, text2=None, bytes2=0, final2=False, max_records=UINT64_MAX, first_index=0):
+        ch = TextChunk()
+        ch.text1, ch.bytes1, ch.final1 = text1.ctypes.data, int(bytes1), 1 if final1 else 0
+        if text2 is not None:
+            ch.text2, ch.bytes2, ch.final2 = text2.ctypes.data, int(bytes2), 1 if final2 else 0
+        ch.max_records, ch.first_index = int(max_records), int(first_index)
+        self._check(self.lib.aqc_frame_begin(self.h, slot, C.byref(ch)))
+
+    def frame_end(self, slot):
+        info = FrameInfo()
+        self._check(self.lib.aqc_frame_end(self.h, slot, C.byref(info)))
+        self.slot_n[slot] = info.n
+        return info
+
+    def fetch_streams(self, slot, sizes, gz=False, split=False):
+        bufs = [np.zeros(int(nb) + 64, dtype=np.uint8) for nb in sizes]
+        dst = (C.c_void_p * 6)(*[b.ctypes.data for b in bufs])
+        cap = (C.c_uint64 * 6)(*[b.size for b in bufs])
+        if split:
+            self._check(self.lib.aqc_fetch_streams_begin(self.h, slot, 1 if gz else 0, C.byref(dst), C.byref(cap)))
+            self._check(self.lib.aqc_fetch_streams_end(self.h, slot))
+        else:
+            self._check(self.lib.aqc_fetch_streams(self.h, slot, 1 if gz else 0, C.byref(dst), C.byref(cap)))
+        return [b[:int(nb)].tobytes() for b, nb in zip(bufs, sizes)]
+
+    def link_stats(self):
+        return link_stats(int(self.lib.aqc_device_index(self.h)))
 
     def reframe(self, slot):
         info = FrameInfo()
diff --git a/afterqc_amd/csrc/aqc_capi.hip b/afterqc_amd/csrc/aqc_capi.hip
--- a/afterqc_amd/csrc/aqc_capi.hip
+++ b/afterqc_amd/csrc/aqc_capi.hip
@@ -9,6 +9,7 @@
 #include <vector>
 
 #include "aqc_ctx.hpp"
+#include "aqc_link.hpp"
 #include <sys/mman.h>
 #include <sched.h>
 #include <pthread.h>
@@ -97,14 +98,22 @@
     return 0;
 }
 
-int fetch_out(Slot& s, const void* src, uint64_t bytes, void* dst, uint64_t cap, const char* who) {
+int fetch_out(const aqc_ctx* c, Slot& s, const void* src, uint64_t bytes, void* dst, uint64_t cap, const char* who) {
     if (bytes > cap) return fail(AQC_ERR_ARG, "%s: %llu bytes do not fit %llu", who, (unsigned long long)bytes, (unsigned long long)cap);
     if (bytes) {
         if (!dst) return fail(AQC_ERR_ARG, "%s: null destination", who);
+        LinkJoin down(c, s, LINK_DOWN);
+        HIP_TRY(down.begin());
         HIP_TRY(hipMemcpyAsync(dst, src, bytes, hipMemcpyDeviceToHost, s.stream));
+        HIP_TRY(down.end());
     }
     HIP_TRY(hipStreamSynchronize(s.stream));
     return check_status(s);
+}
+
+LinkLane* link_lane(int device, int dir) {
+    static LinkLane lanes[LINK_MAX_DEVICES][2];
+    return device >= 0 && device < LINK_MAX_DEVICES ? &lanes[device][dir] : nullptr;
 }
 
 int sync_all(aqc_ctx* c) {
@@ -155,6 +164,8 @@
     c->fuse_opt = fu && fu[0] == '1';
     const char* qi = getenv("AQC_QC_STREAM");
     c->qc_inline = qi && qi[0] == '0';
+    const char* lo = getenv("AQC_LINK_ORDER");
+    c->link_order = lo && lo[0] == '1';
     if (int rc = allow_kmer_lds()) return rc;
     HIP_TRY(hipStreamCreateWithFlags(&c->qc_stream, hipStreamNonBlocking));
     for (auto& s : c->slots) {
@@ -163,6 +174,7 @@
             for (int j = 0; j < 2; j++) HIP_TRY(hipEventCreate(&s.ev[k][j]));
         HIP_TRY(hipEventCreateWithFlags(&s.ev_main, hipEventDisableTiming));
         HIP_TRY(hipEventCreateWithFlags(&s.ev_qc, hipEventDisableTiming));
+        for (hipEvent_t& e : s.ev_lane) HIP_TRY(hipEventCreateWithFlags(&e, hipEventDisableTiming));
     }
     HIP_TRY(hipMalloc((void**)&c->counters, sizeof(unsigned long long) * (AQC_N_COUNTERS + 16)));
     HIP_TRY(hipMalloc((void**)&c->ovl_hist, sizeof(unsigned long long) * AQC_QC_COLS));
@@ -193,6 +205,18 @@
             for (hipEvent_t e : vp.ev) if (e) (void)hipEventDestroy(e);
         if (s.ev_main) (void)hipEventDestroy(s.ev_main);
         if (s.ev_qc) (void)hipEventDestroy(s.ev_qc);
+        for (int dir = 0; dir < 2; ++dir) {
+            if (!s.ev_lane[dir]) continue;
+            if (LinkLane* lane = link_lane(c->device, dir)) {
+                std::lock_guard<std::mutex> g(lane->mu);
+                if (lane->tail == s.ev_lane[dir]) {
+                    (void)hipEventSynchronize(s.ev_lane[dir]);
+                    lane->tail = nullptr;
+                    lane->tail_stream = nullptr;
+                }
+            }
+            (void)hipEventDestroy(s.ev_lane[dir]);
+        }
         if (s.stream) (void)hipStreamDestroy(s.stream);
     }
     if (c->qc_stream) (void)hipStreamDestroy(c->qc_stream);
@@ -206,6 +230,19 @@
 }
 
 int aqc_device_index(aqc_ctx* c) { return c ? c->device : -1; }
+
+int aqc_link_stats(int device, uint64_t out[4]) {
+    LinkLane* up = link_lane(device, LINK_UP);
+    LinkLane* down = link_lane(device, LINK_DOWN);
+    if (!out || !up || !down) return fail(AQC_ERR_ARG, "aqc_link_stats: bad arguments");
+    LinkLane* lanes[2] = {up, down};
+    for (int dir = 0; dir < 2; ++dir) {
+        std::lock_guard<std::mutex> g(lanes[dir]->mu);
+        out[dir] = lanes[dir]->joined;
+        out[2 + dir] = lanes[dir]->behind;
+    }
+    return 0;
+}
 
 int aqc_device_numa_node_of(int device) {
     char bus[64] = "";
diff --git a/afterqc_amd/csrc/aqc_capi_run.hip b/afterqc_amd/csrc/aqc_capi_run.hip
--- a/afterqc_amd/csrc/aqc_capi_run.hip
+++ b/afterqc_amd/csrc/aqc_capi_run.hip
@@ -500,7 +500,7 @@
     if (!s->compressed) return fail(AQC_ERR_STATE, "aqc_fetch_gz before aqc_compress");
     if (file < 0 || file > 1 || stream < 0 || stream > 2) return fail(AQC_ERR_ARG, "aqc_fetch_gz: bad file/stream");
     const int q = file * 3 + stream;
-    return fetch_out(*s, s->g_packed[q].p, s->g_bytes[q], dst, cap, "aqc_fetch_gz");
+    return fetch_out(c, *s, s->g_packed[q].p, s->g_bytes[q], dst, cap, "aqc_fetch_gz");
 }
 
 static int seam_prepare(aqc_ctx* c, const aqc_batch* b, bool need_qual, bool need_pair, Slot** out) {
diff --git a/afterqc_amd/csrc/aqc_capi_text.hip b/afterqc_amd/csrc/aqc_capi_text.hip
--- a/afterqc_amd/csrc/aqc_capi_text.hip
+++ b/afterqc_amd/csrc/aqc_capi_text.hip
@@ -6,6 +6,7 @@
 #include <algorithm>
 
 #include "aqc_ctx.hpp"
+#include "aqc_link.hpp"
 #include "aqc_prim.hpp"
 #include "aqc_fast.hpp"
 #include "aqc_textin.hpp"
@@ -27,16 +28,6 @@
               sizeof(TextScratch) <= TEXT_SCRATCH_BYTES, "the kernels of both stages were measured with these places");
 
 struct FrameExtents { const aqc_text_extent* ext[2]; uint64_t n[2]; uint8_t last[2]; };
-struct FrameJob {
-    const aqc_text_chunk* ch;
-    int nf;
-    const uint8_t* text[2];
-    uint64_t bytes[2];
-    uint8_t* tbase[2];
-    uint64_t tiles[2], cap[2];
-    uint32_t virt[2];
-    bool bubble;
-};
 constexpr size_t TEXT_SLACK = IDX_TILE + 64;
 
 static int put_extents(Slot* s, const FrameJob& j, int k, const FrameExtents& fx) {
@@ -52,18 +43,27 @@
     return 0;
 }
 
-static int put_text(Slot* s, FrameJob& j, int k, bool resident, const FrameExtents* fx) {
+static int reserve_text(Slot* s, FrameJob& j, int k) {
     Mate& m = s->m[k];
     if (m.seq.reserve(TEXT_FRONT + j.bytes[k] + TEXT_SLACK)) return fail(AQC_ERR_HIP, "hipMalloc of %llu bytes failed", (unsigned long long)j.bytes[k]);
     j.tbase[k] = (uint8_t*)m.seq.p + TEXT_FRONT;
-    if (resident) return 0;
-    const bool mixed = fx && fx->n[k];
-    if (mixed) {
-        const int rc = put_extents(s, j, k, *fx);
-        if (rc) return rc;
-    } else if (j.bytes[k]) HIP_TRY(hipMemcpyAsync(j.tbase[k], j.text[k], j.bytes[k], hipMemcpyHostToDevice, s->stream));
+    return 0;
+}
+static int put_text(const aqc_ctx* c, Slot* s, const FrameJob& j, const FrameExtents* fx) {
+    LinkJoin up(c, *s, LINK_UP);
+    HIP_TRY(up.begin());
+    for (int k = 0; k < j.nf; k++) {
+        if (fx && fx->n[k]) {
+            const int rc = put_extents(s, j, k, *fx);
+            if (rc) return rc;
+        } else if (j.bytes[k]) HIP_TRY(hipMemcpyAsync(j.tbase[k], j.text[k], j.bytes[k], hipMemcpyHostToDevice, s->stream));
+    }
+    HIP_TRY(up.end());
+    return 0;
+}
+static int finish_text(Slot* s, const FrameJob& j, int k, const FrameExtents* fx) {
     HIP_TRY(hipMemsetAsync(j.tbase[k] + j.bytes[k], 0, TEXT_SLACK, s->stream));
-    m.last_byte = !j.bytes[k] ? (uint8_t)'\n' : mixed ? fx->last[k] : j.text[k][j.bytes[k] - 1];
+    s->m[k].last_byte = !j.bytes[k] ? (uint8_t)'\n' : (fx && fx->n[k]) ? fx->last[k] : j.text[k][j.bytes[k] - 1];
     return 0;
 }
 
@@ -179,11 +179,14 @@
     info->next_len1 = fo.next_len1;
 }
 
-static int frame_impl(aqc_ctx* c, int slot, const aqc_text_chunk* ch, aqc_frame_info* info, bool resident, const FrameExtents* fx = nullptr) {
-    GET_SLOT(s);
-    if (!ch || !info || !ch->text1) return fail(AQC_ERR_ARG, "aqc_frame: null argument");
+static int frame_begin(aqc_ctx* c, int slot, const aqc_text_chunk* ch, bool resident, const FrameExtents* fx = nullptr) {
+    GET_SLOT(s);
+    if (!ch || !ch->text1) return fail(AQC_ERR_ARG, "aqc_frame: null argument");
+    if (s->frame_open) return fail(AQC_ERR_STATE, "aqc_frame_begin: the slot's last aqc_frame_begin has had no aqc_frame_end");
     const bool paired = ch->text2 != nullptr;
-    FrameJob j{ch, paired ? 2 : 1, {ch->text1, ch->text2}, {ch->bytes1, paired ? ch->bytes2 : 0}};
+    s->open_chunk = *ch;
+    FrameJob& j = s->open_job;
+    j = FrameJob{&s->open_chunk, paired ? 2 : 1, {ch->text1, ch->text2}, {ch->bytes1, paired ? ch->bytes2 : 0}};
     for (int k = 0; k < j.nf; k++)
         if (j.bytes[k] >= (1ull << 31) - IDX_TILE) return fail(AQC_ERR_ARG, "aqc_frame: chunks must be < 2 GiB");
     HIP_TRY(slot_sync(*s));
@@ -193,34 +196,67 @@
     if (s->t_scratch.reserve(TEXT_SCRATCH_BYTES)) return fail(AQC_ERR_HIP, "hipMalloc failed");
     int rc;
     for (int k = 0; k < j.nf; k++)
-        if ((rc = put_text(s, j, k, resident, fx)) || (rc = size_line_table(s, j, k))) return rc;
+        if ((rc = reserve_text(s, j, k)) || (rc = size_line_table(s, j, k))) return rc;
     if (s->t_tile.reserve(sizeof(unsigned long long) * (j.tiles[0] + j.tiles[1] + 1))) return fail(AQC_ERR_HIP, "hipMalloc failed");
+    if (!resident) {
+        if ((rc = put_text(c, s, j, fx))) return rc;
+        for (int k = 0; k < j.nf; k++)
+            if ((rc = finish_text(s, j, k, fx))) return rc;
+    }
     const int final_[2] = {ch->final1, ch->final2};
     for (int k = 0; k < j.nf; k++)
         if (final_[k] && j.bytes[k] > 0 && s->m[k].last_byte != '\n') j.virt[k] = (uint32_t)j.bytes[k] | LINE_WS;
     j.bubble = c->has_cfg && c->cfg.debubble;
+    s->frame_open = true;
+    return 0;
+}
+
+static int frame_end(aqc_ctx* c, int slot, aqc_frame_info* info) {
+    GET_SLOT(s);
+    if (!info) return fail(AQC_ERR_ARG, "aqc_frame: null argument");
+    if (!s->frame_open) return fail(AQC_ERR_STATE, "aqc_frame_end without aqc_frame_begin");
+    s->frame_open = false;
+    FrameJob& j = s->open_job;
+    int rc;
     FrameOut fo{};
     if ((rc = index_and_frame(s, j, fo)) || (rc = publish_view(s, j, fo))) return rc;
-    fill_frame_info(info, fo, paired);
+    fill_frame_info(info, fo, j.nf == 2);
     s->framed = true;
-    s->last_chunk = *ch;
-    return 0;
-}
-
-int aqc_frame(aqc_ctx* c, int slot, const aqc_text_chunk* ch, aqc_frame_info* info) { return frame_impl(c, slot, ch, info, false); }
+    s->last_chunk = s->open_chunk;
+    return 0;
+}
+
+int aqc_frame_begin(aqc_ctx* c, int slot, const aqc_text_chunk* ch) { return frame_begin(c, slot, ch, false); }
+
+int aqc_frame_begin_mixed(aqc_ctx* c, int slot, const aqc_text_chunk* ch, const aqc_text_extent* ext1, uint64_t n_ext1, uint8_t last1,
+                          const aqc_text_extent* ext2, uint64_t n_ext2, uint8_t last2) {
+    if ((n_ext1 && !ext1) || (n_ext2 && !ext2)) return fail(AQC_ERR_ARG, "aqc_frame_mixed: null extent list");
+    const FrameExtents fx{{ext1, ext2}, {n_ext1, ch && ch->text2 ? n_ext2 : 0}, {last1, last2}};
+    return frame_begin(c, slot, ch, false, &fx);
+}
+
+int aqc_frame_end(aqc_ctx* c, int slot, aqc_frame_info* info) { return frame_end(c, slot, info); }
+
+int aqc_frame(aqc_ctx* c, int slot, const aqc_text_chunk* ch, aqc_frame_info* info) {
+    if (!info) return fail(AQC_ERR_ARG, "aqc_frame: null argument");
+    const int rc = aqc_frame_begin(c, slot, ch);
+    return rc ? rc : frame_end(c, slot, info);
+}
 
 int aqc_frame_mixed(aqc_ctx* c, int slot, const aqc_text_chunk* ch, const aqc_text_extent* ext1, uint64_t n_ext1, uint8_t last1,
                     const aqc_text_extent* ext2, uint64_t n_ext2, uint8_t last2, aqc_frame_info* info) {
-    if ((n_ext1 && !ext1) || (n_ext2 && !ext2)) return fail(AQC_ERR_ARG, "aqc_frame_mixed: null extent list");
-    const FrameExtents fx{{ext1, ext2}, {n_ext1, ch && ch->text2 ? n_ext2 : 0}, {last1, last2}};
-    return frame_impl(c, slot, ch, info, false, &fx);
+    if (!info) return fail(AQC_ERR_ARG, "aqc_frame: null argument");
+    const int rc = aqc_frame_begin_mixed(c, slot, ch, ext1, n_ext1, last1, ext2, n_ext2, last2);
+    return rc ? rc : frame_end(c, slot, info);
 }
 
 int aqc_reframe(aqc_ctx* c, int slot, aqc_frame_info* info) {
     GET_SLOT(s);
     if (!s->framed) return fail(AQC_ERR_STATE, "aqc_reframe needs a slot filled by aqc_frame");
+    if (!info) return fail(AQC_ERR_ARG, "aqc_frame: null argument");
     const aqc_text_chunk ch = s->last_chunk;
-    return frame_impl(c, slot, &ch, info, true);
+    const int rc = frame_begin(c, slot, &ch, true);
+    return rc ? rc : frame_end(c, slot, info);
 }
 
 static FormatView make_format_view(const aqc_ctx* c, const Slot* s, const Slot* vs, bool plain, int32_t store_overlap, bool spans) {
@@ -446,22 +482,41 @@
     if (!s->formatted) return fail(AQC_ERR_STATE, "aqc_fetch_text before aqc_format");
     if (file < 0 || file > 1 || stream < 0 || stream > 2) return fail(AQC_ERR_ARG, "aqc_fetch_text: bad file/stream");
     const int q = file * 3 + stream;
-    return fetch_out(*s, s->f_out[q].p, s->f_bytes[q], dst, cap, "aqc_fetch_text");
-}
-
-int aqc_fetch_streams(aqc_ctx* c, int slot, int32_t gz, uint8_t* const dst[6], const uint64_t cap[6]) {
+    return fetch_out(c, *s, s->f_out[q].p, s->f_bytes[q], dst, cap, "aqc_fetch_text");
+}
+
+int aqc_fetch_streams_begin(aqc_ctx* c, int slot, int32_t gz, uint8_t* const dst[6], const uint64_t cap[6]) {
     GET_SLOT(s);
     if (!dst || !cap) return fail(AQC_ERR_ARG, "aqc_fetch_streams: null argument");
     if (!s->formatted) return fail(AQC_ERR_STATE, "aqc_fetch_streams before aqc_format");
     if (gz && !s->compressed) return fail(AQC_ERR_STATE, "aqc_fetch_streams(gz) before aqc_compress");
+    if (s->fetch_open) return fail(AQC_ERR_STATE, "aqc_fetch_streams_begin: the slot's last aqc_fetch_streams_begin has had no aqc_fetch_streams_end");
     for (int q = 0; q < 6; ++q) {
         const uint64_t nb = gz ? s->g_bytes[q] : s->f_bytes[q];
-        if (!nb) continue;
-        if (!dst[q] || nb > cap[q]) return fail(AQC_ERR_ARG, "aqc_fetch_streams: stream %d (%llu bytes) does not fit", q, (unsigned long long)nb);
-        HIP_TRY(hipMemcpyAsync(dst[q], gz ? s->g_packed[q].p : s->f_out[q].p, nb, hipMemcpyDeviceToHost, s->stream));
-    }
+        if (nb && (!dst[q] || nb > cap[q])) return fail(AQC_ERR_ARG, "aqc_fetch_streams: stream %d (%llu bytes) does not fit", q, (unsigned long long)nb);
+    }
+    LinkJoin down(c, *s, LINK_DOWN);
+    HIP_TRY(down.begin());
+    for (int q = 0; q < 6; ++q) {
+        const uint64_t nb = gz ? s->g_bytes[q] : s->f_bytes[q];
+        if (nb) HIP_TRY(hipMemcpyAsync(dst[q], gz ? s->g_packed[q].p : s->f_out[q].p, nb, hipMemcpyDeviceToHost, s->stream));
+    }
+    HIP_TRY(down.end());
+    s->fetch_open = true;
+    return 0;
+}
+
+int aqc_fetch_streams_end(aqc_ctx* c, int slot) {
+    GET_SLOT(s);
+    if (!s->fetch_open) return fail(AQC_ERR_STATE, "aqc_fetch_streams_end without aqc_fetch_streams_begin");
+    s->fetch_open = false;
     HIP_TRY(hipStreamSynchronize(s->stream));
     return check_status(*s);
+}
+
+int aqc_fetch_streams(aqc_ctx* c, int slot, int32_t gz, uint8_t* const dst[6], const uint64_t cap[6]) {
+    const int rc = aqc_fetch_streams_begin(c, slot, gz, dst, cap);
+    return rc ? rc : aqc_fetch_streams_end(c, slot);
 }
 
 int aqc_fetch_span_events(aqc_ctx* c, int slot, int file, aqc_span_event* dst, uint64_t cap) {
@@ -471,7 +526,7 @@
     static_assert(sizeof(aqc_span_event) == sizeof(SpanEvent), "host and device event layouts must agree");
     const uint64_t ne = s->m[file].n_events;
     if (ne > cap) return fail(AQC_ERR_ARG, "aqc_fetch_span_events: %llu events do not fit %llu", (unsigned long long)ne, (unsigned long long)cap);
-    return fetch_out(*s, s->m[file].f_events.p, sizeof(SpanEvent) * ne, dst, sizeof(SpanEvent) * ne, "aqc_fetch_span_events");
+    return fetch_out(c, *s, s->m[file].f_events.p, sizeof(SpanEvent) * ne, dst, sizeof(SpanEvent) * ne, "aqc_fetch_span_events");
 }
 
 int aqc_poly_census(aqc_ctx* c, int slot, int32_t poly_max, uint64_t* n_hits) {
diff --git a/afterqc_amd/csrc/aqc_ctx.hpp b/afterqc_amd/csrc/aqc_ctx.hpp
--- a/afterqc_amd/csrc/aqc_ctx.hpp
+++ b/afterqc_amd/csrc/aqc_ctx.hpp
@@ -48,11 +48,23 @@
     else { v.seq2 = m.seq; v.qual2 = m.qual; v.off2 = m.off; v.qoff2 = m.qoff; v.len2 = m.len; v.qlen2 = m.qlen; v.qview2 = m.qview; }
 }
 
+struct FrameJob {
+    const aqc_text_chunk* ch;
+    int nf;
+    const uint8_t* text[2];
+    uint64_t bytes[2];
+    uint8_t* tbase[2];
+    uint64_t tiles[2], cap[2];
+    uint32_t virt[2];
+    bool bubble;
+};
+
 struct __attribute__((visibility("hidden"))) Slot {
     hipStream_t stream = nullptr;
     int* status = nullptr;
     uint64_t err_record = UINT64_MAX;
     hipEvent_t ev_main = nullptr, ev_qc = nullptr;
+    hipEvent_t ev_lane[2] = {nullptr, nullptr};
     struct QcGen {
         std::atomic<uint64_t> gen{0}, synced{0};
         bool pending() const { return synced.load(std::memory_order_acquire) < gen.load(std::memory_order_acquire); }
@@ -83,6 +95,9 @@
     DevBuf t_scratch;
     aqc_text_chunk last_chunk{};
     bool framed = false, formatted = false;
+    aqc_text_chunk open_chunk{};
+    FrameJob open_job{};
+    bool frame_open = false, fetch_open = false;
     DevBuf f_pos, f_tile, f_plan, f_patch, f_over, f_out[6];
     bool formatted_fused = false;
     uint64_t f_bytes[6] = {0, 0, 0, 0, 0, 0};
@@ -112,6 +127,7 @@
     bool force_generic = false;
     bool fuse_opt = false;
     bool qc_inline = false;
+    bool link_order = false;
     int device = 0;
     int n_slots = 0;
     std::vector<aqc::Slot> slots;
@@ -148,7 +164,7 @@
 AQC_INTERNAL const char* status_text(int st, bool at_record);
 AQC_INTERNAL int check_status(Slot& sl);
 AQC_INTERNAL int get_slot(aqc_ctx* c, int slot, Slot** out);
-AQC_INTERNAL int fetch_out(Slot& s, const void* src, uint64_t bytes, void* dst, uint64_t cap, const char* who);
+AQC_INTERNAL int fetch_out(const aqc_ctx* c, Slot& s, const void* src, uint64_t bytes, void* dst, uint64_t cap, const char* who);
 AQC_INTERNAL int sync_all(aqc_ctx* c);
 AQC_INTERNAL int allow_kmer_lds();
 AQC_INTERNAL void free_kmer(KmerTable& t);
diff --git a/afterqc_amd/csrc/aqc_link.hpp b/afterqc_amd/csrc/aqc_link.hpp
--- /dev/null
+++ b/afterqc_amd/csrc/aqc_link.hpp
@@ -0,0 +1,49 @@
+#pragma once
+#include <hip/hip_runtime.h>
+
+#include <cstdint>
+#include <mutex>
+
+#include "aqc_ctx.hpp"
+
+namespace aqc {
+
+enum LinkDir { LINK_UP = 0, LINK_DOWN = 1 };
+constexpr int LINK_MAX_DEVICES = 64;
+
+struct LinkLane {
+    std::mutex mu;
+    hipEvent_t tail = nullptr;
+    hipStream_t tail_stream = nullptr;
+    uint64_t joined = 0, behind = 0;
+};
+
+AQC_INTERNAL LinkLane* link_lane(int device, int dir);
+
+struct LinkJoin {
+    LinkLane* lane;
+    Slot& s;
+    const int dir;
+    LinkJoin(const aqc_ctx* c, Slot& slot, int direction) : lane(c->link_order ? link_lane(c->device, direction) : nullptr), s(slot), dir(direction) {
+        if (lane) lane->mu.lock();
+    }
+    LinkJoin(const LinkJoin&) = delete;
+    LinkJoin& operator=(const LinkJoin&) = delete;
+    ~LinkJoin() { if (lane) lane->mu.unlock(); }
+    hipError_t begin() {
+        if (!lane || !lane->tail || lane->tail_stream == s.stream) return hipSuccess;
+        lane->behind++;
+        return hipStreamWaitEvent(s.stream, lane->tail, 0);
+    }
+    hipError_t end() {
+        if (!lane) return hipSuccess;
+        const hipError_t e = hipEventRecord(s.ev_lane[dir], s.stream);
+        if (e != hipSuccess) return e;
+        lane->tail = s.ev_lane[dir];
+        lane->tail_stream = s.stream;
+        lane->joined++;
+        return hipSuccess;
+    }
+};
+
+}
diff --git a/afterqc_amd/csrc/aqc_pipe.cpp b/afterqc_amd/csrc/aqc_pipe.cpp
--- a/afterqc_amd/csrc/aqc_pipe.cpp
+++ b/afterqc_amd/csrc/aqc_pipe.cpp
@@ -819,10 +819,11 @@
                 for (int f = 0; f < nf; ++f)
                     if (j.c[f].ext)
                         for (const aqcgz::DevSegment& g : *j.c[f].ext) ex[f].push_back(aqc_text_extent{(uint64_t)g.dst_off, (uint64_t)g.len, g.dev});
-                rc = aqc_frame_mixed(t.c, t.slot, &ch, ex[0].data(), ex[0].size(), j.c[0].last_byte, ex[1].data(), ex[1].size(), nf == 2 ? j.c[1].last_byte : (uint8_t)'\n', &t.info);
-                for (int f = 0; f < nf; ++f) j.c[f].ext.reset();
-            } else rc = aqc_frame(t.c, t.slot, &ch, &t.info);
-        }
+                rc = aqc_frame_begin_mixed(t.c, t.slot, &ch, ex[0].data(), ex[0].size(), j.c[0].last_byte, ex[1].data(), ex[1].size(), nf == 2 ? j.c[1].last_byte : (uint8_t)'\n');
+            } else rc = aqc_frame_begin(t.c, t.slot, &ch);
+        }
+        if (!rc) rc = aqc_frame_end(t.c, t.slot, &t.info);
+        for (int f = 0; f < nf; ++f) j.c[f].ext.reset();
         ns_frame += now_ns() - t.tt;
         t.tt = now_ns();
         if (!spans_on || rc) t.drop_input();
@@ -885,8 +886,7 @@
     }
 
     bool format_and_fetch(Turn& t, OutChunk& oc, int set) {
-        GatePass down(*this);
-        bool have_set = false;
+        bool have_set = false, had_turn = false;
         uint64_t n_ev[2] = {0, 0};
         for (int round = 0; ; ++round) {
             const char* where = "aqc_format";
@@ -903,9 +903,8 @@
             oc.gz = gz_on_device;
             if (!rc && oc.gz) { where = "aqc_compress"; rc = aqc_compress(t.c, t.slot, io->gzip_level, oc.gz_sizes); }
             if (!rc) {
-                if (!down.held() && !down.enter(*down_gate[group_of_ctx[t.ci]], t.j.ticket)) return false;
                 where = "fetching the output streams";
-                if (!fetch_streams(t, oc, set, rc)) return false;
+                if (!fetch_streams(t, oc, set, had_turn, rc)) return false;
                 if (!rc && spans_on && !fetch_spans(t, oc, set, n_ev, rc)) return false;
             }
             if (!rc) break;
@@ -913,11 +912,10 @@
             fail(rc, "%s: %s", where, aqc_last_error());
             return false;
         }
-        down.leave();
         ns_fetch += now_ns() - t.tt;
         return true;
     }
-    bool fetch_streams(Turn& t, OutChunk& oc, int set, int& rc) {
+    bool fetch_streams(Turn& t, OutChunk& oc, int set, bool& had_turn, int& rc) {
         uint8_t* dstq[6] = {nullptr, nullptr, nullptr, nullptr, nullptr, nullptr};
         uint64_t capq[6] = {0, 0, 0, 0, 0, 0};
         for (int q = 0; q < 6; ++q) {
@@ -927,7 +925,13 @@
             if (!hb.p) { fail(AQC_ERR_HIP, "page-locked allocation failed"); return false; }
             dstq[q] = hb.p; capq[q] = hb.cap;
         }
-        rc = aqc_fetch_streams(t.c, t.slot, oc.gz ? 1 : 0, dstq, capq);
+        {
+            GatePass down(*this);
+            if (!had_turn && !down.enter(*down_gate[group_of_ctx[t.ci]], t.j.ticket)) return false;
+            had_turn = true;
+            rc = aqc_fetch_streams_begin(t.c, t.slot, oc.gz ? 1 : 0, dstq, capq);
+        }
+        if (!rc) rc = aqc_fetch_streams_end(t.c, t.slot);
         return true;
     }
     bool fetch_spans(Turn& t, OutChunk& oc, int set, const uint64_t n_ev[2], int& rc) {
diff --git a/include/afterqc_hip.h b/include/afterqc_hip.h
--- a/include/afterqc_hip.h
+++ b/include/afterqc_hip.h
@@ -229,6 +229,11 @@
 int aqc_frame_mixed(aqc_ctx* ctx, int slot, const aqc_text_chunk* chunk, const aqc_text_extent* ext1, uint64_t n_ext1, uint8_t last1,
                     const aqc_text_extent* ext2, uint64_t n_ext2, uint8_t last2, aqc_frame_info* info);
 int aqc_reframe(aqc_ctx* ctx, int slot, aqc_frame_info* info);
+int aqc_frame_begin(aqc_ctx* ctx, int slot, const aqc_text_chunk* chunk);
+int aqc_frame_begin_mixed(aqc_ctx* ctx, int slot, const aqc_text_chunk* chunk, const aqc_text_extent* ext1, uint64_t n_ext1, uint8_t last1,
+                          const aqc_text_extent* ext2, uint64_t n_ext2, uint8_t last2);
+int aqc_frame_end(aqc_ctx* ctx, int slot, aqc_frame_info* info);
+int aqc_link_stats(int device, uint64_t out[4]);
 #define AQC_STORE_OVERLAP 1
 #define AQC_STORE_MERGED 2
 int aqc_format(aqc_ctx* ctx, int slot, uint64_t n, int32_t store_overlap, uint64_t bytes_out[6]);
@@ -263,6 +268,8 @@
 int aqc_format_plain(aqc_ctx* ctx, int slot, int verdict_slot, uint64_t n, int32_t store_overlap, uint64_t bytes_out[6]);
 int aqc_fetch_text(aqc_ctx* ctx, int slot, int file, int stream, uint8_t* dst, uint64_t cap);
 int aqc_fetch_streams(aqc_ctx* ctx, int slot, int32_t gz, uint8_t* const dst[6], const uint64_t cap[6]);
+int aqc_fetch_streams_begin(aqc_ctx* ctx, int slot, int32_t gz, uint8_t* const dst[6], const uint64_t cap[6]);
+int aqc_fetch_streams_end(aqc_ctx* ctx, int slot);
 int aqc_compress(aqc_ctx* ctx, int slot, int32_t level, uint64_t gz_bytes_out[6]);
 int aqc_fetch_gz(aqc_ctx* ctx, int slot, int file, int stream, uint8_t* dst, uint64_t cap);
 int aqc_gunzip_dev(int device, const uint8_t* gz, uint64_t size, uint8_t* out, uint64_t cap, uint64_t* n_out, uint64_t stats[8], int threads,
```

Result: slower. 62.66 (-3.5%).
